# CODEJIN/multi_speaker_tts

Measured on AMD Instinct MI355X. Metric: mel-frames/sec (train step) at batch 32x(128 tok,800 mel), higher is better.
Workload: dtype f32

## Files before the change

### include/mstts.h

```cpp
#ifndef MSTTS_H_
#define MSTTS_H_
#include <stdint.h>
#ifdef __cplusplus
extern "C" {
#endif

typedef void* mstts_stream_t;

enum { MSTTS_OK = 0, MSTTS_ERR_SHAPE = -1, MSTTS_ERR_DTYPE = -2, MSTTS_ERR_ALIGN = -3, MSTTS_ERR_LAUNCH = -4 };
enum { MSTTS_ACT_NONE = 0, MSTTS_ACT_RELU = 1, MSTTS_ACT_TANH = 2, MSTTS_ACT_SIGMOID = 3 };

const char* mstts_last_error(void);
int mstts_abi_version(void);
int mstts_debug_park_cus(int32_t n_workgroups, int64_t microseconds, uint32_t* done_count, mstts_stream_t s);

typedef struct {
    const float* A; const float* B; float* C; const float* bias;
    int64_t M, N, K;
    int64_t lda, ldb, ldc;
    int32_t trans_a, trans_b;
    int32_t win_T, win_C, win_pad;
    int32_t act, accumulate, split_k;
    int64_t batch, stride_a, stride_b, stride_c;
    float alpha;
// ... 215 lines not shown
int32_t mstts_skinny_fwd_splits(int64_t N, int64_t K);
int mstts_skinny_fwd(const float* X, int64_t ldx, const float* W, int64_t ldw, float* P, int64_t pstride, int64_t M, int64_t N,
                     int64_t K, int32_t ksplit, mstts_stream_t s);
int32_t mstts_skinny_bwd_splits(int64_t R, int64_t N);
int mstts_skinny_bwd(const float* dG, int64_t ldg, const float* W, int64_t ldw, float* P, int64_t pstride, int64_t M, int64_t R,
                     int64_t N, int32_t nsplit, mstts_stream_t s);
int mstts_pack_skinny_bwd(const float* W, int64_t ldw, float* Wp, int64_t R, int64_t N, int32_t nsplit, mstts_stream_t s);
int mstts_skinny_bwd_pair(const float* dG, const float* dG2, int64_t ldg, const float* W, const float* W2, int64_t ldw, float* P, float* P2,
                          int64_t pstride, int64_t M, int64_t R, int64_t N, int32_t nsplit, mstts_stream_t s);
int mstts_skinny_bwd_packed(const float* dG, int64_t ldg, const float* Wp, float* P, int64_t pstride, int64_t M, int64_t R,
                            int64_t N, int32_t nsplit, mstts_stream_t s);

int mstts_wg_overlap_add(const float* Y, const float* bias, float* out, int64_t N, int64_t T, int64_t K, int64_t S, int64_t C, mstts_stream_t s);
int mstts_wg_gate(const float* a, int64_t lda, float* z, int64_t rows, int64_t C, mstts_stream_t s);
int mstts_wg_gate_add(const float* a, int64_t lda, const float* b, float* z, int64_t rows, int64_t C, mstts_stream_t s);
int mstts_wg_res_skip(const float* z, const float* rs, float* x, float* out, int64_t rows, int64_t C, int32_t last, int32_t first, mstts_stream_t s);
int mstts_wg_coupling_inv(const float* audio, const float* log_s_b, const float* w_inv, const float* early, float sigma, float* out,
                          int64_t rows, int64_t c, int64_t c_early, mstts_stream_t s);
int mstts_philox_normal(float* out, int64_t n, uint64_t seed, uint32_t stream_id, float sigma, mstts_stream_t s);

typedef struct {
    const float* v; const float* g; float* w; int64_t ldw;
    float* dv; float* dg;
    int64_t rows, cols;
} mstts_wg_wn_desc;
int mstts_wg_weight_norm_fwd(const mstts_wg_wn_desc* table, int64_t n, int64_t max_cols, mstts_stream_t s);
int mstts_wg_weight_norm_bwd(const mstts_wg_wn_desc* table, int64_t n, int64_t max_cols, mstts_stream_t s);
int mstts_wg_coupling_fwd(const float* y, const float* log_s_b, float* next, float* z, int64_t ldz, int64_t z_col, int64_t c_out,
                          float* loss, int64_t rows, int64_t c, mstts_stream_t s);
int mstts_wg_coupling_bwd(const float* y, const float* log_s_b, const float* z, int64_t ldz, int64_t z_col, int64_t c_out, const float* d_next,
                          float inv_size, float* d_y, float* d_log_s_b, int64_t rows, int64_t c, mstts_stream_t s);
int mstts_wg_inv1x1_logdet(const float* params, float* grad, const int64_t* table, int64_t n_flows, float grad_scale, float* loss, mstts_stream_t s);
int mstts_wg_gate_bwd(const float* a, int64_t lda, const float* dz, float* dpre, float* dpre2, int64_t ld2, int64_t rows, int64_t C, mstts_stream_t s);
int mstts_wg_res_skip_bwd(const float* d_x_next, const float* d_skip, float* d_rs, float* d_z, int64_t rows, int64_t C, int32_t last, mstts_stream_t s);
int mstts_wg_overlap_add_bwd(const float* d_up, float* dY, int64_t N, int64_t T, int64_t K, int64_t S, int64_t C, int64_t L, mstts_stream_t s);
int mstts_wg_bias_fold(const float* base, const int64_t* table, float* out, int64_t n_blocks, int64_t width, mstts_stream_t s);
int mstts_adam_tf_clip(float* p, const float* grad, float* m, float* v, const float* sumsq, float sumsq_scale, float clip_norm,
                       float lr_t, float beta1, float beta2, float eps, int64_t n, mstts_stream_t s);

int64_t mstts_ge2e_ws_floats(int64_t N, int64_t D, int64_t S);
int mstts_ge2e_loss_fwd_bwd(const float* x, int64_t ldx, int64_t S, int64_t P, int64_t D, const float* wb, float* out,
                            float* dx, int64_t lddx, float* ws, mstts_stream_t s);

int32_t mstts_skinny_bf16_fwd_splits(int64_t N, int64_t K);
int32_t mstts_skinny_bf16_bwd_splits(int64_t R, int64_t N);
int mstts_pack_bf16_fwd(const float* W, int64_t ldw, void* Wp, int64_t K, int64_t N, int32_t ksplit, mstts_stream_t s);
int mstts_pack_bf16_bwd(const float* W, int64_t ldw, void* Wq, int64_t R, int64_t N, int32_t nsplit, mstts_stream_t s);
int mstts_skinny_fwd_bf16(const float* X, int64_t ldx, const void* Wp, float* P, int64_t pstride, int64_t M, int64_t N, int64_t K,
                          int32_t ksplit, mstts_stream_t s);
int mstts_skinny_bwd_bf16(const float* dG, int64_t ldg, const void* Wq, float* P, int64_t pstride, int64_t M, int64_t R, int64_t N,
                          int32_t nsplit, mstts_stream_t s);

int mstts_fold_rows(const float* src, float* dst, int64_t rows, int64_t cols, int64_t r0, int64_t n, mstts_stream_t s);

typedef struct {
    int64_t B, T, H;
    const float* xw;
    const float* wh; int64_t wh_ld;
    const int32_t* lengths;
    int32_t reverse;
    float zoneout;
    const uint8_t* zc; const uint8_t* zh;
    const float* residual;
    float* out; int64_t out_sb, out_st;
    float* c_hist; float* h_hist; float* acts; float* c_raw;
    float* gates_ws;
    const float* wh_p; float* h_p;
} mstts_lstm_seq_fwd_desc;
int mstts_lstm_seq_fwd(const mstts_lstm_seq_fwd_desc* d, mstts_stream_t s);
int mstts_lstm_seq_fwd_pair(const mstts_lstm_seq_fwd_desc* a, const mstts_lstm_seq_fwd_desc* b, mstts_stream_t s);
int64_t mstts_lstm_seq_ws_floats(int64_t B, int64_t H, int32_t backward);

typedef struct {
    int64_t B, T, H;
    const float* wh; int64_t wh_ld;
    const int32_t* lengths; int32_t reverse;
    float zoneout;
    const uint8_t* zc; const uint8_t* zh;
    const float* d_out; int64_t dout_sb, dout_st;
    const float* c_hist; const float* acts; const float* c_raw;
    float* dgates_step; float* dgates_pos;
    float* ws;
} mstts_lstm_seq_bwd_desc;
int mstts_lstm_seq_bwd(const mstts_lstm_seq_bwd_desc* d, mstts_stream_t s);
int mstts_lstm_seq_bwd_pair(const mstts_lstm_seq_bwd_desc* a, const mstts_lstm_seq_bwd_desc* b, mstts_stream_t s);

int32_t mstts_persist_lstm_supported(int64_t B, int64_t H);
int64_t mstts_persist_lstm_pack_floats(void);
int64_t mstts_persist_lstm_ws_bytes(void);
int mstts_persist_lstm_pack(const float* wh, int64_t wh_ld, float* fwd_pk, float* bwd_pk, mstts_stream_t s);
int64_t mstts_persist_lstm_hist_floats(int64_t T);
int64_t mstts_persist_lstm_bwd_floats(int64_t T);
int mstts_lstm_seq_fwd_pair_persistent(const mstts_lstm_seq_fwd_desc* a, const mstts_lstm_seq_fwd_desc* b, const float* pk_a, const float* pk_b,
                                       float* xch, uint32_t* ctrl, float* hist, mstts_stream_t s);
int mstts_lstm_seq_bwd_pair_persistent(const mstts_lstm_seq_bwd_desc* a, const mstts_lstm_seq_bwd_desc* b, const float* pkt_a, const float* pkt_b,
                                       float* xch, uint32_t* ctrl, const float* hist, float* bws, mstts_stream_t s);
int32_t mstts_persist_lstm_supported_n(int64_t B, int64_t H, int32_t ndir);
int32_t mstts_persist_lstm_fwd_supported_n(int64_t B, int64_t H, int32_t ndir);
int mstts_persist_lstm_pack_fwd(const float* wh, int64_t wh_ld, int64_t H, float* fwd_pk, mstts_stream_t s);
int64_t mstts_persist_lstm_ws_bytes_n(int64_t B, int32_t ndir);
int64_t mstts_persist_lstm_hist_floats_n(int64_t T, int64_t B, int32_t ndir);
int64_t mstts_persist_lstm_bwd_floats_n(int64_t T, int64_t B, int32_t ndir);
int mstts_lstm_seq_fwd_persistent(const mstts_lstm_seq_fwd_desc* a, const float* pk, float* xch, uint32_t* ctrl, float* hist, mstts_stream_t s);
int mstts_lstm_seq_bwd_persistent(const mstts_lstm_seq_bwd_desc* a, const float* pkt, float* xch, uint32_t* ctrl, const float* hist, float* bws, mstts_stream_t s);

typedef struct {
    int64_t B, S, H, P;
    mstts_lsa_const lsa;
    const float* xw0;
    const float* w0f;
    const float* w1; const float* b1;
    const float* wq;
    const uint8_t* zc0; const uint8_t* zh0; const uint8_t* zc1; const uint8_t* zh1;
    float zoneout;
    float* in0; float* in1; float* pj;
    float* c0; float* c1; float* acts0; float* acts1; float* craw0; float* craw1;
    float* q_hist; float* align_hist; float* cum_hist;
    float* gates_ws; float* energy_ws;
    float* q_ws;
    int32_t chains;
    const void* bf_w0f_f; const void* bf_w1_f; const void* bf_wq_f; const void* bf_w0f_b; const void* bf_w1_b; const void* bf_wq_b;
    const float* w0p; const float* w1p;
    const void* w0p16; const void* w1p16;
    const float* w0f_bp; const float* w1_bp; const float* wq_bp;
    const float* wq_t;
    float* act_p;
    int64_t energy_ws_floats;
} mstts_decoder_train_desc;
int32_t mstts_decoder_bf16_splits(int64_t H, int64_t M, int64_t A, int32_t* out6);
int mstts_decoder_train_ws_floats(int64_t B, int64_t H, int64_t M, int64_t A, int64_t* gates, int64_t* q);
int mstts_decoder_train_fwd(const mstts_decoder_train_desc* d, mstts_stream_t s);

typedef struct {
    const float* w0pk; const float* w1pk; const float* wqpk;
    float* xch; uint32_t* ctrl; uint64_t* stamps;
    float* opk;
    int32_t selftest_fail_step;
    int32_t near_xcd;
    const float* pre; const float* b0;
    int32_t recurrent_bf16;
} mstts_persist_desc;
int32_t mstts_persist_fwd_supported(int64_t B, int64_t H, int64_t M, int64_t A, int64_t T, int64_t KS);
int64_t mstts_persist_fwd_ws_bytes(void);
int64_t mstts_persist_pack_floats(int32_t which);
int mstts_persist_pack(const float* w0f, const float* w1, const float* wq, const float* wx0, float* w0pk, float* w1pk, float* wqpk, mstts_stream_t s);
int mstts_decoder_train_fwd_persistent(const mstts_decoder_train_desc* d, const mstts_persist_desc* p, mstts_stream_t s);
int64_t mstts_persist_opk_floats(int64_t S);
int mstts_persist_unpack_history(const float* opk, const mstts_decoder_train_desc* d, mstts_stream_t s);

typedef struct {
    const mstts_decoder_train_desc* fwd;
    float* d_pj; float* dg0; float* dg1; float* dq_hist; float* de_hist; float* d_in0;
    float* ws;
} mstts_decoder_train_bwd_desc;
int mstts_decoder_train_bwd(const mstts_decoder_train_bwd_desc* d, mstts_stream_t s);
int64_t mstts_decoder_train_bwd_ws_floats(int64_t B, int64_t H, int64_t M, int64_t A, int64_t T, int64_t CH);
int32_t mstts_decoder_train_bwd_parts(int64_t H, int64_t M);

int32_t mstts_persist_bwd_supported(int64_t B, int64_t H, int64_t M, int64_t A, int64_t T, int64_t KS);
int64_t mstts_persist_bwd_ws_bytes(void);
int64_t mstts_persist_bwd_pack_floats(int32_t which);
int mstts_persist_bwd_pack(const float* w0f, const float* w1, const float* wq, float* w0t, float* w1t, float* wqt, mstts_stream_t s);
int mstts_decoder_train_bwd_persistent(const mstts_decoder_train_bwd_desc* bd, const mstts_persist_desc* p, mstts_stream_t s);

typedef struct {
    int64_t B, H, P, n_mel, Smax;
    mstts_lsa_const lsa;
    const float* pw0; const float* pb0; const float* pw1; const float* pb1;
    const uint8_t* pm0; const uint8_t* pm1; float prenet_keep;
    const float* wx0; const float* b0;
    const float* w0f; const float* w1; const float* b1; const float* wq;
    const float* wproj; const float* bproj;
    float zoneout;
    float* in0; float* in1; float* pj;
    float* c0; float* c1;
    float* cum;
    float* pre_ws;
    float* linear; float* stop; float* align_hist;
    const float* w0s; const float* wp_pad;
    const float* w0sp; const float* w1p; float* act_p;
    const float* wp_own; const float* vp;
} mstts_decoder_infer_desc;
int32_t mstts_decoder_infer_fast(int64_t B, int64_t H, int64_t P, int64_t M, int64_t A, int64_t n_mel);
int mstts_decoder_infer_steps(const mstts_decoder_infer_desc* d, int64_t step0, int64_t n, mstts_stream_t s);
int64_t mstts_decoder_infer_ws_floats(int64_t B, int64_t H, int64_t P, int64_t T, int64_t A, int64_t n_mel);

typedef struct {
    const float* w0pk; const float* w1pk; const float* wqppk;
    const float* pre0; const float* bf; const float* u; const float* vp; const float* bp_pad;
    float* xch; uint32_t* ctrl;
    void* stamps;
    int32_t selftest_fail_step;
    int32_t near_xcd;
} mstts_persist_infer_desc;
int32_t mstts_persist_infer_supported(int64_t B, int64_t H, int64_t P, int64_t M, int64_t A, int64_t T, int64_t KS, int64_t n_mel);
int64_t mstts_persist_infer_ws_bytes(void);
int64_t mstts_persist_infer_pack_floats(void);
int mstts_persist_infer_pack(const float* wq, const float* wp_pad, int64_t wp_ld, const float* wfm, float* wqppk, mstts_stream_t s);
int mstts_decoder_infer_persistent(const mstts_decoder_infer_desc* d, const mstts_persist_infer_desc* p, mstts_stream_t s);

int mstts_f32_to_bf16(const float* x, void* y_bf16, int64_t n, mstts_stream_t s);
int mstts_bf16_to_f32(const void* x_bf16, float* y, int64_t n, mstts_stream_t s);
int mstts_bf16_chunks_sum(const void* chunks_bf16, int32_t nchunks, int64_t stride, int64_t n, void* out_bf16, mstts_stream_t s);

enum { MSTTS_PROBE_OFF = 0, MSTTS_PROBE_LSA_ENERGY = 1, MSTTS_PROBE_LSA_CONTEXT = 2, MSTTS_PROBE_CELL0_GEMM = 3,
       MSTTS_PROBE_CELL1_GEMM = 4, MSTTS_PROBE_LSA_DALIGN = 5, MSTTS_PROBE_LSA_DENERGY = 6, MSTTS_PROBE_CELL0_DGEMM = 7,
       MSTTS_PROBE_CELL1_DGEMM = 8 };
int mstts_probe_begin(int32_t kind, int64_t max_launches);
int64_t mstts_probe_result(double* total_ms, double* empty_total_ms);

#ifdef __cplusplus
}
#endif
#endif
```

### multi_speaker_tts_amd/csrc/lsa.hip

```cpp
#include "common.h"

namespace mstts {

constexpr int TS = 8;
constexpr int A_ = 128;
constexpr int CH_ = 32;
constexpr int FLD = CH_ + 4;
constexpr int KS_MAX = 31;
constexpr int LKT_LD = 36;

__device__ __forceinline__ float fast_tanh(float x) {
    const float ax = fabsf(x);
    const float e = __expf(-2.0f * ax);
    return copysignf((1.0f - e) / (1.0f + e), x);
}


__global__ __launch_bounds__(256) void lsa_energy_kernel(mstts_lsa_const c, const float* __restrict__ q, int q_parts, long q_pstride,
                                                         float* __restrict__ q_sum, const float* __restrict__ cum,
                                                         float* __restrict__ energy) {
    __shared__ float s_cum[TS + KS_MAX - 1];
    __shared__ float s_red[TS][2];
    const int b = blockIdx.x, t0 = blockIdx.y * TS, T = (int)c.T, KS = (int)c.KS, pad = (KS - 1) / 2;
    const int k = threadIdx.x & (A_ - 1), grp = threadIdx.x >> 7;
// ... 880 lines not shown
        if (t < T) s_a[t] = av[i];
    }
    *reinterpret_cast<float4*>(&s_dc[lane * 4 + 256 * w]) = dsum;
    if (threadIdx.x < TS) s_gn[threadIdx.x] = gn_own;
#pragma unroll
    for (int i = 0; i < NLK4; ++i) {
        const int e = (threadIdx.x + 256 * i) * 4;
        if (e < KS_MAX * A_) *reinterpret_cast<float4*>(&s_lk[e / A_][e % A_]) = lkv[i];
    }
    if (threadIdx.x < TS + KS_MAX - 1) s_cum[threadIdx.x] = cwin;
    __syncthreads();
    float fac[TS / 2];
    {
        float lk[KS_MAX];
#pragma unroll
        for (int j = 0; j < KS_MAX; ++j) lk[j] = s_lk[j][k];
#pragma unroll
        for (int i = 0; i < TS / 2; ++i) {
            const int tt = grp + 2 * i;
            float pre = kv[i] + qk;
#pragma unroll
            for (int j = 0; j < KS_MAX; ++j) pre += s_cum[tt + j] * lk[j];
            const float u = fast_tanh(pre);
            fac[i] = (t0 + tt < T) ? wk * (1.f - u * u) : 0.f;
        }
    }
#pragma unroll
    for (int m = 0; m < MROW; ++m) dcv[m] = *reinterpret_cast<const float4*>(&s_dc[lane * 4 + 256 * m]);
    float part = 0.f;
#pragma unroll
    for (int i = 0; i < T_MAX / 256; ++i) part += av[i] * gnv[i];
    auto tile_dot = [&](const float4& hq, int e) {
        const int tau = e >> 3, j0 = (e & 7) * 4, t = tau - pad + j0;
        float r = 0.f;
        if (j0 < KS && t >= 0 && t < T) r += hq.x * s_a[t];
        if (j0 + 1 < KS && t + 1 >= 0 && t + 1 < T) r += hq.y * s_a[t + 1];
        if (j0 + 2 < KS && t + 2 >= 0 && t + 2 < T) r += hq.z * s_a[t + 2];
        if (j0 + 3 < KS && t + 3 >= 0 && t + 3 < T) r += hq.w * s_a[t + 3];
        return r;
    };
#pragma unroll
    for (int i = 0; i < HT4; ++i) part += tile_dot(ht[i], threadIdx.x + 256 * i);
    if (h_next)
        for (int e = threadIdx.x + 256 * HT4; (e >> 3) < T; e += 256)
            part += tile_dot(reinterpret_cast<const float4*>(h_next + (long)b * T * HLD)[e], e);
    if (w == 0) {
        float p2 = 0.f;
#pragma unroll
        for (int m = 0; m < MROW; ++m) p2 += cxv[m].x * dcv[m].x + cxv[m].y * dcv[m].y + cxv[m].z * dcv[m].z + cxv[m].w * dcv[m].w;
        for (int i = lane * 4 + 256 * MROW; i < M; i += 256) {
            const float4 x = *reinterpret_cast<const float4*>(ctx_fwd + (long)b * ctx_fwd_ld + i);
            float4 y = *reinterpret_cast<const float4*>(dc + i);
            if (d_ctx2)
                for (int pp = 0; pp < max(d_ctx2_parts, 1); ++pp) {
                    const float4 y2 = *reinterpret_cast<const float4*>(d_ctx2 + pp * d_ctx2_pstride + (long)b * d_ctx2_ld + i);
                    y.x += y2.x; y.y += y2.y; y.z += y2.z; y.w += y2.w;
                }
            p2 += x.x * y.x + x.y * y.y + x.z * y.z + x.w * y.w;
        }
        p2 = wave_sum(p2);
        if (lane == 0) s_dot2 = p2;
    }
    part = wave_sum(part);
    if (lane == 0) scratch[w] = part;
#pragma unroll
    for (int r = 0; r < TS / 4; ++r) {
        const int tt = w + 4 * r, t = t0 + tt;
        float acc = 0.f;
#pragma unroll
        for (int m = 0; m < MROW; ++m)
            acc += val[r][m].x * dcv[m].x + val[r][m].y * dcv[m].y + val[r][m].z * dcv[m].z + val[r][m].w * dcv[m].w;
        if (t < len) {
            for (int i = lane * 4 + 256 * MROW; i < M; i += 256) {
                const float4 x = *reinterpret_cast<const float4*>(c.values + ((long)b * T + t) * M + i);
                float4 y = *reinterpret_cast<const float4*>(dc + i);
                if (d_ctx2)
                    for (int pp = 0; pp < max(d_ctx2_parts, 1); ++pp) {
                        const float4 y2 = *reinterpret_cast<const float4*>(d_ctx2 + pp * d_ctx2_pstride + (long)b * d_ctx2_ld + i);
                        y.x += y2.x; y.y += y2.y; y.z += y2.z; y.w += y2.w;
                    }
                acc += x.x * y.x + x.y * y.y + x.z * y.z + x.w * y.w;
            }
        }
        acc = wave_sum(acc);
        if (lane == 0) {
            const float g = (t < T) ? s_G[tt] + s_gn[tt] : 0.f;
            if (t < T) G[(long)b * T + t] = g;
            s_da[tt] = (t < T) ? g + acc : 0.f;
        }
    }
    __syncthreads();
    const float dot = ((scratch[0] + scratch[1]) + (scratch[2] + scratch[3])) + s_dot2;
    if (threadIdx.x < TS) {
        const int t = t0 + threadIdx.x;
        if (t < T) d_e_out[(long)b * T + t] = a_own * (s_da[threadIdx.x] - dot);
    }
    float dq_acc = 0.f;
#pragma unroll
    for (int i = 0; i < TS / 2; ++i) {
        const int tt = grp + 2 * i;
        const float de = (t0 + tt < T) ? s_a[t0 + tt] * (s_da[tt] - dot) : 0.f;
        const float g = de * fac[i];
        s_g[tt][k] = g;
        dq_acc += g;
    }
    if (grp == 1) s_dq[k] = dq_acc;
    __syncthreads();
    if (grp == 0) atomicAdd(dq + (long)b * A_ + k, dq_acc + s_dq[k]);
    {
        const int tt = threadIdx.x >> 5, j = threadIdx.x & 31;
        float acc = 0.f;
        if (j < KS) {
#pragma unroll 8
            for (int kk = 0; kk < A_; kk += 4) {
                const float4 g4 = *reinterpret_cast<const float4*>(&s_g[tt][kk]);
                const float4 l4 = *reinterpret_cast<const float4*>(&s_lk[j][kk]);
                acc += g4.x * l4.x + g4.y * l4.y + g4.z * l4.z + g4.w * l4.w;
            }
        }
        if (t0 + tt < T) h[((long)b * T + t0 + tt) * HLD + j] = acc;
    }
}

constexpr int PT = 32;
constexpr int LP_ROWS = 34, LP_GROUPS = 16;
constexpr int LP_WN = 80;
typedef float lp_f32x16 __attribute__((ext_vector_type(16)));
typedef __bf16 lp_bf16x8 __attribute__((ext_vector_type(8)));
__device__ __forceinline__ uint32_t lp_cvt_pk(float a, float b) {
    uint32_t r;
    asm("v_cvt_pk_bf16_f32 %0, %1, %2" : "=v"(r) : "v"(a), "v"(b));
    return r;
}
__device__ __forceinline__ void lp_split2(float x0, float x1, uint32_t& hi, uint32_t& mid, uint32_t& lo) {
    hi = lp_cvt_pk(x0, x1);
    x0 -= __uint_as_float(hi << 16); x1 -= __uint_as_float(hi & 0xffff0000u);
    mid = lp_cvt_pk(x0, x1);
    x0 -= __uint_as_float(mid << 16); x1 -= __uint_as_float(mid & 0xffff0000u);
    lo = lp_cvt_pk(x0, x1);
}
__device__ __forceinline__ void lp_split8(const float* x, lp_bf16x8& hi, lp_bf16x8& mid, lp_bf16x8& lo) {
    uint4 h, m, l;
    lp_split2(x[0], x[1], h.x, m.x, l.x); lp_split2(x[2], x[3], h.y, m.y, l.y);
    lp_split2(x[4], x[5], h.z, m.z, l.z); lp_split2(x[6], x[7], h.w, m.w, l.w);
    hi = __builtin_bit_cast(lp_bf16x8, h); mid = __builtin_bit_cast(lp_bf16x8, m); lo = __builtin_bit_cast(lp_bf16x8, l);
}
#define LP_SIX(acc, ah, am, al, bh, bm, bl) do { \
        acc = __builtin_amdgcn_mfma_f32_32x32x16_bf16(al, bh, acc, 0, 0, 0); acc = __builtin_amdgcn_mfma_f32_32x32x16_bf16(ah, bl, acc, 0, 0, 0); \
        acc = __builtin_amdgcn_mfma_f32_32x32x16_bf16(am, bm, acc, 0, 0, 0); acc = __builtin_amdgcn_mfma_f32_32x32x16_bf16(am, bh, acc, 0, 0, 0); \
        acc = __builtin_amdgcn_mfma_f32_32x32x16_bf16(ah, bm, acc, 0, 0, 0); acc = __builtin_amdgcn_mfma_f32_32x32x16_bf16(ah, bh, acc, 0, 0, 0); } while (0)
#ifndef LSA_PARAM_WAVES
#define LSA_PARAM_WAVES 3
#endif
__global__ __launch_bounds__(256, LSA_PARAM_WAVES) void lsa_param_bwd_kernel(mstts_lsa_const c, int S, int steps_per_block,
                                                            const float* __restrict__ q_hist, const float* __restrict__ cum_hist,
                                                            const float* __restrict__ de_hist, float* __restrict__ d_keys,
                                                            float* __restrict__ d_loc_k, float* __restrict__ d_score_w,
                                                            float* __restrict__ d_score_b, float* __restrict__ part) {
    __shared__ __attribute__((aligned(16))) uint16_t s_wp[2][3][8][LP_WN];
    __shared__ __attribute__((aligned(16))) float s_de[2][PT];
    const int b = blockIdx.x, t0 = blockIdx.y * PT, T = (int)c.T, B = (int)c.B, KS = (int)c.KS, pad = (KS - 1) / 2;
    const int s_beg = blockIdx.z * steps_per_block, s_end = min(S, s_beg + steps_per_block);
    const int lane = threadIdx.x & 63, wave = threadIdx.x >> 6, l31 = lane & 31, kh = lane >> 5;
    const int a = wave * 32 + l31;
    const int pl = (l31 & 0x13) | ((l31 & 4) << 1) | ((l31 & 8) >> 1);
    const int o1 = (pl & 7) * LP_WN + 8 + (pl & ~7) + 8 * kh, o2 = (l31 & 7) * LP_WN + 8 + (l31 & ~7) + 8 * kh;
    lp_bf16x8 fh[2], fm[2], fl[2];
#pragma unroll
    for (int ks = 0; ks < 2; ++ks) {
        float f[8];
#pragma unroll
        for (int i = 0; i < 8; ++i) { const int j = 16 * ks + 8 * kh + i; f[i] = j < KS ? c.loc_k[j * A_ + a] : 0.f; }
        lp_split8(f, fh[ks], fm[ks], fl[ks]);
    }
    const float sb = c.score_b[a] + c.loc_b[a], wk = c.score_w[a];
    float key_v[16];
    lp_f32x16 acc_keys, acc_lk;
#pragma unroll
    for (int r = 0; r < 16; ++r) {
        const int t = t0 + (r & 7) + 8 * kh + 16 * (r >> 3);
        key_v[r] = t < T ? c.keys[((long)b * T + t) * A_ + a] : 0.f;
        acc_keys[r] = 0.f; acc_lk[r] = 0.f;
    }
    float acc_w = 0.f, acc_b = 0.f;
    auto load_win = [&](int s) -> float {
        float v = 0.f;
        if (wave < 3) {
            const int t = t0 - pad + lane;
            if (lane < PT + KS - 1 && t >= 0 && t < T) v = cum_hist[((long)s * B + b) * T + t];
        } else if (lane < PT) {
            if (t0 + lane < T) v = de_hist[((long)s * B + b) * T + t0 + lane];
        }
        return v;
    };
    float nv = 0.f, nq = 0.f;
    if (s_beg < s_end) { nv = load_win(s_beg); nq = q_hist[((long)s_beg * B + b) * A_ + a]; }
    int buf = 0;
    for (int s = s_beg; s < s_end; ++s, buf ^= 1) {
        if (wave < 3) {
            uint32_t p0, p1, p2;
            lp_split2(nv, 0.f, p0, p1, p2);
            const uint16_t bits = (uint16_t)(wave == 0 ? p0 : wave == 1 ? p1 : p2);
            uint16_t* w = &s_wp[buf][wave][0][8 + lane];
#pragma unroll
            for (int cc = 0; cc < 8; ++cc) w[cc * LP_WN - cc] = bits;
        } else if (lane < PT) s_de[buf][lane] = nv;
        const float qk = nq + sb;
        if (s + 1 < s_end) { nv = load_win(s + 1); nq = q_hist[((long)(s + 1) * B + b) * A_ + a]; }
        __syncthreads();
        const uint16_t* wp = &s_wp[buf][0][0][0];
        lp_f32x16 L;
#pragma unroll
        for (int r = 0; r < 16; ++r) L[r] = 0.f;
#pragma unroll
        for (int ks = 0; ks < 2; ++ks) {
            const lp_bf16x8 ah = *reinterpret_cast<const lp_bf16x8*>(wp + o1 + 16 * ks), am = *reinterpret_cast<const lp_bf16x8*>(wp + 8 * LP_WN + o1 + 16 * ks),
                            al = *reinterpret_cast<const lp_bf16x8*>(wp + 16 * LP_WN + o1 + 16 * ks);
            LP_SIX(L, ah, am, al, fh[ks], fm[ks], fl[ks]);
        }
        float g[16];
#pragma unroll
        for (int r8 = 0; r8 < 2; ++r8) {
            const float4 d0 = *reinterpret_cast<const float4*>(&s_de[buf][8 * kh + 16 * r8]), d1 = *reinterpret_cast<const float4*>(&s_de[buf][8 * kh + 16 * r8 + 4]);
            const float de8[8] = {d0.x, d0.y, d0.z, d0.w, d1.x, d1.y, d1.z, d1.w};
#pragma unroll
            for (int i = 0; i < 8; ++i) {
                const int r = 8 * r8 + i;
                const float u = tanhf_(L[r] + key_v[r] + qk);
                g[r] = de8[i] * wk * (1.f - u * u);
                acc_w += de8[i] * u;
                acc_b += g[r];
                acc_keys[r] += g[r];
            }
        }
#pragma unroll
        for (int ks = 0; ks < 2; ++ks) {
            lp_bf16x8 gh, gm, gl;
            lp_split8(g + 8 * ks, gh, gm, gl);
            const lp_bf16x8 ah = *reinterpret_cast<const lp_bf16x8*>(wp + o2 + 16 * ks), am = *reinterpret_cast<const lp_bf16x8*>(wp + 8 * LP_WN + o2 + 16 * ks),
                            al = *reinterpret_cast<const lp_bf16x8*>(wp + 16 * LP_WN + o2 + 16 * ks);
            LP_SIX(acc_lk, ah, am, al, gh, gm, gl);
        }
    }
#pragma unroll
    for (int r = 0; r < 16; ++r) {
        const int row = (r & 7) + 8 * kh + 16 * (r >> 3);
        if (t0 + row < T) atomicAdd(d_keys + ((long)b * T + t0 + row) * A_ + a, acc_keys[r]);
    }
    acc_w += __shfl_xor(acc_w, 32);
    acc_b += __shfl_xor(acc_b, 32);
    if (part) {
        float* pb = part + ((long)(blockIdx.z * gridDim.y + blockIdx.y) * gridDim.x + blockIdx.x) * (LP_ROWS * A_);
#pragma unroll
        for (int r = 0; r < 16; ++r) pb[((r & 3) + 8 * (r >> 2) + 4 * kh) * A_ + a] = acc_lk[r];
        if (kh == 0) { pb[32 * A_ + a] = acc_w; pb[33 * A_ + a] = acc_b; }
        return;
    }
#pragma unroll
    for (int r = 0; r < 16; ++r) {
        const int row = (r & 3) + 8 * (r >> 2) + 4 * kh;
        if (row < KS) atomicAdd(d_loc_k + row * A_ + a, acc_lk[r]);
    }
    if (kh == 0) {
        atomicAdd(d_score_w + a, acc_w);
        atomicAdd(d_score_b + a, acc_b);
    }
}
__global__ __launch_bounds__(256) void lsa_param_reduce1_kernel(const float* __restrict__ part, int nblk, double* __restrict__ gsum) {
    __shared__ double red[4][64];
    const int e = blockIdx.x * 64 + (threadIdx.x & 63), sub = threadIdx.x >> 6, gz = blockIdx.y;
    const int per = (nblk + LP_GROUPS - 1) / LP_GROUPS, b0 = gz * per, b1 = min(nblk, b0 + per);
    double acc = 0.0;
#pragma unroll 8
    for (int bl = b0 + sub; bl < b1; bl += 4) acc += (double)part[(long)bl * (LP_ROWS * A_) + e];
    red[sub][threadIdx.x & 63] = acc;
    __syncthreads();
    if (sub == 0) gsum[(long)gz * (LP_ROWS * A_) + e] = (red[0][threadIdx.x] + red[1][threadIdx.x]) + (red[2][threadIdx.x] + red[3][threadIdx.x]);
}
__global__ void lsa_param_reduce2_kernel(const double* __restrict__ gsum, int KS, float* __restrict__ d_loc_k, float* __restrict__ d_score_w, float* __restrict__ d_score_b) {
    const int e = blockIdx.x * blockDim.x + threadIdx.x;
    if (e >= LP_ROWS * A_) return;
    double v = 0.0;
#pragma unroll
    for (int gz = 0; gz < LP_GROUPS; ++gz) v += gsum[(long)gz * (LP_ROWS * A_) + e];
    const int row = e / A_, a = e - row * A_;
    if (row < KS) d_loc_k[row * A_ + a] += (float)v;
    else if (row == 32) d_score_w[a] += (float)v;
    else if (row == 33) d_score_b[a] += (float)v;
}

static int check_const(const mstts_lsa_const* c) {
    MSTTS_REQUIRE(c != nullptr, MSTTS_ERR_SHAPE, "lsa: null const block");
    MSTTS_REQUIRE(c->A == A_ && c->CH == CH_, MSTTS_ERR_SHAPE, "lsa: built for A=%d CH=%d, got A=%ld CH=%ld", A_, CH_, (long)c->A, (long)c->CH);
    MSTTS_REQUIRE(c->loc_k && c->loc_b, MSTTS_ERR_SHAPE, "lsa: folded location filter (loc_k/loc_b) missing - call mstts_lsa_fold_location first");
    MSTTS_REQUIRE(c->KS >= 1 && c->KS <= KS_MAX && (c->KS & 1), MSTTS_ERR_SHAPE, "lsa: conv taps must be odd and <= %d", KS_MAX);
    MSTTS_REQUIRE(c->T >= 1 && c->T <= T_MAX, MSTTS_ERR_SHAPE, "lsa: T must be in [1,%d]", T_MAX);
    MSTTS_REQUIRE(c->M % 4 == 0 && aligned16(c->values), MSTTS_ERR_ALIGN, "lsa: memory width %% 4 and 16-byte aligned values required");
    MSTTS_REQUIRE(c->B >= 1, MSTTS_ERR_SHAPE, "lsa: B must be >= 1");
    return MSTTS_OK;
}

}

using namespace mstts;
#define ST(s) ((hipStream_t)(s))

extern "C" int mstts_lsa_energy_fwd(const mstts_lsa_const* c, const float* q, int32_t q_parts, int64_t q_pstride, float* q_sum,
                                    const float* cum, float* energy, mstts_stream_t s) {
    int rc = check_const(c); if (rc) return rc;
    hipLaunchKernelGGL(lsa_energy_kernel, dim3((unsigned)c->B, cdiv(c->T, TS)), dim3(256), 0, ST(s), *c, q, (int)q_parts, (long)q_pstride, q_sum, cum, energy);
    MSTTS_CHECK_LAUNCH("lsa_energy_fwd");
    return MSTTS_OK;
}
extern "C" int mstts_lsa_context_fwd(const mstts_lsa_const* c, const float* energy, const float* cum, float* align, float* cum_next,
                                     float* ctx, int64_t ctx_ld, float* ctx2, int64_t ctx2_ld, mstts_stream_t s) {
    int rc = check_const(c); if (rc) return rc;
    hipLaunchKernelGGL(lsa_context_kernel, dim3((unsigned)c->B, cdiv(c->M, DS)), dim3(256), 0, ST(s), *c, energy, cum, align, cum_next,
                       ctx, (long)ctx_ld, ctx2, (long)ctx2_ld);
    MSTTS_CHECK_LAUNCH("lsa_context_fwd");
    return MSTTS_OK;
}
static void lsa_step_geometry(long T, long M, int* cs, int* tsl, int* dsl) {
    long n = cdiv(T, FS_TSL);
    const long nm = cdiv(M, FS_DSL);
    if (nm > n) n = nm;
    *cs = (int)n;
    *tsl = (int)cdiv(T, n);
    *dsl = (int)(cdiv(cdiv(M, n), 4) * 4);
}
extern "C" int64_t mstts_lsa_step_ws_bytes(int64_t B, int64_t T) { return (B * T + 1) * 8; }
static int lsa_step_fwd_launch(const mstts_lsa_const* c, const float* q, int32_t q_parts, int64_t q_pstride, float* q_sum,
                               const float* cum, float* align, float* cum_next, float* ctx, int64_t ctx_ld, float* ctx2, int64_t ctx2_ld,
                               const mstts_cell_packed_dst* ctx_p, void* granules, uint32_t epoch, int skip, mstts_stream_t s,
                               const LsaQIn* qin = nullptr, const LsaProj* proj = nullptr, const mstts_lsa_prenet* pre = nullptr) {
    int rc = check_const(c); if (rc) return rc;
    MSTTS_REQUIRE(granules && epoch != 0 && ((uintptr_t)granules & 7) == 0, MSTTS_ERR_SHAPE, "lsa_step_fwd: granule buffer (8-byte aligned) and a non-zero epoch required");
    PackedDst cp;
    rc = packed_dst_from(ctx_p, c->M, &cp, "ctx_p"); if (rc) return rc;
    int cs, tsl, dsl;
    lsa_step_geometry(c->T, c->M, &cs, &tsl, &dsl);
    LsaQIn qi;
    memset(&qi, 0, sizeof(qi));
    LsaProj pz;
    memset(&pz, 0, sizeof(pz));
    LsaPre px;
    memset(&px, 0, sizeof(px));
    const bool lkt = c->loc_kt && aligned16(c->loc_kt);
    if (qin && proj) {
        qi = *qin; pz = *proj;
        MSTTS_REQUIRE(cs >= 8 && qi.H == 128 * QJ && lkt, MSTTS_ERR_SHAPE, "lsa_step_fwd_qp: needs >= 8 slices, H == %d and the by-unit filter", 128 * QJ);
        MSTTS_REQUIRE(qi.m1 && qi.wq && aligned16(qi.m1) && aligned16(qi.wq) && qi.m1_ld % 4 == 0, MSTTS_ERR_ALIGN, "lsa_step_fwd_qp: m1 / wq must be 16-byte aligned");
        MSTTS_REQUIRE(pz.wp_own && aligned16(pz.wp_own) && pz.vp && pz.linear && pz.stop && pz.NP >= 2 && pz.NP <= 8 * PJ_OWN && pz.NM < pz.NP, MSTTS_ERR_SHAPE,
                      "lsa_step_fwd_qp: projection width must be 2..%d columns", 8 * PJ_OWN);
        if (pre) {
            MSTTS_REQUIRE(pre->w0 && pre->b0 && pre->w1 && pre->b1 && pre->m0 && pre->m1 && pre->out && pre->P == PR_P && pz.NM <= 8 * PR_K0 &&
                          pz.NM < PR_GLD && pz.NP == 4 * PF_Q && aligned16(pre->w0) && aligned16(pre->w1) && aligned16(pz.vp), MSTTS_ERR_SHAPE,
                          "lsa_step_fwd_qp: in-launch prenet needs P == %d, n_mel <= %d, NP == %d and 16-byte aligned w0 / w1 / vp", PR_P, 8 * PR_K0, 4 * PF_Q);
            px.w0 = pre->w0; px.b0 = pre->b0; px.w1 = pre->w1; px.b1 = pre->b1; px.m0 = pre->m0; px.m1 = pre->m1; px.inv_keep = pre->inv_keep;
            px.out = pre->out; px.out_ld = (long)pre->out_ld;
            rc = packed_dst_from(pre->out_p.base ? &pre->out_p : nullptr, PR_P, &px.out_p, "prenet out_p"); if (rc) return rc;
            px.gf = (unsigned long long*)granules + (c->B * c->T + 1 + c->B * A_);
            if (skip >= 0)
                hipLaunchKernelGGL((lsa_step_kernel<true, true, true, true, true>), dim3((unsigned)(cs * c->B)), dim3(FS_THREADS), 0, ST(s), *c, q, 0, 0L, q_sum, cum,
                                   align, cum_next, ctx, (long)ctx_ld, ctx2, (long)ctx2_ld, cp, (unsigned long long*)granules, (unsigned)epoch, tsl, dsl, cs, skip, qi, pz, px);
            else
                hipLaunchKernelGGL((lsa_step_kernel<false, true, true, true, true>), dim3((unsigned)(cs * c->B)), dim3(FS_THREADS), 0, ST(s), *c, q, 0, 0L, q_sum, cum,
                                   align, cum_next, ctx, (long)ctx_ld, ctx2, (long)ctx2_ld, cp, (unsigned long long*)granules, (unsigned)epoch, tsl, dsl, cs, -1, qi, pz, px);
        } else if (skip >= 0)
            hipLaunchKernelGGL((lsa_step_kernel<true, true, true, true>), dim3((unsigned)(cs * c->B)), dim3(FS_THREADS), 0, ST(s), *c, q, 0, 0L, q_sum, cum,
                               align, cum_next, ctx, (long)ctx_ld, ctx2, (long)ctx2_ld, cp, (unsigned long long*)granules, (unsigned)epoch, tsl, dsl, cs, skip, qi, pz, px);
        else
            hipLaunchKernelGGL((lsa_step_kernel<false, true, true, true>), dim3((unsigned)(cs * c->B)), dim3(FS_THREADS), 0, ST(s), *c, q, 0, 0L, q_sum, cum,
                               align, cum_next, ctx, (long)ctx_ld, ctx2, (long)ctx2_ld, cp, (unsigned long long*)granules, (unsigned)epoch, tsl, dsl, cs, -1, qi, pz, px);
    } else if (qin) {
        qi = *qin;
        MSTTS_REQUIRE(cs >= 8 && qi.H == 128 * QJ && lkt, MSTTS_ERR_SHAPE, "lsa_step_fwd_q: needs at least 8 slices (T > 112 or M > 672), H == %d and the by-unit filter", 128 * QJ);
        MSTTS_REQUIRE(qi.m1 && qi.wq && aligned16(qi.m1) && aligned16(qi.wq) && qi.m1_ld % 4 == 0, MSTTS_ERR_ALIGN, "lsa_step_fwd_q: m1 / wq must be 16-byte aligned");
        if (skip >= 0)
            hipLaunchKernelGGL((lsa_step_kernel<true, true, true>), dim3((unsigned)(cs * c->B)), dim3(FS_THREADS), 0, ST(s), *c, q, 0, 0L, q_sum, cum,
                               align, cum_next, ctx, (long)ctx_ld, ctx2, (long)ctx2_ld, cp, (unsigned long long*)granules, (unsigned)epoch, tsl, dsl, cs, skip, qi, pz, px);
        else
            hipLaunchKernelGGL((lsa_step_kernel<false, true, true>), dim3((unsigned)(cs * c->B)), dim3(FS_THREADS), 0, ST(s), *c, q, 0, 0L, q_sum, cum,
                               align, cum_next, ctx, (long)ctx_ld, ctx2, (long)ctx2_ld, cp, (unsigned long long*)granules, (unsigned)epoch, tsl, dsl, cs, -1, qi, pz, px);
    } else if (skip >= 0)
        hipLaunchKernelGGL(lsa_step_kernel<true>, dim3((unsigned)(cs * c->B)), dim3(FS_THREADS), 0, ST(s), *c, q, (int)q_parts, (long)q_pstride, q_sum, cum,
                           align, cum_next, ctx, (long)ctx_ld, ctx2, (long)ctx2_ld, cp, (unsigned long long*)granules, (unsigned)epoch, tsl, dsl, cs, skip, qi, pz, px);
    else if (lkt)
        hipLaunchKernelGGL((lsa_step_kernel<false, true>), dim3((unsigned)(cs * c->B)), dim3(FS_THREADS), 0, ST(s), *c, q, (int)q_parts, (long)q_pstride, q_sum, cum,
                           align, cum_next, ctx, (long)ctx_ld, ctx2, (long)ctx2_ld, cp, (unsigned long long*)granules, (unsigned)epoch, tsl, dsl, cs, -1, qi, pz, px);
    else
        hipLaunchKernelGGL(lsa_step_kernel<false>, dim3((unsigned)(cs * c->B)), dim3(FS_THREADS), 0, ST(s), *c, q, (int)q_parts, (long)q_pstride, q_sum, cum,
                           align, cum_next, ctx, (long)ctx_ld, ctx2, (long)ctx2_ld, cp, (unsigned long long*)granules, (unsigned)epoch, tsl, dsl, cs, -1, qi, pz, px);
    MSTTS_CHECK_LAUNCH("lsa_step_fwd");
    return MSTTS_OK;
}
extern "C" int mstts_lsa_step_fwd(const mstts_lsa_const* c, const float* q, int32_t q_parts, int64_t q_pstride, float* q_sum,
                                  const float* cum, float* align, float* cum_next, float* ctx, int64_t ctx_ld, float* ctx2, int64_t ctx2_ld,
                                  const mstts_cell_packed_dst* ctx_p, void* granules, uint32_t epoch, mstts_stream_t s) {
    return lsa_step_fwd_launch(c, q, q_parts, q_pstride, q_sum, cum, align, cum_next, ctx, ctx_ld, ctx2, ctx2_ld, ctx_p, granules, epoch, -1, s);
}
extern "C" int32_t mstts_lsa_step_q_supported(int64_t T, int64_t M, int64_t H) {
    int cs, tsl, dsl;
    if (T < 1 || M < 4) return 0;
    lsa_step_geometry(T, M, &cs, &tsl, &dsl);
    return cs >= 8 && H == 128 * QJ;
}
extern "C" int64_t mstts_lsa_step_q_ws_bytes(int64_t B, int64_t T) { return (B * T + 1 + B * A_) * 8; }
extern "C" int mstts_lsa_step_fwd_q(const mstts_lsa_const* c, const float* m1, int64_t m1_ld, const float* wq, int64_t H, int32_t q_bf16,
                                    float* q_sum, const float* cum, float* align, float* cum_next, float* ctx, int64_t ctx_ld, float* ctx2,
                                    int64_t ctx2_ld, const mstts_cell_packed_dst* ctx_p, void* granules, uint32_t epoch, int32_t skip_slice,
                                    mstts_stream_t s) {
    LsaQIn qi;
    qi.m1 = m1; qi.m1_ld = (long)m1_ld; qi.wq = wq; qi.H = (int)H; qi.bf16 = q_bf16 ? 1 : 0;
    return lsa_step_fwd_launch(c, nullptr, 0, 0, q_sum, cum, align, cum_next, ctx, ctx_ld, ctx2, ctx2_ld, ctx_p, granules, epoch,
                               skip_slice >= 0 ? skip_slice : -1, s, &qi);
}
extern "C" int32_t mstts_lsa_step_qp_supported(int64_t T, int64_t M, int64_t H, int64_t NP) {
    return mstts_lsa_step_q_supported(T, M, H) && NP >= 2 && NP <= 8 * PJ_OWN;
}
extern "C" int64_t mstts_lsa_step_qp_ws_bytes(int64_t B, int64_t T) { return (B * T + 1 + B * A_ + B * PR_GLD) * 8; }
extern "C" int32_t mstts_lsa_step_prenet_supported(int64_t P, int64_t NM) { return P == PR_P && NM >= 1 && NM <= 8 * PR_K0 && (NM + 1 + 3) / 4 == PF_Q; }
extern "C" int64_t mstts_lsa_proj_pack_floats(void) { return 8L * QJ * 128 * PJ_OW; }
namespace mstts {
__global__ void lsa_proj_pack_kernel(const float* __restrict__ wp, long ld, int NP, float* __restrict__ out) {
    const int idx = blockIdx.x * blockDim.x + threadIdx.x;
    if (idx >= 8 * QJ * 128 * PJ_OW) return;
    const int i = idx % PJ_OW, ch = (idx / PJ_OW) % 128, jj = (idx / (PJ_OW * 128)) % QJ, cs = idx / (PJ_OW * 128 * QJ);
    const int o = PJ_OWN * cs + i;
    out[idx] = (i < PJ_OWN && o < NP) ? wp[(long)(QJ * ch + jj) * ld + o] : 0.f;
}
}
extern "C" int mstts_lsa_proj_pack(const float* wp, int64_t ld, int64_t H, int64_t NP, float* wp_own, mstts_stream_t s) {
    MSTTS_REQUIRE(wp && wp_own && H == 128 * QJ && NP >= 1 && NP <= 8 * PJ_OWN && ld >= NP, MSTTS_ERR_SHAPE, "lsa_proj_pack: needs H == %d and NP <= %d", 128 * QJ, 8 * PJ_OWN);
    const int n = 8 * QJ * 128 * PJ_OW;
    hipLaunchKernelGGL(mstts::lsa_proj_pack_kernel, dim3((n + 255) / 256), dim3(256), 0, ST(s), wp, (long)ld, (int)NP, wp_own);
    MSTTS_CHECK_LAUNCH("lsa_proj_pack");
    return MSTTS_OK;
}
extern "C" int mstts_lsa_step_fwd_qp(const mstts_lsa_const* c, const float* m1, int64_t m1_ld, const float* wq, int64_t H, const float* wp_own,
                                     const float* vp, const float* bias, int64_t NP, int64_t NM, float* linear, float* stop, const float* cum,
                                     float* align, float* cum_next, float* ctx, int64_t ctx_ld, float* ctx2, int64_t ctx2_ld,
                                     const mstts_cell_packed_dst* ctx_p, const mstts_lsa_prenet* pre, void* granules, uint32_t epoch,
                                     int32_t skip_slice, mstts_stream_t s) {
    MSTTS_REQUIRE(c && granules, MSTTS_ERR_SHAPE, "lsa_step_fwd_qp: null pointer");
    LsaQIn qi;
    qi.m1 = m1; qi.m1_ld = (long)m1_ld; qi.wq = wq; qi.H = (int)H; qi.bf16 = 0;
    LsaProj pj;
    pj.wp_own = wp_own; pj.vp = vp; pj.bias = bias; pj.NP = (int)NP; pj.NM = (int)NM; pj.linear = linear; pj.stop = stop;
    return lsa_step_fwd_launch(c, nullptr, 0, 0, nullptr, cum, align, cum_next, ctx, ctx_ld, ctx2, ctx2_ld, ctx_p, granules, epoch,
                               skip_slice >= 0 ? skip_slice : -1, s, &qi, &pj, pre);
}
extern "C" int mstts_lsa_step_fwd_selftest(const mstts_lsa_const* c, const float* q, int32_t q_parts, int64_t q_pstride, float* q_sum,
                                           const float* cum, float* align, float* cum_next, float* ctx, int64_t ctx_ld, void* granules,
                                           uint32_t epoch, int32_t skip_slice, mstts_stream_t s) {
    MSTTS_REQUIRE(skip_slice >= 0, MSTTS_ERR_SHAPE, "lsa_step_fwd_selftest: skip_slice must be >= 0");
    return lsa_step_fwd_launch(c, q, q_parts, q_pstride, q_sum, cum, align, cum_next, ctx, ctx_ld, nullptr, 0, nullptr, granules, epoch, skip_slice, s);
}
extern "C" int mstts_lsa_dalign_bwd(const mstts_lsa_const* c, const float* d_ctx, int64_t d_ctx_ld, const float* d_ctx2, int64_t d_ctx2_ld,
                                    int32_t d_ctx2_parts, int64_t d_ctx2_pstride, const float* G_next, const float* d_f_next, float* G, float* d_align, mstts_stream_t s) {
    int rc = check_const(c); if (rc) return rc;
    MSTTS_REQUIRE(aligned16(d_ctx) && aligned16(d_ctx2) && d_ctx_ld % 4 == 0 && d_ctx2_ld % 4 == 0, MSTTS_ERR_ALIGN,
                  "lsa_dalign: d_ctx rows must be 16-byte aligned");
    hipLaunchKernelGGL(lsa_dalign_kernel, dim3((unsigned)c->B, cdiv(c->T, TS)), dim3(256), 0, ST(s), *c, d_ctx, (long)d_ctx_ld, d_ctx2,
                       (long)d_ctx2_ld, (int)d_ctx2_parts, (long)d_ctx2_pstride, G_next, d_f_next, G, d_align);
    MSTTS_CHECK_LAUNCH("lsa_dalign_bwd");
    return MSTTS_OK;
}
extern "C" int mstts_lsa_denergy_bwd(const mstts_lsa_const* c, const float* align, const float* d_align, const float* q, const float* cum,
                                     float* d_e, float* dq, float* d_f, mstts_stream_t s) {
    int rc = check_const(c); if (rc) return rc;
    hipLaunchKernelGGL(lsa_denergy_kernel, dim3((unsigned)c->B, cdiv(c->T, TS)), dim3(256), 0, ST(s), *c, align, d_align, q, cum, d_e, dq, d_f);
    MSTTS_CHECK_LAUNCH("lsa_denergy_bwd");
    return MSTTS_OK;
}
extern "C" int mstts_lsa_step_bwd(const mstts_lsa_const* c, const float* d_ctx, int64_t d_ctx_ld, const float* d_ctx2, int64_t d_ctx2_ld,
                                  int32_t d_ctx2_parts, int64_t d_ctx2_pstride, const float* G_next, const float* d_f_next, float* G,
                                  const float* align, const float* q, const float* cum, const float* ctx_fwd, int64_t ctx_fwd_ld,
                                  float* d_e, float* dq, float* d_f, mstts_stream_t s) {
    int rc = check_const(c); if (rc) return rc;
    MSTTS_REQUIRE(aligned16(d_ctx) && aligned16(d_ctx2) && d_ctx_ld % 4 == 0 && d_ctx2_ld % 4 == 0, MSTTS_ERR_ALIGN,
                  "lsa_step_bwd: d_ctx rows must be 16-byte aligned");
    MSTTS_REQUIRE(ctx_fwd && aligned16(ctx_fwd) && ctx_fwd_ld % 4 == 0, MSTTS_ERR_ALIGN, "lsa_step_bwd: the forward context rows (16-byte aligned) are required");
    MSTTS_REQUIRE(aligned16(c->loc_k), MSTTS_ERR_ALIGN, "lsa_step_bwd: the folded filter loc_k must be 16-byte aligned");
    hipLaunchKernelGGL(lsa_step_bwd_kernel, dim3((unsigned)(cdiv(c->T, TS) * c->B)), dim3(256), 0, ST(s), *c, d_ctx, (long)d_ctx_ld, d_ctx2,
                       (long)d_ctx2_ld, (int)d_ctx2_parts, (long)d_ctx2_pstride, G_next, d_f_next, G, align, q, cum, ctx_fwd, (long)ctx_fwd_ld, d_e, dq, d_f,
                       cdiv(c->T, TS));
    MSTTS_CHECK_LAUNCH("lsa_step_bwd");
    return MSTTS_OK;
}
namespace mstts { int gemm_deterministic_now(); }
static void lsa_param_geometry(long B, long T, long S, int* nt, int* chunks, int* spb, bool fixed_order) {
    *nt = cdiv(T, PT);
    int ch = (int)(2048 / (B * *nt));
    if (ch < 1) ch = 1;
    if (fixed_order) ch = 1;
    if (ch > S) ch = (int)S;
    *spb = cdiv(S, ch);
    *chunks = cdiv(S, *spb);
}
extern "C" int64_t mstts_lsa_param_bwd_ws_floats(int64_t B, int64_t T, int64_t S) {
    if (B < 1 || T < 1 || S < 1) return 0;
    int nt, chunks, spb;
    lsa_param_geometry(B, T, S, &nt, &chunks, &spb, false);
    return (int64_t)B * nt * chunks * (LP_ROWS * A_) + 2 * (int64_t)LP_GROUPS * (LP_ROWS * A_);
}
extern "C" int mstts_lsa_param_bwd(const mstts_lsa_const* c, int64_t S, const float* q_hist, const float* cum_hist, const float* de_hist,
                                   float* d_keys, float* d_loc_k, float* d_score_w, float* d_score_b, float* ws, mstts_stream_t s) {
    int rc = check_const(c); if (rc) return rc;
    if (S <= 0) return MSTTS_OK;
    MSTTS_REQUIRE(!ws || (reinterpret_cast<uintptr_t>(ws) & 7u) == 0, MSTTS_ERR_ALIGN, "lsa_param_bwd: the workspace must be 8-byte aligned");
    int nt, chunks, spb;
    lsa_param_geometry(c->B, c->T, S, &nt, &chunks, &spb, gemm_deterministic_now() != 0);
    hipLaunchKernelGGL(lsa_param_bwd_kernel, dim3((unsigned)c->B, nt, chunks), dim3(256), 0, ST(s), *c, (int)S, spb, q_hist, cum_hist,
                       de_hist, d_keys, d_loc_k, d_score_w, d_score_b, ws);
    MSTTS_CHECK_LAUNCH("lsa_param_bwd");
    if (ws) {
        const int nblk = (int)c->B * nt * chunks;
        long nb = (long)nblk * (LP_ROWS * A_);
        nb += nb & 1;
        double* gsum = reinterpret_cast<double*>(ws + nb);
        hipLaunchKernelGGL(lsa_param_reduce1_kernel, dim3(LP_ROWS * A_ / 64, LP_GROUPS), dim3(256), 0, ST(s), ws, nblk, gsum);
        MSTTS_CHECK_LAUNCH("lsa_param_reduce1");
        hipLaunchKernelGGL(lsa_param_reduce2_kernel, dim3(cdiv(LP_ROWS * A_, 256)), dim3(256), 0, ST(s), gsum, (int)c->KS, d_loc_k, d_score_w, d_score_b);
        MSTTS_CHECK_LAUNCH("lsa_param_reduce2");
    }
    return MSTTS_OK;
}

namespace mstts {
__global__ void lsa_filter_by_unit_kernel(const float* __restrict__ loc_k, float* __restrict__ loc_kt, int KS, int A) {
    const int i = blockIdx.x * blockDim.x + threadIdx.x;
    if (i >= A * LKT_LD) return;
    const int a = i / LKT_LD, j = i - a * LKT_LD;
    loc_kt[i] = j < KS ? loc_k[j * A + a] : 0.f;
}
}
extern "C" int mstts_lsa_filter_by_unit(const float* loc_k, float* loc_kt, int64_t KS, int64_t A, mstts_stream_t s) {
    MSTTS_REQUIRE(loc_k && loc_kt && KS >= 1 && KS <= KS_MAX && A >= 1, MSTTS_ERR_SHAPE, "lsa_filter_by_unit: bad arguments (KS <= %d)", KS_MAX);
    MSTTS_REQUIRE(aligned16(loc_kt), MSTTS_ERR_ALIGN, "lsa_filter_by_unit: loc_kt must be 16-byte aligned");
    hipLaunchKernelGGL(lsa_filter_by_unit_kernel, dim3((unsigned)((A * LKT_LD + 255) / 256)), dim3(256), 0, ST(s), loc_k, loc_kt, (int)KS, (int)A);
    MSTTS_CHECK_LAUNCH("lsa_filter_by_unit");
    return MSTTS_OK;
}

extern "C" int mstts_lsa_fold_location(const float* conv_k, const float* conv_b, const float* dense_k, float* loc_k, float* loc_b,
                                       int64_t KS, int64_t CH, int64_t A, mstts_stream_t s) {
    mstts_gemm_desc g;
    memset(&g, 0, sizeof(g));
    g.A = conv_k; g.B = dense_k; g.C = loc_k; g.M = KS; g.N = A; g.K = CH; g.lda = CH; g.ldb = A; g.ldc = A; g.alpha = 1.f; g.split_k = 1; g.batch = 1;
    int rc = mstts_gemm_f32(&g, s);
    if (rc) return rc;
    g.A = conv_b; g.C = loc_b; g.M = 1;
    return mstts_gemm_f32(&g, s);
}

extern "C" int mstts_lsa_unfold_location_grad(const float* conv_k, const float* conv_b, const float* dense_k, const float* d_loc_k,
                                              const float* d_loc_b, float* d_conv_k, float* d_conv_b, float* d_dense_k,
                                              int64_t KS, int64_t CH, int64_t A, mstts_stream_t s) {
    mstts_gemm_desc g;
    memset(&g, 0, sizeof(g));
    g.alpha = 1.f; g.split_k = 1; g.batch = 1; g.accumulate = 1;
    g.A = d_loc_k; g.lda = A; g.B = dense_k; g.ldb = A; g.trans_b = 1; g.C = d_conv_k; g.ldc = CH; g.M = KS; g.N = CH; g.K = A;
    int rc = mstts_gemm_f32(&g, s); if (rc) return rc;
    g.A = d_loc_b; g.C = d_conv_b; g.M = 1;
    rc = mstts_gemm_f32(&g, s); if (rc) return rc;
    memset(&g, 0, sizeof(g));
    g.alpha = 1.f; g.split_k = 1; g.batch = 1; g.accumulate = 1;
    g.A = conv_k; g.lda = CH; g.trans_a = 1; g.B = d_loc_k; g.ldb = A; g.C = d_dense_k; g.ldc = A; g.M = CH; g.N = A; g.K = KS;
    rc = mstts_gemm_f32(&g, s); if (rc) return rc;
    g.A = conv_b; g.lda = CH; g.B = d_loc_b; g.K = 1;
    return mstts_gemm_f32(&g, s);
}
```

### multi_speaker_tts_amd/csrc/persist_bwd.hip

```cpp
#include "persist_fwd_parts.h"

#ifndef BG0_LATE
#define BG0_LATE 10
#endif
#ifndef BSPLIT_C1
#define BSPLIT_C1 1
#endif
#ifndef BPTT_QOWN
#define BPTT_QOWN 1
#endif
#ifndef BPTT_W0LDS
#define BPTT_W0LDS 1
#endif
#ifndef BPTT_KEYS_PER_STEP
#define BPTT_KEYS_PER_STEP 0
#endif
#ifndef BPTT_LATE_OP0
#define BPTT_LATE_OP0 0
#endif
#ifndef BSPLIT_C0
#define BSPLIT_C0 0
#endif
namespace mstts {

__device__ __forceinline__ void bsp_split8(const float (&x)[8], pbf16x8& hi, pbf16x8& mid, pbf16x8& lo) {
#pragma unroll
    for (int e = 0; e < 8; ++e) {
        hi[e] = (__bf16)x[e]; const float r1 = x[e] - (float)hi[e];
        mid[e] = (__bf16)r1; lo[e] = (__bf16)(r1 - (float)mid[e]);
    }
}

constexpr long BDG = 8L * 8 * 2 * 4 * 256;
constexpr long BPART = 256L * 8 * 32 * 4;
constexpr long BPCTX = 32L * 192 * 8 * 4;
constexpr long BDM1 = 32L * 8 * PH;
constexpr long BDA = 32L * 8 * PTMAX;
constexpr long BO_DG1 = 0, BO_DG0 = BO_DG1 + PRING * BDG, BO_PM0 = BO_DG0 + PRING * BDG, BO_PH1 = BO_PM0 + PRING * BPART,
               BO_PH0 = BO_PH1 + PRING * BPART, BO_PCTX = BO_PH0 + PRING * BPART, BO_DM1 = BO_PCTX + PRING * BPCTX,
               BO_DA = BO_DM1 + PRING * BDM1, BXCH_FLOATS = BO_DA + PRING * BDA;
template <int TT> struct BL {
    static constexpr int B_RED = 0,
              B_G = B_RED,
              B_PC = B_G + (TT + 32) * 16,
              B_DA = B_PC + 192 * 4,
              B_PD = B_DA + 8 * TT,
              B_SCR_END = B_PD + 4 * TT,
              B_TR = B_SCR_END > B_RED + 8 * 4 * 256 ? B_SCR_END : B_RED + 8 * 4 * 256,
              B_GP = B_TR + 3 * 128 + 512,
              B_A = B_GP + TT, B_CUM = B_A + TT, B_DE = B_CUM + TT + 48, B_DC = B_DE + TT, B_DPJ = B_DC + 96, B_QF = B_DPJ + 96,
              B_DQ = B_QF + 16, B_DQF = B_DQ + 512, B_LK = B_DQF + 16, B_FLAG = B_LK + 32 * 16, B_STAMP = B_FLAG + 4,
              B_VALT = B_STAMP + 2 * 16,
              B_WQT = B_VALT + 96 * PT,
              B_WQO = B_WQT + 16 * 256 * 4,
              B_FLOATS = B_WQO + (BPTT_QOWN ? 4 * 128 : 0);
    static_assert(B_FLOATS * 4 <= 160 * 1024, "LDS budget");
};
constexpr int NBSTAMP = 16;

struct PersistBwd {
    const float* w1t; const float* w0t; const float* wqt;
    const float* acts0; const float* acts1; const float* craw0; const float* craw1; const float* c0; const float* c1;
    const uint8_t* zc0; const uint8_t* zh0; const uint8_t* zc1; const uint8_t* zh1; float keep;
    const float* align_hist; const float* cum_hist; const float* q_hist;
    const float* keys; const float* values; const int32_t* lengths;
    const float* loc_k; const float* loc_b; const float* score_w; const float* score_b;
    const float* d_pj;
    const float* opk;
    int B, S, T;
    float* dg0; float* dg1; float* dq_hist; float* de_hist; float* d_in0;
    float* xch; unsigned* ctrl; unsigned long long* stamps; int fail_step; int near_xcd;
};

__device__ __forceinline__ pf32x4 cell_bwd(float dm, float& dhs, float& dcs, float si, float tj, float sf, float so, float c, float cp,
                                           float mh, float mc) {
    dm += mh * dhs;
    const float tc = tanhf_(c);
    const float dc = dm * so * (1.f - tc * tc) + mc * dcs;
    pf32x4 dg;
    dg[0] = dc * tj * si * (1.f - si);
    dg[1] = dc * si * (1.f - tj * tj);
    dg[2] = dc * cp * sf * (1.f - sf);
    dg[3] = dm * tc * so * (1.f - so);
    dcs = dcs * (1.f - mc) + dc * sf;
    dhs = dhs * (1.f - mh);
    return dg;
}

template <bool PROF, int TT, bool BF16 = false>
__global__ __launch_bounds__(PTH) void persist_bwd_kernel(PersistBwd d) {
    typedef BL<TT> Y;
    constexpr int B_RED = Y::B_RED, B_G = Y::B_G, B_PC = Y::B_PC, B_DA = Y::B_DA, B_PD = Y::B_PD, B_TR = Y::B_TR, B_GP = Y::B_GP, B_A = Y::B_A, B_CUM = Y::B_CUM,
                  B_DE = Y::B_DE, B_DC = Y::B_DC, B_DPJ = Y::B_DPJ, B_QF = Y::B_QF, B_DQ = Y::B_DQ, B_DQF = Y::B_DQF, B_LK = Y::B_LK, B_FLAG = Y::B_FLAG,
                  B_STAMP = Y::B_STAMP, B_VALT = Y::B_VALT, B_WQT = Y::B_WQT, B_WQO = Y::B_WQO;
    constexpr bool QOWN = BPTT_QOWN != 0 && !BF16;
    constexpr bool W0L = QOWN && BPTT_W0LDS != 0 && !BF16;
    constexpr int NH = TT / 128;
    extern __shared__ __attribute__((aligned(16))) float sm[];
    const int g0 = blockIdx.x, tid0 = threadIdx.x, wave0 = __builtin_amdgcn_readfirstlane(tid0 >> 6);
    int g = g0, gi = g & 7, gj = g >> 3;
    int tid = tid0, lane = tid & 63, wave = wave0;
    const int B = d.B, S = d.S, T = d.T;
    const __amdgpu_buffer_rsrc_t xr = __builtin_amdgcn_make_buffer_rsrc(d.xch, 0, (int)(BXCH_FLOATS * 4), 0x00020000);
    unsigned* sflag = reinterpret_cast<unsigned*>(sm + B_FLAG);

    if (d.near_xcd) persist_scrub(xr, BO_DG1, BO_PM0 - BO_DG1, g0, tid);
    __syncthreads();
    if (tid == 0) {
        const int rz = persist_rendezvous(d.ctrl, g0);
        sflag[0] = rz == 0 ? 1u : 0u;
        sflag[1] = (rz == 2 && d.near_xcd) ? 1u : 0u;
        if (rz == 2 && g0 < 8) __hip_atomic_fetch_add(d.ctrl + 3, 1u, __ATOMIC_RELAXED, __HIP_MEMORY_SCOPE_AGENT);
    }
    __syncthreads();
    if (sflag[0]) return;
    const bool near = sflag[1] != 0;

    constexpr bool BS1 = BSPLIT_C1 != 0 && !BF16 && BPTT_QOWN != 0 && BPTT_W0LDS != 0, BS0 = BSPLIT_C0 != 0 && !BF16;
    constexpr int NW0 = BF16 ? 1 : ((BS0 ? 0 : 32) + (W0L ? 0 : 32)) > 0 ? ((BS0 ? 0 : 32) + (W0L ? 0 : 32)) : 1;
    constexpr int W0H1 = BS0 ? 0 : 32;
    float w1t[BF16 ? 1 : (BS1 ? 32 : 64)], w0t[NW0];
    pbf16x8 wb1t[BF16 ? 8 : 1], wb0t[BF16 ? 8 : 1];
    pbf16x8 w1s[3][BS1 ? 4 : 1];
    pbf16x8 w0s[3][BS0 ? 4 : 1];
    {
        const float* p1 = d.w1t + ((long)(g * 8 + wave) * 64) * 64 + lane;
        const float* p0 = d.w0t + ((long)(g * 8 + wave) * 64) * 64 + lane;
        if constexpr (BF16) {
#pragma unroll
            for (int r = 0; r < 64; ++r) { wb1t[r >> 3][r & 7] = (__bf16)p1[r * 64]; wb0t[r >> 3][r & 7] = (__bf16)p0[r * 64]; }
        } else {
            if constexpr (BS1) {
#pragma unroll
                for (int o = 0; o < 4; ++o) {
                    float x[8];
#pragma unroll
                    for (int e = 0; e < 8; ++e) x[e] = p1[((o >> 1) * 16 + 8 * (o & 1) + e) * 64];
                    bsp_split8(x, w1s[0][o], w1s[1][o], w1s[2][o]);
                }
#pragma unroll
                for (int r = 0; r < 32; ++r) w1t[r] = p1[(32 + r) * 64];
            } else {
#pragma unroll
                for (int r = 0; r < 64; ++r) w1t[r] = p1[r * 64];
            }
            if constexpr (BS0) {
#pragma unroll
                for (int o = 0; o < 4; ++o) {
                    float x[8];
#pragma unroll
                    for (int e = 0; e < 8; ++e) x[e] = p0[((o >> 1) * 16 + 8 * (o & 1) + e) * 64];
                    bsp_split8(x, w0s[0][o], w0s[1][o], w0s[2][o]);
                }
            } else {
#pragma unroll
                for (int r = 0; r < 32; ++r) w0t[r] = p0[r * 64];
            }
            if constexpr (W0L) {
#pragma unroll
                for (int r = 0; r < 32; ++r) sm[B_WQT + r * PTH + tid] = p0[(32 + r) * 64];
            } else {
#pragma unroll
                for (int r = 0; r < 32; ++r) w0t[W0H1 + r] = p0[(32 + r) * 64];
            }
        }
    }
    int ab = gj;
    const bool arow = ab < B;
    const int alen = arow ? (d.lengths ? d.lengths[ab] : T) : 0;
    int ak = tid & 15, atg = tid >> 4;
    float kreg[4 * NH];
    float asb = 0.f, awk = 0.f, asb2 = 0.f;
#define LOAD_KEYS() do { const int gi__ = g & 7, ab__ = g >> 3, ak__ = tid & 15, atg__ = tid >> 4; const bool ar__ = ab__ < B;              \
        _Pragma("unroll") for (int m = 0; m < 4 * NH; ++m) {                                                                              \
            const int t = 128 * (m >> 2) + 4 * atg__ + (m & 3);                                                                            \
            kreg[m] = d.keys[((long)(ar__ ? ab__ : 0) * T + (t < T ? t : 0)) * PA + 16 * gi__ + ak__];    \
        }                                                                                                                                  \
        asb = d.score_b[16 * gi__ + ak__]; asb2 = d.loc_b[16 * gi__ + ak__]; awk = d.score_w[16 * gi__ + ak__]; } while (0)
    {
        LOAD_KEYS();
#if !BPTT_KEYS_PER_STEP
        asb += asb2;
#endif
        for (int x = tid; x < 32 * 16; x += PTH) sm[B_LK + x] = (x < PKS * 16) ? d.loc_k[(x >> 4) * PA + 16 * gi + (x & 15)] : 0.f;
        for (int x = tid; x < 96 * PT; x += PTH) {
            const int c = x >> 7, t = x & 127;
            sm[B_VALT + x] = (arow && t < alen && t < T) ? d.values[((long)ab * T + t) * PM + 96 * gi + c] : 0.f;
        }
        for (int x = tid; x < TT + 48; x += PTH) sm[B_CUM + x] = 0.f;
        for (int x = tid; x < TT; x += PTH) { sm[B_GP + x] = 0.f; sm[B_A + x] = 0.f; sm[B_DE + x] = 0.f; }
        if constexpr (QOWN) {
            if (tid < 128) {
                const int sl = tid >> 4, k4 = (tid >> 2) & 3, e = tid & 3;
                pf32x4 v = reinterpret_cast<const pf32x4*>(d.wqt)[((long)(sl * 16 + k4 * 4 + e)) * 256 + g];
                if constexpr (BF16) { v[0] = bf16_round(v[0]); v[1] = bf16_round(v[1]); v[2] = bf16_round(v[2]); v[3] = bf16_round(v[3]); }
                *reinterpret_cast<pf32x4*>(sm + B_WQO + e * 128 + 16 * sl + 4 * k4) = v;
            }
        } else {
            const pf32x4* wqs = reinterpret_cast<const pf32x4*>(d.wqt) + (long)gi * 16 * 256;
            for (int x = tid; x < 16 * 256; x += PTH) {
                pf32x4 v = wqs[x];
                if constexpr (BF16) { v[0] = bf16_round(v[0]); v[1] = bf16_round(v[1]); v[2] = bf16_round(v[2]); v[3] = bf16_round(v[3]); }
                reinterpret_cast<pf32x4*>(sm + B_WQT)[x] = v;
            }
        }
    }
    int et = wave & 1, er = 16 * et + (lane & 15), ee = lane >> 4, eu = 4 * g + ee;
    bool ew = wave < 2, elive = ew && er < B;
    float dc0s = 0.f, dh0s = 0.f, dc1s = 0.f, dh1s = 0.f;
    unsigned long long* sstamp = reinterpret_cast<unsigned long long*>(sm + B_STAMP);
    unsigned tprev = 0;
    if (PROF && tid < NBSTAMP) sstamp[tid] = 0;
#define PSTAMP(idx) do { if (PROF && tid == 0) { const unsigned n__ = (unsigned)wall_clock64(); sstamp[idx] += (unsigned)(n__ - tprev); tprev = n__; } } while (0)
#define PABORT_CHECK() do { __syncthreads(); if (sflag[0]) return; } while (0)
#define PFAIL() do { sflag[0] = 1; unsigned z__ = 0u; __hip_atomic_compare_exchange_strong(d.ctrl + 1, &z__, 2u, __ATOMIC_RELAXED, __ATOMIC_RELAXED, __HIP_MEMORY_SCOPE_AGENT); } while (0)
    float rav = 0.f, rcv = 0.f, rqv = 0.f, rdv = 0.f;
    const int abc = arow ? ab : 0;
#define LOAD_ROWS(ST) do { const long r__ = (long)(ST) * B + abc; const int t__ = tid & (TT - 1);                                   \
        rav = (d.align_hist + r__ * T)[t__ < T ? t__ : 0]; rcv = (d.cum_hist + r__ * T)[t__ < T ? t__ : 0];                     \
        rqv = (d.q_hist + r__ * PA + 16 * (g & 7))[tid & 15]; rdv = (d.d_pj + r__ * (PH + PM) + PH + 96 * (g & 7))[tid < 96 ? tid : 0]; } while (0)
#define STORE_ROWS() do { const int t__ = tid & (TT - 1);                                                                           \
        sm[B_A + t__] = t__ < T ? rav : 0.f; sm[B_CUM + 15 + t__] = t__ < T ? rcv : 0.f;                                        \
        sm[B_QF + (tid & 15)] = rqv; sm[B_DPJ + (tid < 96 ? tid : 0)] = rdv; } while (0)
    float a1v[4], cr1, cp1, dpm1;
    uint8_t zc1v, zh1v;
#define LOAD_OPERANDS1(ST) do { const long b__ = (long)(ST) * B; const unsigned r__ = (16 * (wave & 1) + (tid & 15)) < (unsigned)B ? 16 * (wave & 1) + (tid & 15) : 0u; \
        const unsigned u__ = 4 * g + ((tid & 63) >> 4);                                                                                   \
                              \
        const pf32x4* ob__ = reinterpret_cast<const pf32x4*>(d.opk) + opk_index((ST), g, 1, 0, tid & 127);                                \
        const pf32x4 A__ = ob__[0], B__ = ob__[128];                                                                                        \
        a1v[0] = A__[0]; a1v[1] = A__[1]; a1v[2] = A__[2]; a1v[3] = A__[3]; cr1 = B__[0]; cp1 = B__[1];                                      \
        zc1v = (uint8_t)(__float_as_uint(B__[2]) & 1u); zh1v = (uint8_t)((__float_as_uint(B__[2]) >> 1) & 1u);                               \
        dpm1 = (d.d_pj + b__ * (PH + PM))[wave < 2 ? r__ * (PH + PM) + u__ : 0u]; } while (0)
    LOAD_OPERANDS1(S - 1);
    LOAD_ROWS(S - 1);
    __syncthreads();
    STORE_ROWS();
    __syncthreads();
    if (PROF && tid == 0) tprev = (unsigned)wall_clock64();

    for (int s = S - 1; s >= 0; --s) {
        const bool first = s == S - 1;
        const unsigned kk = (unsigned)(S - 1 - s);
        const unsigned slot = kk & 3u, nslot = (kk + 3u) & 3u;
        const unsigned gen = (kk >> 2) & 1u, ngen = ((kk - 1u) >> 2) & 1u;
        tid = tid0; g = g0; wave = wave0;
        asm volatile("" : "+v"(tid));
        asm volatile("" : "+s"(g), "+s"(wave));
        lane = tid & 63; gi = g & 7; gj = g >> 3; ab = gj; ak = tid & 15; atg = tid >> 4;
        et = wave & 1; er = 16 * et + (lane & 15); ee = lane >> 4; eu = 4 * g + ee;
        ew = wave < 2; elive = ew && er < B;
        if (s == d.fail_step && g == 0 && tid == 0) {
            __hip_atomic_store(d.ctrl + 1, 3u, __ATOMIC_RELAXED, __HIP_MEMORY_SCOPE_AGENT);
            sflag[0] = 1;
        }
        const long sB = (long)s * B, sB1 = sB + B;
        const bool rowok = er < B;
        const unsigned erc = rowok ? (unsigned)er : 0u;
        const unsigned oH = erc * PH + eu, o4H = erc * 4 * PH + eu;
        unsigned uoff[2], qoff[QOWN ? 5 : 1];
        pf32x4 uv[2] = {{0.f, 0.f, 0.f, 0.f}, {0.f, 0.f, 0.f, 0.f}};
        pf32x4 qv5[QOWN ? 5 : 1];
#define ISSUE_UPDATE1() do { if (tid < 256) { const int row = tid >> 3, sl = tid & 7;                                                  \
            if constexpr (QOWN) {                   \
                _Pragma("unroll") for (int p = 0; p < 4; ++p) qoff[p] = (unsigned)((BO_DM1 + slot * BDM1 + ((long)row * 8 + sl) * 16 + 4 * p) * 4); \
                qoff[4] = first ? qoff[0] : (unsigned)((BO_PH1 + nslot * BPART + (((long)g * 8 + sl) * 32 + row) * 4) * 4);           \
                issue<5>(xr, qoff, qv5);                                                                                              \
            } else {                                                                                                                  \
            uoff[0] = (unsigned)((BO_DM1 + slot * BDM1 + (((long)g * 8 + sl) * 32 + row) * 4) * 4);                                   \
            uoff[1] = first ? uoff[0] : (unsigned)((BO_PH1 + nslot * BPART + (((long)g * 8 + sl) * 32 + row) * 4) * 4);               \
            issue<2>(xr, uoff, uv); } } } while (0)
#define ISSUE_UPDATE0() do { if (tid < 256) { const int row = tid >> 3, src = tid & 7;                                                 \
            uoff[0] = (unsigned)((BO_PM0 + slot * BPART + (((long)g * 8 + src) * 32 + row) * 4) * 4);                                 \
            uoff[1] = first ? uoff[0] : (unsigned)((BO_PH0 + nslot * BPART + (((long)g * 8 + src) * 32 + row) * 4) * 4);              \
            issue<2>(xr, uoff, uv); } } while (0)
        float fac[4 * NH];
#pragma unroll
        for (int m = 0; m < 4 * NH; ++m) fac[m] = 0.f;
        if (arow) {
            sm[B_G + (tid < 240 ? tid : (15 + TT) * 16 + (tid - 240))] = 0.f;
            pf32x4 pc[1] = {{0.f, 0.f, 0.f, 0.f}};
            unsigned pcoff[1];
            pcoff[0] = (unsigned)((BO_PCTX + nslot * BPCTX + ((long)ab * 192 + 24 * gi) * 32) * 4 + 16 * (tid < 192 ? tid : 0));
            if (!first && tid < 192) issue<1>(xr, pcoff, pc);
            __syncthreads();
            PSTAMP(15);
            {
                const float qk = sm[B_QF + ak] + (BPTT_KEYS_PER_STEP ? asb + asb2 : asb);
#pragma unroll
                for (int hh = 0; hh < NH; ++hh) {
                    pf32x4 loc = {0.f, 0.f, 0.f, 0.f};
#pragma unroll
                    for (int ks = 0; ks < 8; ++ks)
                        loc = PMFMA(sm[B_CUM + 128 * hh + 16 * wave + (lane & 15) + 4 * ks + (lane >> 4)], sm[B_LK + (4 * ks + (lane >> 4)) * 16 + (lane & 15)], loc);
#pragma unroll
                    for (int m = 0; m < 4; ++m) {
                        const float kv = (128 * hh + 4 * atg + m < T) ? kreg[4 * hh + m] : 0.f;
                        const float u = tanhf_(kv + qk + loc[m]); fac[4 * hh + m] = awk * (1.f - u * u);
                    }
                }
            }
            PSTAMP(0);
            if (!first) {
                if (tid < 192) {
                    { const unsigned g1[1] = {ngen}; if (!complete<1>(xr, pcoff, pc, d.ctrl, g1)) PFAIL(); }
                    *reinterpret_cast<pf32x4*>(sm + B_PC + 4 * tid) = pc[0];
                }
            }
            PABORT_CHECK();
            PSTAMP(1);
            if (tid < 24) {
                pf32x4 acc = {0.f, 0.f, 0.f, 0.f};
                if (!first) {
#pragma unroll
                    for (int src = 0; src < 8; ++src) acc += *reinterpret_cast<const pf32x4*>(sm + B_PC + (tid * 8 + src) * 4);
                    reinterpret_cast<pf32x4*>(d.d_in0 + (sB1 + ab) * (PM + PH) + 96 * gi)[tid] = acc;
                }
                *reinterpret_cast<pf32x4*>(sm + B_DC + 4 * tid) = acc + *reinterpret_cast<const pf32x4*>(sm + B_DPJ + 4 * tid);
            }
            __syncthreads();
            {
                const int t = tid & 127, cq = tid >> 7;
                pf32x4 vg[6];
                if (NH > 1) {
                    const int tt = 128 + t < T ? 128 + t : 0;
                    const pf32x4* vp4 = reinterpret_cast<const pf32x4*>(d.values + ((long)ab * T + tt) * PM + 96 * gi + 24 * cq);
#pragma unroll
                    for (int c4 = 0; c4 < 6; ++c4) vg[c4] = vp4[c4];
                }
                float acc = 0.f, acc2 = 0.f;
#pragma unroll 2
                for (int c4 = 0; c4 < 6; ++c4) {
                    const pf32x4 dcv = *reinterpret_cast<const pf32x4*>(sm + B_DC + 24 * cq + 4 * c4);
#pragma unroll
                    for (int e = 0; e < 4; ++e) acc += sm[B_VALT + (24 * cq + 4 * c4 + e) * PT + t] * dcv[e];
                }
                sm[B_PD + cq * TT + t] = acc;
                if (NH > 1) {
#pragma unroll
                    for (int c4 = 0; c4 < 6; ++c4) {
                        const pf32x4 dcv = *reinterpret_cast<const pf32x4*>(sm + B_DC + 24 * cq + 4 * c4);
#pragma unroll
                        for (int e = 0; e < 4; ++e) acc2 += vg[c4][e] * dcv[e];
                    }
                    sm[B_PD + cq * TT + 128 + t] = 128 + t < T ? acc2 : 0.f;
                }
            }
            __syncthreads();
            if (tid < 32 * NH) {
                pf32x4 pd = (*reinterpret_cast<const pf32x4*>(sm + B_PD + 4 * tid) + *reinterpret_cast<const pf32x4*>(sm + B_PD + TT + 4 * tid)) +
                            (*reinterpret_cast<const pf32x4*>(sm + B_PD + 2 * TT + 4 * tid) + *reinterpret_cast<const pf32x4*>(sm + B_PD + 3 * TT + 4 * tid));
                pd += *reinterpret_cast<const pf32x4*>(sm + B_GP + 4 * tid);
                const long o = ((long)ab * 8 + gi) * TT + 4 * tid;
                xpublish(xr, (unsigned)((BO_DA + slot * BDA + o) * 4), pd, gen);
            }
            PSTAMP(2);
        }
        if (arow) {
            if (tid < 256 * NH) {
                unsigned off[1]; pf32x4 v[1];
                off[0] = (unsigned)((BO_DA + slot * BDA + (long)ab * 8 * TT) * 4 + 16 * tid);
                const unsigned g1[1] = {gen};
                if (!gather<1>(xr, off, v, d.ctrl, g1)) PFAIL();
                *reinterpret_cast<pf32x4*>(sm + B_DA + 4 * tid) = v[0];
            }
            PABORT_CHECK();
            PSTAMP(3);
            if (wave == 0) {
                float da[2 * NH], av[2 * NH];
                float dp = 0.f;
#pragma unroll
                for (int i = 0; i < 2 * NH; ++i) {
                    float x = 0.f;
#pragma unroll
                    for (int k = 0; k < 8; ++k) x += sm[B_DA + k * TT + 64 * i + lane];
                    da[i] = x; av[i] = sm[B_A + 64 * i + lane];
                }
                if (NH == 1) dp = av[0] * da[0] + av[1] * da[1];
                else {
#pragma unroll
                    for (int i = 0; i < 2 * NH; ++i) dp += av[i] * da[i];
                }
                const float dot = wave_sum(dp);
                float* de = d.de_hist + (sB + ab) * T;
#pragma unroll
                for (int i = 0; i < 2 * NH; ++i) {
                    const float e = av[i] * (da[i] - dot);
                    sm[B_DE + 64 * i + lane] = e;
                    if (gi == 0 && lane + 64 * i < T) de[lane + 64 * i] = e;
                }
            }
            __syncthreads();
            {
                float dqp = 0.f;
#pragma unroll
                for (int m = 0; m < 4 * NH; ++m) {
                    const int t = 128 * (m >> 2) + 4 * atg + (m & 3);
                    const float gv = sm[B_DE + t] * fac[m];
                    sm[B_G + (15 + t) * 16 + ak] = gv;
                    dqp += gv;
                }
                sm[B_DQ + atg * 16 + ak] = dqp;
            }
            __syncthreads();
            if (tid < 16) {
                float qv = 0.f;
#pragma unroll
                for (int u = 0; u < 32; ++u) qv += sm[B_DQ + u * 16 + tid];
                sm[B_DQF + tid] = BF16 ? bf16_round(qv) : qv;
                (d.dq_hist + (sB + ab) * PA + 16 * gi)[tid] = qv;
            }
            __syncthreads();
            if constexpr (QOWN) {
                if (tid < 4) xpublish(xr, (unsigned)((BO_DM1 + slot * BDM1 + ((long)ab * 8 + gi) * 16 + 4 * tid) * 4), *reinterpret_cast<const pf32x4*>(sm + B_DQF + 4 * tid), gen);
            } else
            if (tid < 256) {
                pf32x4 out = {0.f, 0.f, 0.f, 0.f};
#pragma unroll 1
                for (int k4 = 0; k4 < 4; ++k4) {
                    const pf32x4 dq4 = *reinterpret_cast<const pf32x4*>(sm + B_DQF + 4 * k4);
#pragma unroll
                    for (int e = 0; e < 4; ++e) {
                        const pf32x4 wv = *reinterpret_cast<const pf32x4*>(sm + B_WQT + ((k4 * 4 + e) * 256 + tid) * 4);
                        out[e] += wv[0] * dq4[0] + wv[1] * dq4[1] + wv[2] * dq4[2] + wv[3] * dq4[3];
                    }
                }
                const long o = (((long)tid * 8 + gi) * 32 + ab) * 4;
                xpublish(xr, (unsigned)((BO_DM1 + slot * BDM1 + o) * 4), out, gen);
            }
            PSTAMP(4);
#pragma unroll 1
            for (int hh = 0; hh < NH; ++hh) {
                const int p0 = 128 * hh + 4 * atg;
                float acc[4] = {0.f, 0.f, 0.f, 0.f};
                float w0 = sm[B_G + p0 * 16 + ak], w1 = sm[B_G + (p0 + 1) * 16 + ak], w2 = sm[B_G + (p0 + 2) * 16 + ak],
                      w3 = sm[B_G + (p0 + 3) * 16 + ak];
#pragma unroll 4
                for (int x = 0; x < PKS; ++x) {
                    const float lk = sm[B_LK + (PKS - 1 - x) * 16 + ak];
                    acc[0] += w0 * lk; acc[1] += w1 * lk; acc[2] += w2 * lk; acc[3] += w3 * lk;
                    w0 = w1; w1 = w2; w2 = w3; w3 = sm[B_G + (p0 + x + 4) * 16 + ak];
                }
#pragma unroll
                for (int m = 0; m < 4; ++m) {
                    float v = acc[m];
                    v += dpp_mov<0xB1, 0xf>(0.f, v);
                    v += dpp_mov<0x4E, 0xf>(0.f, v);
                    v += dpp_mov<0x141, 0xf>(0.f, v);
                    v += dpp_mov<0x140, 0xf>(0.f, v);
                    acc[m] = v;
                }
                if (ak == 0) {
#pragma unroll
                    for (int m = 0; m < 4; ++m) sm[B_GP + p0 + m] += acc[m];
                }
            }
        } else {
            PSTAMP(0); PSTAMP(1); PSTAMP(2); PSTAMP(3);
            if constexpr (QOWN) {
                if (tid < 4) xpublish(xr, (unsigned)((BO_DM1 + slot * BDM1 + ((long)ab * 8 + gi) * 16 + 4 * tid) * 4), (pf32x4){0.f, 0.f, 0.f, 0.f}, gen);
            } else
            if (tid < 256) {
                const long o = (((long)tid * 8 + gi) * 32 + ab) * 4;
                xpublish(xr, (unsigned)((BO_DM1 + slot * BDM1 + o) * 4), (pf32x4){0.f, 0.f, 0.f, 0.f}, gen);
            }
            PSTAMP(4);
        }
        PSTAMP(5);
        LOAD_ROWS(s > 0 ? s - 1 : 0);
        __syncthreads();
        ISSUE_UPDATE1();
        if (tid < 256) {
            const int row = tid >> 3, sl = tid & 7;
            if constexpr (QOWN) {
                { const unsigned g5[5] = {gen, gen, gen, gen, first ? gen : ngen}; if (!complete<5>(xr, qoff, qv5, d.ctrl, g5)) PFAIL(); }
                uv[1] = qv5[4];
                uv[0] = (pf32x4){0.f, 0.f, 0.f, 0.f};
#pragma unroll
                for (int p = 0; p < 4; ++p) {
#pragma unroll
                    for (int e = 0; e < 4; ++e) {
                        const pf32x4 wv = *reinterpret_cast<const pf32x4*>(sm + B_WQO + e * 128 + 16 * sl + 4 * p);
                        uv[0][e] += wv[0] * qv5[p][0] + wv[1] * qv5[p][1] + wv[2] * qv5[p][2] + wv[3] * qv5[p][3];
                    }
                    asm volatile("" ::: "memory");
                }
            } else {
                const unsigned g2[2] = {gen, first ? gen : ngen}; if (!complete<2>(xr, uoff, uv, d.ctrl, g2)) PFAIL();
            }
            if (first) uv[1] = (pf32x4){0.f, 0.f, 0.f, 0.f};
#pragma unroll
            for (int e = 0; e < 4; ++e) {
                float x = uv[0][e], y = uv[1][e];
                x += dpp_mov<0xB1, 0xf>(0.f, x); x += dpp_mov<0x4E, 0xf>(0.f, x); x += dpp_mov<0x141, 0xf>(0.f, x);
                y += dpp_mov<0xB1, 0xf>(0.f, y); y += dpp_mov<0x4E, 0xf>(0.f, y); y += dpp_mov<0x141, 0xf>(0.f, y);
                uv[0][e] = x; uv[1][e] = y;
            }
            if (sl == 0) {
                *reinterpret_cast<pf32x4*>(sm + B_TR + row * 4) = uv[0];
                *reinterpret_cast<pf32x4*>(sm + B_TR + 128 + row * 4) = uv[1];
            }
        }
        STORE_ROWS();
        PABORT_CHECK();
        PSTAMP(6);
        {
            const float dm = sm[B_TR + er * 4 + ee] + dpm1;
            float dhs = dh1s + sm[B_TR + 128 + er * 4 + ee];
            const float mh = zh1v ? d.keep : 0.f, mc = zc1v ? d.keep : 0.f;
            const pf32x4 dgv = cell_bwd(dm, dhs, dc1s, a1v[0], a1v[1], a1v[2], a1v[3], cr1, cp1, mh, mc);
            dh1s = dhs;
            if (ew) {
#pragma unroll
                for (int q = 0; q < 4; ++q) sm[B_TR + 384 + (q * 32 + er) * 4 + ee] = dgv[q];
            }
            __syncthreads();
            if (tid < 128) {
                const int gate = tid >> 5, row = tid & 31;
                const pf32x4 val = *reinterpret_cast<const pf32x4*>(sm + B_TR + 384 + tid * 4);
                const long o = ((((long)(gi * 8 + (gj >> 2)) * 2 + (row >> 4)) * 4 + (gj & 3)) * 64 + gate * 16 + (row & 15)) * 4;
                xpublish_near(xr, (unsigned)((BO_DG1 + slot * BDG + o) * 4), val, gen, near);
            }
            if (elive) { float* o = d.dg1 + sB * 4 * PH; o[o4H] = dgv[0]; o[o4H + PH] = dgv[1]; o[o4H + 2 * PH] = dgv[2]; o[o4H + 3 * PH] = dgv[3]; }
        }
        PSTAMP(7);
#define PROD_GATHER(OFF_DG)                                                                                                           \
        pf32x4 bq[8];                                                                                                                \
        {                                                                                                                            \
            unsigned off[8];                                                                                                         \
            _Pragma("unroll") for (int x = 0; x < 8; ++x)                                                                            \
                off[x] = (unsigned)(((OFF_DG) + slot * BDG + ((((long)(gi * 8 + wave) * 2 + (x >> 2)) * 4 + (x & 3)) * 64 + lane) * 4) * 4); \
            const unsigned g8[8] = {gen, gen, gen, gen, gen, gen, gen, gen};                                                         \
            if (!gather<8>(xr, off, bq, d.ctrl, g8)) PFAIL();                                                                            \
        }                                                                                                                            \
        pbf16x8 bqh[BF16 ? 4 : 1];              \
        if constexpr (BF16) {                                                                                                        \
            _Pragma("unroll") for (int x = 0; x < 4; ++x)                                                                            \
                _Pragma("unroll") for (int e = 0; e < 8; ++e) bqh[x][e] = (__bf16)bq[(x >> 1) * 4 + 2 * (x & 1) + (e >> 2)][e & 3];  \
        }
#define PROD_HALF(half, WT, WBASE, WB, WS, OFF_OUT, IS_CTX, SPL, ALDS)                                                                \
        {                                                                                                                            \
            pf32x4 acc[2][2];                                                                                                        \
            _Pragma("unroll") for (int kt = 0; kt < 2; ++kt)                                                                         \
                _Pragma("unroll") for (int t = 0; t < 2; ++t) acc[kt][t] = (pf32x4){0.f, 0.f, 0.f, 0.f};                             \
            if constexpr (BF16) {                                                                                                    \
                _Pragma("unroll") for (int j = 0; j < 2; ++j)                                                                        \
                    _Pragma("unroll") for (int kt = 0; kt < 2; ++kt) {                                                               \
                        acc[kt][0] = PMFMA_BF16(WB[(half) * 4 + kt * 2 + j], bqh[j], acc[kt][0]);                                     \
                        acc[kt][1] = PMFMA_BF16(WB[(half) * 4 + kt * 2 + j], bqh[2 + j], acc[kt][1]);                                 \
                    }                                                                                                                \
            } else if constexpr (SPL) {                                                                                              \
                                                   \
                _Pragma("unroll") for (int t = 0; t < 2; ++t) {                                                                      \
                    pbf16x8 bp__[3][2];                                                                                              \
                    _Pragma("unroll") for (int j = 0; j < 2; ++j) {                                                                  \
                        float f__[8];                                                                                                \
                        _Pragma("unroll") for (int e = 0; e < 8; ++e) f__[e] = bq[t * 4 + 2 * j + (e >> 2)][e & 3];                  \
                        bsp_split8(f__, bp__[0][j], bp__[1][j], bp__[2][j]);                                                         \
                    }                                                                                                                \
                    _Pragma("unroll") for (int kt = 0; kt < 2; ++kt) {                                                               \
                        pf32x4 a__ = {0.f, 0.f, 0.f, 0.f};                                                                           \
                        _Pragma("unroll") for (int j = 0; j < 2; ++j) {                                                              \
                            a__ = PMFMA_BF16(WS[2][kt * 2 + j], bp__[0][j], a__);                                                    \
                            a__ = PMFMA_BF16(WS[0][kt * 2 + j], bp__[2][j], a__);                                                    \
                            a__ = PMFMA_BF16(WS[1][kt * 2 + j], bp__[1][j], a__);                                                    \
                            a__ = PMFMA_BF16(WS[1][kt * 2 + j], bp__[0][j], a__);                                                    \
                            a__ = PMFMA_BF16(WS[0][kt * 2 + j], bp__[1][j], a__);                                                    \
                            a__ = PMFMA_BF16(WS[0][kt * 2 + j], bp__[0][j], a__);                                                    \
                        }                                                                                                            \
                        *reinterpret_cast<pf32x4*>(sm + B_RED + ((wave * 4 + kt * 2 + t) * 64 + lane) * 4) = a__;                    \
                    }                                                                                                                \
                    __builtin_amdgcn_sched_barrier(0);                                                                               \
                }                                                                                                                    \
            } else {                                                                                                                 \
                _Pragma("unroll") for (int ks = 0; ks < 16; ++ks)                                                                    \
                    _Pragma("unroll") for (int kt = 0; kt < 2; ++kt) {                                                               \
                        float a__;                                                                                                   \
                        if constexpr (ALDS) a__ = sm[B_WQT + (kt * 16 + ks) * PTH + tid]; else a__ = WT[(WBASE) + kt * 16 + ks];     \
                        acc[kt][0] = PMFMA(a__, bq[ks >> 2][ks & 3], acc[kt][0]);                                                    \
                        acc[kt][1] = PMFMA(a__, bq[4 + (ks >> 2)][ks & 3], acc[kt][1]);                                              \
                    }                                                                                                                \
            }                                                                                                                        \
            if ((half) == 1) __syncthreads();                                                 \
            if constexpr (BF16 || !(SPL)) {                           \
                _Pragma("unroll") for (int kt = 0; kt < 2; ++kt)                                                                     \
                    _Pragma("unroll") for (int t = 0; t < 2; ++t)                                                                    \
                        *reinterpret_cast<pf32x4*>(sm + B_RED + ((wave * 4 + kt * 2 + t) * 64 + lane) * 4) = acc[kt][t];             \
            }                                                                                                                        \
            PABORT_CHECK();                                                                                                          \
            if (tid < 256) {                                                                                                         \
                const int tile = tid >> 6, l = tid & 63, kt = tile >> 1, t = tile & 1;                                               \
                pf32x4 r = {0.f, 0.f, 0.f, 0.f};                                                                                     \
                _Pragma("unroll") for (int w = 0; w < 8; ++w) r += *reinterpret_cast<const pf32x4*>(sm + B_RED + ((w * 4 + tile) * 64 + l) * 4); \
                const int blk = 4 * kt + (l >> 4), row = 16 * t + (l & 15);                                                          \
                if (IS_CTX) {                                                                                                        \
                    if (blk < 6) {                                                                                                   \
                        const long o = (((long)row * 192 + 6 * gj + blk) * 8 + gi) * 4;                                              \
                        xpublish(xr, (unsigned)((BO_PCTX + slot * BPCTX + o) * 4), r, gen);                                                 \
                    }                                                                                                                \
                } else {                                                                                                             \
                    const long o = (((long)(8 * gj + blk) * 8 + gi) * 32 + row) * 4;                                                 \
                    xpublish(xr, (unsigned)(((OFF_OUT) + slot * BPART + o) * 4), r, gen);                                                   \
                }                                                                                                                    \
            }                                                                                                                        \
        }
        pf32x4 A0_, B0_;
        {
            PROD_GATHER(BO_DG1)
            PROD_HALF(0, w1t, 0, wb1t, w1s, BO_PM0, false, BS1, false)
            PSTAMP(8);
#define LOAD_OPERANDS0() do {  \
                const pf32x4* ob = reinterpret_cast<const pf32x4*>(d.opk) + opk_index(s, g, 0, 0, tid & 127);        \
                A0_ = ob[0]; B0_ = ob[128];                                                                                           \
                 \
            } while (0)
#if !BPTT_LATE_OP0
            LOAD_OPERANDS0();
#endif
            PROD_HALF(1, w1t, (BS1 ? 0 : 32), wb1t, w1s, BO_PH1, false, false, false)
        }
        PSTAMP(9);
        __syncthreads();
#if BPTT_LATE_OP0
        LOAD_OPERANDS0();
#endif
        ISSUE_UPDATE0();
        if (tid < 256) {
            const int row = tid >> 3, src = tid & 7;
            { const unsigned g2[2] = {gen, first ? gen : ngen}; if (!complete<2>(xr, uoff, uv, d.ctrl, g2)) PFAIL(); }
            if (first) uv[1] = (pf32x4){0.f, 0.f, 0.f, 0.f};
#pragma unroll
            for (int e = 0; e < 4; ++e) {
                float x = uv[0][e], y = uv[1][e];
                x += dpp_mov<0xB1, 0xf>(0.f, x); x += dpp_mov<0x4E, 0xf>(0.f, x); x += dpp_mov<0x141, 0xf>(0.f, x);
                y += dpp_mov<0xB1, 0xf>(0.f, y); y += dpp_mov<0x4E, 0xf>(0.f, y); y += dpp_mov<0x141, 0xf>(0.f, y);
                uv[0][e] = x; uv[1][e] = y;
            }
            if (src == 0) {
                *reinterpret_cast<pf32x4*>(sm + B_TR + row * 4) = uv[0];
                *reinterpret_cast<pf32x4*>(sm + B_TR + 128 + row * 4) = uv[1];
            }
        }
        PABORT_CHECK();
        PSTAMP(10);
        {
            const float dm = sm[B_TR + er * 4 + ee];
            float dhs = dh0s + sm[B_TR + 128 + er * 4 + ee];
            const unsigned bits0 = __float_as_uint(B0_[2]);
            const float mh = (bits0 & 2u) ? d.keep : 0.f, mc = (bits0 & 1u) ? d.keep : 0.f;
            const pf32x4 dgv = cell_bwd(dm, dhs, dc0s, A0_[0], A0_[1], A0_[2], A0_[3], B0_[0], B0_[1], mh, mc);
            dh0s = dhs;
            if (ew) {
#pragma unroll
                for (int q = 0; q < 4; ++q) sm[B_TR + 384 + (q * 32 + er) * 4 + ee] = dgv[q];
            }
            __syncthreads();
            if (tid < 128) {
                const int gate = tid >> 5, row = tid & 31;
                const pf32x4 val = *reinterpret_cast<const pf32x4*>(sm + B_TR + 384 + tid * 4);
                const long o = ((((long)(gi * 8 + (gj >> 2)) * 2 + (row >> 4)) * 4 + (gj & 3)) * 64 + gate * 16 + (row & 15)) * 4;
                xpublish_near(xr, (unsigned)((BO_DG0 + slot * BDG + o) * 4), val, gen, near);
            }
            if (elive) { float* o = d.dg0 + sB * 4 * PH; o[o4H] = dgv[0]; o[o4H + PH] = dgv[1]; o[o4H + 2 * PH] = dgv[2]; o[o4H + 3 * PH] = dgv[3]; }
        }
        PSTAMP(11);
        {
            if constexpr (BG0_LATE > 0) { const unsigned long long t__ = wall_clock64(); while (wall_clock64() - t__ < (unsigned long long)BG0_LATE) __builtin_amdgcn_s_sleep(1); }
            PROD_GATHER(BO_DG0)
            PROD_HALF(0, w0t, 0, wb0t, w0s, BO_PM0, true, BS0, false)
            PSTAMP(12);
            PROD_HALF(1, w0t, W0H1, wb0t, w0s, BO_PH0, false, false, W0L)
        }
        PSTAMP(13);
#ifndef EXP_NO_OPLOAD
        LOAD_OPERANDS1(s > 0 ? s - 1 : 0);
#endif
#if BPTT_KEYS_PER_STEP
        LOAD_KEYS();
#endif
        __syncthreads();
        PSTAMP(14);
    }
    if (tid == 0) {
        __hip_atomic_fetch_add(d.ctrl + 2, 1u, __ATOMIC_RELAXED, __HIP_MEMORY_SCOPE_AGENT);
        if (PROF && d.stamps) {
#pragma unroll
            for (int x = 0; x < NBSTAMP; ++x) d.stamps[(long)g * NBSTAMP + x] = sstamp[x];
        }
    }
#undef PSTAMP
#undef PABORT_CHECK
#undef PFAIL
#undef PROD_GATHER
#undef ISSUE_UPDATE1
#undef ISSUE_UPDATE0
#undef PROD_HALF
#undef LOAD_OPERANDS0
#undef LOAD_KEYS
#undef LOAD_ROWS
#undef LOAD_OPERANDS1
#undef STORE_ROWS
}

__global__ void persist_pack_bwd_kernel(const float* __restrict__ w0f, const float* __restrict__ w1, float* __restrict__ w0t, float* __restrict__ w1t) {
    const long n = 256L * 8 * 64 * 64;
    for (long p = blockIdx.x * (long)blockDim.x + threadIdx.x; p < 2 * n; p += (long)gridDim.x * blockDim.x) {
        const bool c1 = p >= n;
        long r = c1 ? p - n : p;
        const int lane = (int)(r & 63); r >>= 6;
        const int reg = (int)(r & 63); r >>= 6;
        const int wave = (int)(r & 7), g = (int)(r >> 3);
        const int gi = g & 7, gj = g >> 3;
        const int half = reg >> 5, kt = (reg >> 4) & 1, ks = reg & 15;
        const int m = lane & 15, gate = lane >> 4;
        const int unit_c = 32 * (4 * wave + (ks >> 2)) + 4 * gi + (ks & 3);
        const long col = (long)gate * PH + unit_c;
        const int ok = 16 * kt + m;
        float v;
        if (c1) {
            const long row = (half == 0 ? 0 : PH) + 32 * gj + ok;
            v = w1[row * 4 * PH + col];
        } else if (half == 0) {
            v = ok < 24 ? w0f[(long)(24 * gj + ok) * 4 * PH + col] : 0.f;
        } else {
            v = w0f[(long)(PM + 32 * gj + ok) * 4 * PH + col];
        }
        if (c1) w1t[p - n] = v; else w0t[p] = v;
    }
}
__global__ void persist_pack_wqt_kernel(const float* __restrict__ wq, float* __restrict__ wqt) {
    const int p = blockIdx.x * blockDim.x + threadIdx.x;
    if (p >= 8 * 16 * 256 * 4) return;
    const int kq = p & 3, l = (p >> 2) & 255, ke = (p >> 10) & 15, gi = p >> 14;
    const int k4 = ke >> 2, e = ke & 3;
    wqt[p] = wq[(long)(4 * l + e) * PA + 16 * gi + 4 * k4 + kq];
}

__global__ void persist_unpack_history_kernel(const float* __restrict__ opk, int S, int B, float* acts0, float* acts1, float* craw0, float* craw1,
                                              float* c0, float* c1) {
    const long n = (long)S * PWG * 2 * 128;
    for (long i = blockIdx.x * (long)blockDim.x + threadIdx.x; i < n; i += (long)gridDim.x * blockDim.x) {
        const int tid = (int)(i & 127), cell = (int)((i >> 7) & 1), g = (int)((i >> 8) & 255), s = (int)(i >> 16);
        const int row = 16 * (tid >> 6) + (tid & 15), u = 4 * g + ((tid & 63) >> 4);
        if (row >= B) continue;
        const pf32x4* ob = reinterpret_cast<const pf32x4*>(opk) + opk_index(s, g, cell, 0, tid);
        const pf32x4 A = ob[0], Bv = ob[128];
        float* acts = (cell ? acts1 : acts0) + ((long)s * B + row) * 4 * PH + u;
        acts[0] = A[0]; acts[PH] = A[1]; acts[2 * PH] = A[2]; acts[3 * PH] = A[3];
        (cell ? craw1 : craw0)[((long)s * B + row) * PH + u] = Bv[0];
        (cell ? c1 : c0)[((long)s * B + row) * PH + u] = Bv[1];
    }
}

}
using namespace mstts;

extern "C" int64_t mstts_persist_opk_floats(int64_t S) { return S * OPK_FLOATS_PER_STEP; }

extern "C" int mstts_persist_unpack_history(const float* opk, const mstts_decoder_train_desc* d, mstts_stream_t s) {
    MSTTS_REQUIRE(opk && d && d->acts0 && d->acts1 && d->craw0 && d->craw1 && d->c0 && d->c1 && d->H == PH && d->B >= 1 && d->B <= PROWS, MSTTS_ERR_SHAPE,
                  "persist_unpack_history: null pointer or unsupported shape");
    hipLaunchKernelGGL(persist_unpack_history_kernel, dim3(4096), dim3(256), 0, (hipStream_t)s, opk, (int)d->S, (int)d->B, d->acts0, d->acts1, d->craw0,
                       d->craw1, d->c0, d->c1);
    MSTTS_CHECK_LAUNCH("persist_unpack_history");
    return MSTTS_OK;
}

extern "C" int64_t mstts_persist_bwd_ws_bytes(void) { return BXCH_FLOATS * 4; }
extern "C" int64_t mstts_persist_bwd_pack_floats(int32_t which) { return which < 2 ? 256L * 8 * 64 * 64 : 8L * 16 * 256 * 4; }

extern "C" int32_t mstts_persist_bwd_supported(int64_t B, int64_t H, int64_t M, int64_t A, int64_t T, int64_t KS) {
    if (!(B >= 1 && B <= PROWS && H == PH && M == PM && A == PA && T >= 1 && T <= PTMAX && KS == PKS)) return 0;
    static int memo[PERSIST_MAX_DEVICES];
    return persist_device_memo(memo, [](int dev) {
        int cus = 0, per_cu = 0;
        if (hipDeviceGetAttribute(&cus, hipDeviceAttributeMultiprocessorCount, dev) != hipSuccess || cus < PWG) return false;
        bool ok = true;
        int per = 0;
#define PBW_SETUP(P_, T_)                                                                                                                              \
        ok = ok && hipFuncSetAttribute((const void*)persist_bwd_kernel<P_, T_>, hipFuncAttributeMaxDynamicSharedMemorySize, (int)(BL<T_>::B_FLOATS * 4)) == hipSuccess && \
             hipOccupancyMaxActiveBlocksPerMultiprocessor(&per, (const void*)persist_bwd_kernel<P_, T_>, PTH, (size_t)BL<T_>::B_FLOATS * 4) == hipSuccess && per >= 1;
        PBW_SETUP(false, 128) PBW_SETUP(true, 128) PBW_SETUP(false, 256) PBW_SETUP(true, 256)
#undef PBW_SETUP
#define PBW_SETUP16(P_, T_)                                                                                                                            \
        ok = ok && hipFuncSetAttribute((const void*)persist_bwd_kernel<P_, T_, true>, hipFuncAttributeMaxDynamicSharedMemorySize, (int)(BL<T_>::B_FLOATS * 4)) == hipSuccess && \
             hipOccupancyMaxActiveBlocksPerMultiprocessor(&per, (const void*)persist_bwd_kernel<P_, T_, true>, PTH, (size_t)BL<T_>::B_FLOATS * 4) == hipSuccess && per >= 1;
        PBW_SETUP16(false, 128) PBW_SETUP16(true, 128) PBW_SETUP16(false, 256) PBW_SETUP16(true, 256)
#undef PBW_SETUP16
        (void)per_cu;
        return ok;
    });
}

extern "C" int mstts_persist_bwd_pack(const float* w0f, const float* w1, const float* wq, float* w0t, float* w1t, float* wqt, mstts_stream_t s) {
    MSTTS_REQUIRE(w0f && w1 && wq && w0t && w1t && wqt, MSTTS_ERR_SHAPE, "persist_bwd_pack: null pointer");
    hipLaunchKernelGGL(persist_pack_bwd_kernel, dim3(4096), dim3(256), 0, (hipStream_t)s, w0f, w1, w0t, w1t);
    MSTTS_CHECK_LAUNCH("persist_pack_bwd");
    hipLaunchKernelGGL(persist_pack_wqt_kernel, dim3(8 * 16 * 4), dim3(256), 0, (hipStream_t)s, wq, wqt);
    MSTTS_CHECK_LAUNCH("persist_pack_wqt");
    return MSTTS_OK;
}

extern "C" int mstts_decoder_train_bwd_persistent(const mstts_decoder_train_bwd_desc* bd, const mstts_persist_desc* p, mstts_stream_t s) {
    MSTTS_REQUIRE(bd && bd->fwd && p && bd->d_pj && bd->dg0 && bd->dg1 && bd->dq_hist && bd->de_hist && bd->d_in0 && p->w0pk && p->w1pk && p->wqpk &&
                  p->xch && p->ctrl, MSTTS_ERR_SHAPE, "decoder_train_bwd_persistent: null pointer");
    const mstts_decoder_train_desc* d = bd->fwd;
    const long B = d->B, S = d->S, H = d->H, M = d->lsa.M, A = d->lsa.A, T = d->lsa.T;
    MSTTS_REQUIRE(d->lsa.B == B && mstts_persist_bwd_supported(B, H, M, A, T, d->lsa.KS), MSTTS_ERR_SHAPE,
                  "decoder_train_bwd_persistent: shape or device not supported (see mstts_persist_bwd_supported)");
    MSTTS_REQUIRE(d->zc0 && d->zh0 && d->zc1 && d->zh1, MSTTS_ERR_SHAPE, "decoder_train_bwd_persistent: the four zoneout keep-masks are required");
    MSTTS_REQUIRE(p->opk, MSTTS_ERR_SHAPE, "decoder_train_bwd_persistent: the packed operand blocks of the persistent forward (opk) are required");
    MSTTS_REQUIRE(d->align_hist && d->cum_hist && d->q_hist && d->lsa.keys && d->lsa.values &&
                  d->lsa.loc_k && d->lsa.loc_b && d->lsa.score_w && d->lsa.score_b, MSTTS_ERR_SHAPE, "decoder_train_bwd_persistent: forward state missing");
    MSTTS_REQUIRE(aligned16(p->xch) && aligned16(bd->d_in0) && (M + H) % 4 == 0, MSTTS_ERR_ALIGN, "decoder_train_bwd_persistent: 16-byte alignment");
    hipStream_t hs = (hipStream_t)s;
    hipError_t e = hipMemsetAsync(p->xch, 0xFF, BXCH_FLOATS * 4, hs);
    if (e == hipSuccess) e = hipMemsetAsync(p->ctrl, 0, PCTRL_WORDS * sizeof(unsigned), hs);
    if (e != hipSuccess) return set_err(MSTTS_ERR_LAUNCH, "decoder_train_bwd_persistent: memset: %s", hipGetErrorString(e));
    PersistBwd a;
    a.w1t = p->w1pk; a.w0t = p->w0pk; a.wqt = p->wqpk;
    a.acts0 = d->acts0; a.acts1 = d->acts1; a.craw0 = d->craw0; a.craw1 = d->craw1; a.c0 = d->c0; a.c1 = d->c1;
    a.zc0 = d->zc0; a.zh0 = d->zh0; a.zc1 = d->zc1; a.zh1 = d->zh1; a.keep = 1.f - d->zoneout;
    a.align_hist = d->align_hist; a.cum_hist = d->cum_hist; a.q_hist = d->q_hist;
    a.keys = d->lsa.keys; a.values = d->lsa.values; a.lengths = d->lsa.lengths;
    a.loc_k = d->lsa.loc_k; a.loc_b = d->lsa.loc_b; a.score_w = d->lsa.score_w; a.score_b = d->lsa.score_b;
    a.d_pj = bd->d_pj; a.opk = p->opk; a.B = (int)B; a.S = (int)S; a.T = (int)T;
    a.dg0 = bd->dg0; a.dg1 = bd->dg1; a.dq_hist = bd->dq_hist; a.de_hist = bd->de_hist; a.d_in0 = bd->d_in0;
    a.xch = p->xch; a.ctrl = p->ctrl; a.stamps = (unsigned long long*)p->stamps; a.fail_step = p->selftest_fail_step > 0 ? p->selftest_fail_step - 1 : -1; a.near_xcd = p->near_xcd;
#define PBW_LAUNCH(T_)                                                                                                                  \
    {                                                                                                                                   \
        const size_t lds = (size_t)BL<T_>::B_FLOATS * 4;                                                                                \
        if (p->recurrent_bf16) {                                                                                                        \
            if (p->stamps) hipLaunchKernelGGL((persist_bwd_kernel<true, T_, true>), dim3(PWG), dim3(PTH), lds, hs, a);                  \
            else hipLaunchKernelGGL((persist_bwd_kernel<false, T_, true>), dim3(PWG), dim3(PTH), lds, hs, a);                           \
        } else {                                                                                                                        \
            if (p->stamps) hipLaunchKernelGGL((persist_bwd_kernel<true, T_>), dim3(PWG), dim3(PTH), lds, hs, a);                        \
            else hipLaunchKernelGGL((persist_bwd_kernel<false, T_>), dim3(PWG), dim3(PTH), lds, hs, a);                                 \
        }                                                                                                                               \
    }
    if (a.T <= 128) PBW_LAUNCH(128) else PBW_LAUNCH(256)
#undef PBW_LAUNCH
    MSTTS_CHECK_LAUNCH("persist_bwd");
    return MSTTS_OK;
}
```

### multi_speaker_tts_amd/engine.py

```python
from __future__ import annotations

import ctypes as C
import os
import warnings

import numpy as np
import torch

from . import lib
from .lib import ACT_NONE, ACT_RELU, ACT_TANH, gemm, ptr, call
from .masks import MaskSet, step_seed
from .params import CELL, ENC_CELL, LSA, VOC, Dims, ParamStore, bank_suffix
from .training import (Engine, _split_k, _split_k_big, bn_train_fwd, conv_bn_bwd, conv_fwd, exponential_decay, lstm_layer_grads, lstm_seq_bwd,
                       lstm_seq_fwd)

MAX_PLANS = 64



def learning_rate(step):
    from . import Hyper_Parameters as hp
    return exponential_decay(hp.Train.Learning_Rate, step)


PERSIST_STRIKES = 2
PERSIST_COOLDOWN = 200
VOC_OVERLAP = os.environ.get("MSTTS_VOC_OVERLAP", "1") != "0"
POSTNET_WGRAD_OVERLAP = os.environ.get("MSTTS_POSTNET_WGRAD_OVERLAP", "1") != "0"
ENC_TAIL_OVERLAP = os.environ.get("MSTTS_ENC_TAIL_OVERLAP", "1") != "0"
ENC_OVERLAP = os.environ.get("MSTTS_ENC_OVERLAP", "1") != "0"


class _WS:
    """Attribute bag of device buffers for one (B, T_enc, L) shape: views into the engine's workspace arena."""


class _LateScalars:

    def __init__(self, event, slot, wr_rate):
        self.event, self.slot, self.wr_rate, self._res = event, slot, wr_rate, None

    def get(self):
        if self._res is None:
            self.event.synchronize()
            s = self.slot.numpy().copy()
            wr = float(s[3]) * self.wr_rate
            self._res = {"Linear_Loss": float(s[0]), "Postnet_Loss": float(s[1]), "Stop_Loss": float(s[2]),
                         "Weight_Regularization_Loss": wr, "Loss": float(s[0] + s[1] + s[2]) + wr}
        return self._res


class _Arena:

    ALIGN = 256

    def __init__(self, device):
        self.device, self.buf, self.cap, self.generation = device, None, 0, 0

    def ensure(self, nbytes):
        if nbytes <= self.cap:
            return False
        self.buf = None
        self.cap = int(nbytes)
        self.buf = torch.zeros(self.cap, dtype=torch.uint8, device=self.device)
        self.generation += 1
        return True


class _Carver:

    def __init__(self, arena, count):
        self.arena, self.count, self.off = arena, count, 0
        self.zero = []
        self.overflow = False

    def take(self, shape, dtype=torch.float32, zero=False):
        n = int(np.prod(shape)) if not isinstance(shape, int) else int(shape)
        size = torch.empty(0, dtype=dtype).element_size()
        nbytes = (n * size + _Arena.ALIGN - 1) // _Arena.ALIGN * _Arena.ALIGN
        off, self.off = self.off, self.off + max(nbytes, _Arena.ALIGN)
        if self.count or self.off > self.arena.cap:
            self.overflow = self.overflow or not self.count
            return None
        t = self.arena.buf[off:off + n * size].view(dtype)
        t = t.view(shape) if not isinstance(shape, int) else t
        if zero:
            self.zero.append(t)
        return t


class TrainEngine(Engine):
    def __init__(self, dims: Dims = None, device="cuda", seed=1234, rank=0, world=1, values=None,
                 update_vocoder_bn=True, use_l1=None, wr_rate=None, adam=None, recurrent_dtype=None, gemm_dtype=None, fuse_query=True,
                 arena_hint=None, deterministic=None):
        lib.load()
        self.d = dims or Dims()
        self.device = torch.device(device)
        self.seed, self.rank, self.world = seed, rank, world
        self.update_vocoder_bn = update_vocoder_bn
        self.fuse_query = bool(fuse_query)
        from . import Hyper_Parameters as hp
        self.use_l1 = bool(hp.Train.Use_L1_Loss) if use_l1 is None else use_l1
        self.wr_rate = float(hp.Train.Weight_Regularization_Rate) if wr_rate is None else wr_rate
        self.adam = (hp.Train.ADAM.Beta1, hp.Train.ADAM.Beta2, hp.Train.ADAM.Epsilon) if adam is None else adam
        self.params = ParamStore(self.d, self.device, seed=seed, values=values)
        self._plans = {}
        self._arena = _Arena(self.device)
        self._active_plan = None
        self._pinned = {}
        self.arena_hint = arena_hint
        self.deterministic = (os.environ.get("MSTTS_DETERMINISTIC", "0") == "1") if deterministic is None else bool(deterministic)
        self.arena_poison = os.environ.get("MSTTS_ARENA_POISON", "0") == "1"
        self.global_step = 0
        d = self.d
        H, M = d.dec_lstm, d.mem
        self.w0f = self._f(M + H, 4 * H)
        self.proj_ld = (d.n_mel + 1 + 3) // 4 * 4
        self.wp_pad = self._f(H + M, self.proj_ld)
        self.bp_pad = self._f(self.proj_ld)
        self.dwp_pad = self._f(H + M, self.proj_ld)
        self.dw0f = self._f(M + H, 4 * H)
        self.loc_k, self.loc_b, self.d_loc_k = self._f(d.att_k, d.att), self._f(d.att), self._f(d.att_k, d.att)
        self.loc_kt = self._f(d.att, 36) if d.att_k <= 31 else None
        lb = lib.load()
        self.fused_cells = bool(lb.mstts_cell_fwd_supported(H, M + H)) and bool(lb.mstts_cell_fwd_supported(H, 2 * H))
        self.w0p = self._f((M + H) * 4 * H) if self.fused_cells else None
        self.w1p = self._f(2 * H * 4 * H) if self.fused_cells else None
        self.w0p16 = self.w1p16 = None
        self.bwd_splits = (int(lb.mstts_skinny_bwd_splits(M + H, 4 * H)), int(lb.mstts_skinny_bwd_splits(2 * H, 4 * H)), int(lb.mstts_skinny_bwd_splits(H, d.att)))
        ok = lambda R, sp: sp > 0 and R % 32 == 0
        self.w0f_bp = self._f((M + H) * 4 * H) if ok(M + H, self.bwd_splits[0]) else None
        self.w1_bp = self._f(2 * H * 4 * H) if ok(2 * H, self.bwd_splits[1]) else None
        self.wq_bp = self._f(H * d.att) if ok(H, self.bwd_splits[2]) else None
        He = d.enc_lstm
        self.enc_whp = {dr: self._f(He * 4 * He) for dr in ("fw", "bw")} if lb.mstts_cell_fwd_supported(He, He) else None
        self.wq_t = self._f(d.att * H) if d.att == 128 else None
        rdt, gdt = (recurrent_dtype or "f32").lower(), (gemm_dtype or "f32").lower()
        self.persist_bf16 = rdt == "bf16" and gdt == "bf16" and d.prenet == 256 and os.environ.get("MSTTS_PERSIST_BF16", "1") != "0"
        self.persist = (os.environ.get("MSTTS_PERSIST", "1") != "0" and (rdt == "f32" or self.persist_bf16)
                        and bool(lb.mstts_persist_fwd_supported(1, H, M, d.att, 1, d.att_k)))
        self.exact_f32_products = False
        self.persist_fallbacks = 0
        self._moving_snapshot = None
        self._persist_strikes = 0
        self._persist_off = 0
        self._persist_warned = False
        self.persist_disabled_steps = 0
        self.non_persistent_plans = 0
        self._warned_shapes = set()
        self.persist_selftest = 0
        self.persist_bwd_selftest = 0
        self.persist_stamps = None
        self.persist_bwd = self.persist and os.environ.get("MSTTS_PERSIST_BWD", "1") != "0" and bool(lb.mstts_persist_bwd_supported(1, H, M, d.att, 1, d.att_k))
        self.persist_bwd_fallbacks = 0
        self.speaker_ticket_redos = 0
        self.trace_events, self.bptt_end_event = False, None
        self.collective_redos = 0
        self.persist_bwd_stamps = None
        if self.persist:
            self.pk = [self._f(int(lb.mstts_persist_pack_floats(i))) for i in range(3)]
        self.persist_enc = os.environ.get("MSTTS_PERSIST_ENC", "1") != "0" and bool(lb.mstts_persist_lstm_supported(1, He))
        self.persist_enc_fallbacks = 0
        if self.persist_enc:
            n = int(lb.mstts_persist_lstm_pack_floats())
            self.enc_pk = {dr: (self._f(n), self._f(n)) for dr in ("fw", "bw")}
        if self.device.type == "cuda":
            self._side = torch.cuda.Stream(device=self.device)
            self._enc_stream = torch.cuda.Stream(device=self.device)
            self._voc_stream = self._enc_stream
        if self.persist_bwd:
            self.pkb = [self._f(int(lb.mstts_persist_bwd_pack_floats(i))) for i in range(3)]
        self.flip = {}
        self.big_tiles = os.environ.get("MSTTS_SPLIT_K_BIG", "1") != "0"
        self._derived_stale = True
        self.gemm_dtype = (gemm_dtype or "f32").lower()
        if self.gemm_dtype not in ("f32", "bf16"):
            raise ValueError("gemm_dtype must be 'f32' or 'bf16'")
        self.recurrent_dtype = (recurrent_dtype or "f32").lower()
        if self.recurrent_dtype not in ("f32", "bf16"):
            raise ValueError("recurrent_dtype must be 'f32' or 'bf16'")
        self.bf = None
        if self.recurrent_dtype == "bf16" and lb.mstts_cell_fwd_bf16_supported(H, M + H) and lb.mstts_cell_fwd_bf16_supported(H, 2 * H):
# ... 405 lines not shown
        host = w.enc_ctrl_host if which == 0 else w.enc_ctrl_host_b
        host.copy_(w.enc_ctrl, non_blocking=True)
        done = torch.cuda.Event()
        done.record()
        return done, host, n_wg

    def _enc_check(self, w, ticket):
        done, host, n_wg = ticket
        done.synchronize()
        if int(host[1]) != 0 or int(host[2]) != n_wg:
            self.persist_enc_fallbacks += 1
            self._step_fell_back = True
            return False
        return True

    def _persist_begin_step(self):
        if getattr(self, "_step_fell_back", False):
            self._persist_strikes += 1
            if self._persist_strikes >= PERSIST_STRIKES:
                self._persist_off = PERSIST_COOLDOWN
                self._persist_strikes = 0
                if not self._persist_warned:
                    self._persist_warned = True
                    warnings.warn("multi_speaker_tts_amd: %d consecutive steps fell back from the persistent launches (status %r: something "
                                  "else holds compute units); running the launch-per-step loops for %d steps before probing again"
                                  % (PERSIST_STRIKES, getattr(self, "persist_last_status", None), PERSIST_COOLDOWN), RuntimeWarning, stacklevel=4)
        elif getattr(self, "_step_was_persistent", False):
            self._persist_strikes = 0
        self._step_fell_back = False
        if self._persist_off > 0:
            self._persist_off -= 1
            self.persist_disabled_steps += 1
            self._step_was_persistent = False
            return False
        self._step_was_persistent = True
        return True

    def unpack_history(self, w):
        if getattr(w, "opk_valid", False):
            call("mstts_persist_unpack_history", ptr(w.opk), C.byref(w.dec))

    def _forward_tail(self, w, overlap_vocoder=False):
        d = self.d
        B, S = w.B, w.S
        H, M = d.dec_lstm, d.mem
        mk = w.masks
        self._gemm(w.pj, self.wp_pad, w.proj, S * B, self.proj_ld, H + M, H + M, self.proj_ld, self.proj_ld, bias=self.bp_pad)
        call("mstts_unpack_proj", ptr(w.proj), self.proj_ld, ptr(w.linear), ptr(w.stop), B, S, d.n_mel)
        x, cin = w.linear, d.n_mel
        for i in range(d.post_n):
            pre = "decoder/conv_%d/" % i
            cout = d.post_ch if i < d.post_n - 1 else d.n_mel
            conv_fwd(self, self._gemm, x, B * S, S, cin, cout, d.post_k, pre + "conv1d", w.post_a[i], ACT_TANH)
            bn_train_fwd(self, pre + "batch_normalization/", w.post_a[i], w.post_y[i], w.post_mean[i], w.post_rstd[i],
                         mk["post_drop_%d" % i], 1 - d.conv_drop, B * S, cout, w.bn_ws)
            x, cin = w.post_y[i], cout
        call("mstts_add", ptr(w.linear), ptr(x), ptr(w.mel_out), B * S * d.n_mel)
        if self.update_vocoder_bn and overlap_vocoder:
            ready = torch.cuda.Event()
            ready.record()
            with torch.cuda.stream(self._voc_stream):
                self._voc_stream.wait_event(ready)
                self._vocoder_bn_update(w)
                w.voc_done = torch.cuda.Event()
                w.voc_done.record()
        elif self.update_vocoder_bn:
            self._vocoder_bn_update(w)

    def _join_vocoder(self, w):
        if getattr(w, "voc_done", None) is not None:
            torch.cuda.current_stream().wait_event(w.voc_done)
            w.voc_done = None
        if getattr(w, "side_wgrads", False):
            done = torch.cuda.Event()
            done.record(self._enc_stream)
            torch.cuda.current_stream().wait_event(done)
            w.side_wgrads = False

    def _vocoder_bn_update(self, w):
        d = self.d
        B, S = w.B, w.S
        rows = B * S
        for k in range(1, d.bank_k + 1):
            sfx = bank_suffix(k)
            kk, ok = self.P(VOC + "convbank_0/conv1d%s/kernel" % sfx); b, ob = self.P(VOC + "convbank_0/conv1d%s/bias" % sfx)
            self._gemm(w.mel_out, kk, w.v_tmp, rows, d.bank_ch, k * d.n_mel, d.n_mel, d.bank_ch, d.bank_ch, bias=b, act=ACT_RELU,
                 win=(S, d.n_mel, (k - 1) // 2), b_off=ok, bias_off=ob, exact=True)
            bn_train_fwd(self, VOC + "convbank_0/batch_normalization%s/" % sfx, w.v_tmp, w.v_tmp2, w.v_stat, w.v_stat[d.bank_ch:], None, 1.0, rows, d.bank_ch, w.v_bn_ws)
            call("mstts_copy2d", ptr(w.v_tmp2), d.bank_ch, ptr(w.v_cat, (k - 1) * d.bank_ch), d.bank_k * d.bank_ch, rows, d.bank_ch, 0)
        C1 = d.bank_k * d.bank_ch
        call("mstts_maxpool2_same", ptr(w.v_cat), ptr(w.v_pool), B, S, C1)
        kk, ok = self.P(VOC + "convbank_0/conv1d_8/kernel"); b, ob = self.P(VOC + "convbank_0/conv1d_8/bias")
        self._gemm(w.v_pool, kk, w.v_p1, rows, d.proj1_ch, d.proj1_k * C1, C1, d.proj1_ch, d.proj1_ch, bias=b, act=ACT_RELU,
             win=(S, C1, (d.proj1_k - 1) // 2), b_off=ok, bias_off=ob, exact=True)
        bn_train_fwd(self, VOC + "convbank_0/batch_normalization_8/", w.v_p1, w.v_p1y, w.v_stat, w.v_stat[d.proj1_ch:], None, 1.0, rows, d.proj1_ch, w.v_bn_ws)
        kk, ok = self.P(VOC + "convbank_0/conv1d_9/kernel"); b, ob = self.P(VOC + "convbank_0/conv1d_9/bias")
        self._gemm(w.v_p1y, kk, w.v_p2, rows, d.n_mel, d.proj2_k * d.proj1_ch, d.proj1_ch, d.n_mel, d.n_mel, bias=b,
             win=(S, d.proj1_ch, (d.proj2_k - 1) // 2), b_off=ok, bias_off=ob, exact=True)
        bn_train_fwd(self, VOC + "convbank_0/batch_normalization_9/", w.v_p2, w.v_p2y, w.v_stat, w.v_stat[d.n_mel:], None, 1.0, rows, d.n_mel, w.v_bn_ws)

    def loss_and_backward(self, w, grad_scale=1.0, on_ready=None, on_abort=None, agree=None, agree_async=None, _redo=False):
        d, ps = self.d, self.params
        B, Te, L, S = w.B, w.Te, w.L, w.S
        H, M, A, Pn, He = d.dec_lstm, d.mem, d.att, d.prenet, d.enc_lstm
        mk, batch = w.masks, w.batch
        tok, tlen, mel, mlen = batch["Token"], batch["Token_Length"], batch["Mel"], batch["Mel_Length"]
        ps.grad.zero_()
        w.scalars.zero_()
        call("mstts_tts_loss_fwd_bwd", ptr(w.linear), ptr(w.mel_out), ptr(mel), ptr(w.stop), ptr(mlen), B, S, d.n_mel,
             int(self.use_l1), float(grad_scale), ptr(w.scalars), ptr(w.d_linear), ptr(w.d_post), ptr(w.d_stop))
        call("mstts_l2_loss_acc", ptr(ps.train), ptr(ps.wd_mask), ps.n_train, ptr(w.scalars, 3))
        wg_stream = self._enc_stream if (POSTNET_WGRAD_OVERLAP and getattr(w, "voc_done", None) is not None and not _redo) else None
        w.side_wgrads = wg_stream is not None
        chans = [d.post_ch] * (d.post_n - 1) + [d.n_mel]
        dy = w.d_post
        for i in range(d.post_n - 1, -1, -1):
            cin = d.n_mel if i == 0 else d.post_ch
            x_in = w.linear if i == 0 else w.post_y[i - 1]
            dx = w.post_dx if (i % 2 == 0) else w.post_dx2
            pre = "decoder/conv_%d/" % i
            conv_bn_bwd(self, self._gemm, pre + "conv1d", pre + "batch_normalization/", dy, x_in, w.post_a[i], w.post_mean[i], w.post_rstd[i],
                        mk["post_drop_%d" % i], 1 - d.conv_drop, ACT_TANH, B * S, S, cin, chans[i], d.post_k, w.post_dz[i], dx, self._bnws,
                        wgrad_stream=wg_stream)
            dy = dx
        postnet_ready_deferred = on_ready is not None and bool(getattr(w, "persist_bwd_now", False)) and bool(getattr(w, "persist_bwd", False)) and not _redo
        if on_ready is not None and not postnet_ready_deferred:
            self._join_vocoder(w)
            on_ready(*self._grad_range("decoder/conv_"))
        n = B * S * d.n_mel
        call("mstts_add", ptr(w.d_linear), ptr(w.d_post), ptr(w.d_linear), n)
        call("mstts_add", ptr(w.d_linear), ptr(dy), ptr(w.d_linear), n)
        call("mstts_pack_dproj", ptr(w.d_linear), ptr(w.d_stop), ptr(w.d_proj), self.proj_ld, B, S, d.n_mel)
        self.dwp_pad.zero_()
        self._gemm(w.pj, w.d_proj, self.dwp_pad, H + M, self.proj_ld, S * B, H + M, self.proj_ld, self.proj_ld, trans_a=True,
             split_k=max(2, _split_k(H + M, self.proj_ld, S * B)))
        gwp, ogwp = self.G("decoder/decoder/linear_projection/dense/kernel")
        gbp, ogbp = self.G("decoder/decoder/linear_projection/dense/bias")
        call("mstts_copy2d", ptr(self.dwp_pad), self.proj_ld, ptr(gwp, ogwp), d.n_mel + 1, H + M, d.n_mel + 1, 1)
        call("mstts_colsum", ptr(w.d_proj), S * B, d.n_mel + 1, self.proj_ld, ptr(gbp, ogbp), 1)
        self._gemm(w.d_proj, self.wp_pad, w.d_pj, S * B, H + M, self.proj_ld, self.proj_ld, self.proj_ld, H + M, trans_b=True)
        self._join_vocoder(w)
        w.dq_hist.zero_()
        db = w.dec_b
        db.fwd = C.pointer(w.dec)
        db.d_pj, db.dg0, db.dg1, db.dq_hist, db.de_hist, db.d_in0, db.ws = (ptr(w.d_pj), ptr(w.dg0), ptr(w.dg1), ptr(w.dq_hist),
                                                                             ptr(w.de_hist), ptr(w.d_in0), ptr(w.dec_bwd_ws))
        SB = S * B
        self.dw0f.zero_()
        w.d_keys.zero_()
        self.d_loc_k.zero_()
        parts = w.d_in0_parts
        use_pbwd = bool(getattr(w, "persist_bwd_now", False)) and bool(getattr(w, "persist_bwd", False)) and bool(getattr(w, "opk_valid", False)) and not _redo
        bwd_done = None
        if getattr(w, "opk_valid", False) and not use_pbwd:
            self.unpack_history(w)
        if use_pbwd:
            pb = w.pdesc_b
            pb.w0pk, pb.w1pk, pb.wqpk, pb.xch, pb.ctrl = ptr(self.pkb[0]), ptr(self.pkb[1]), ptr(self.pkb[2]), ptr(w.xch_b), ptr(w.pctrl_b)
            pb.stamps = ptr(self.persist_bwd_stamps) if self.persist_bwd_stamps is not None else None
            pb.opk = ptr(w.opk)
            pb.selftest_fail_step = int(self.persist_bwd_selftest)
            pb.near_xcd = int(os.environ.get("MSTTS_PERSIST_NEAR", "1") != "0")
            pb.recurrent_bf16 = int(self.persist_bf16)
            call("mstts_decoder_train_bwd_persistent", C.byref(db), C.byref(pb))
            ev = torch.cuda.Event(enable_timing=self.trace_events)
            ev.record()
            self.bptt_end_event = ev
            w.pctrl_b_host.copy_(w.pctrl_b, non_blocking=True)
            bwd_done = torch.cuda.Event()
            bwd_done.record()
            parts = 1
        else:
            self._ensure_fallback_packs()
            call("mstts_decoder_train_bwd", C.byref(db))
        if postnet_ready_deferred:
            on_ready(*self._grad_range("decoder/conv_"))
        def decoder_products():
            self._recurrent_wgrads(w, 0, S, part="products")
            g0, og0 = self.G(CELL % 0 + "kernel")
            call("mstts_copy2d", ptr(self.dw0f), 4 * H, ptr(g0, og0 + Pn * 4 * H), 4 * H, M, 4 * H, 1)
            call("mstts_copy2d", ptr(self.dw0f), 4 * H, ptr(g0, og0 + (Pn + M) * 4 * H), 4 * H, M, 4 * H, 1)
            call("mstts_copy2d", ptr(self.dw0f, M * 4 * H), 4 * H, ptr(g0, og0 + (Pn + 2 * M) * 4 * H), 4 * H, H, 4 * H, 1)
            dcur, dnxt = w.d_pre, w.d_pre2
            for i in range(d.prenet_n - 1, -1, -1):
                cin = d.n_mel if i == 0 else Pn
                x_in = w.frames if i == 0 else w.pre_d[i - 1]
                call("mstts_relu_dropout_bwd", ptr(dcur), ptr(w.pre_d[i]), ptr(mk["prenet_drop_%d" % i]), 1 - d.prenet_drop, ptr(dcur), SB * Pn)
                gk, ogk = self.G("decoder/decoder/prenet_%d/dense/kernel" % i); gb, ogb = self.G("decoder/decoder/prenet_%d/dense/bias" % i)
                self._gemm(x_in, dcur, gk, cin, Pn, SB, cin, Pn, Pn, trans_a=True, split_k=max(2, _split_k(cin, Pn, SB)), c_off=ogk)
                call("mstts_colsum", ptr(dcur), SB, Pn, Pn, ptr(gb, ogb), 1)
                if i > 0:
                    k, ok = self.P("decoder/decoder/prenet_%d/dense/kernel" % i)
                    self._gemm(dcur, k, dnxt, SB, cin, Pn, Pn, Pn, cin, trans_b=True, b_off=ok)
                    dcur, dnxt = dnxt, dcur
            gs = {}
            for field, name in (("conv_k", "attention_convolution_dense_layer/conv1d/kernel"), ("conv_b", "attention_convolution_dense_layer/conv1d/bias"),
                                ("dense_k", "attention_convolution_dense_layer/dense/kernel"), ("score_w", "score_layer/weight_w"), ("score_b", "score_layer/bias_b")):
                t, o = self.G(LSA + name)
                gs[field] = ptr(t, o)
            ls = w.dec.lsa
            call("mstts_lsa_unfold_location_grad", ls.conv_k, ls.conv_b, ls.dense_k, ptr(self.d_loc_k), gs["score_b"],
                 gs["conv_k"], gs["conv_b"], gs["dense_k"], d.att_k, d.att_ch, d.att)

        def memory_gradient():
            self._gemm(w.align_hist, w.d_pj, w.d_values, Te, M, S, B * Te, B * (H + M), M, trans_a=True, batch=B,
                       strides=(Te, H + M, Te * M), b_off=H, exact=True)
            if S > 1:
                for part in range(parts):
                    self._gemm(w.align_hist, w.d_in0, w.d_values, Te, M, S - 1, B * Te, B * (M + H), M, trans_a=True, batch=B,
                               strides=(Te, M + H, Te * M), b_off=(part * S + 1) * B * (M + H), accumulate=True, exact=True)
            wm, owm = self.P("attention/memory_layer/kernel"); gwm, ogwm = self.G("attention/memory_layer/kernel")
            self._gemm(w.values, w.d_keys, gwm, M, A, B * Te, M, A, A, trans_a=True, split_k=max(2, _split_k(M, A, B * Te)), c_off=ogwm)
            self._gemm(w.d_keys, wm, w.d_values, B * Te, M, A, A, A, M, trans_b=True, accumulate=True, b_off=owm)

        x_in, cin = w.enc_y[-1], d.enc_conv_ch
        bseqs = []
        for di, dr in enumerate(("fw", "bw")):
            k, ok = self.P(ENC_CELL % dr + "kernel")
            bseqs.append(lstm_seq_bwd(B, Te, He, (k, ok + cin * 4 * He), tlen, di, d.zoneout, mk["enc_zc_" + dr], mk["enc_zh_" + dr],
                                      (w.d_values, di * He), Te * M, M, w.enc_c[dr], w.enc_acts[dr], w.enc_craw[dr], w.enc_dgs[dr], w.enc_dgp[dr],
                                      w.enc_bwd_ws[dr]))
        def encoder_tail():
            x_in, cin = w.enc_y[-1], d.enc_conv_ch
            for di, dr in enumerate(("fw", "bw")):
                lstm_layer_grads(self, self._gemm, ENC_CELL % dr, x_in, w.enc_h[dr], w.enc_dgp[dr], w.enc_dgs[dr], w.enc_dy, B * Te, cin, He,
                                 dx_accumulate=di == 1)
            dy = w.enc_dy
            bufs = [w.enc_dx, w.enc_dy]
            for i in range(d.enc_conv_n - 1, -1, -1):
                cin = d.emb if i == 0 else d.enc_conv_ch
                x_in = w.emb if i == 0 else w.enc_y[i - 1]
                dx = bufs[(d.enc_conv_n - 1 - i) % 2]
                pre = "encoder/conv_%d/" % i
                conv_bn_bwd(self, self._gemm, pre + "conv1d", pre + "batch_normalization/", dy, x_in, w.enc_a[i], w.enc_mean[i], w.enc_rstd[i],
                            mk["enc_conv_drop_%d" % i], 1 - d.conv_drop, ACT_RELU, B * Te, Te, cin, d.enc_conv_ch, d.enc_conv_k, w.enc_dz, dx, self._bnws)
                dy = dx
            ge, oge = self.G("encoder/embedding_variable")
            call("mstts_embedding_bwd", ptr(tok), ptr(dy), ptr(ge, oge), B * Te, d.n_tok, d.emb)

        enc_ticket = None
        enc_persistent = bool(getattr(w, "enc_hist_valid", False)) and not _redo
        if enc_persistent and ENC_OVERLAP:
            self._recurrent_wgrads(w, 0, S, part="attention")
            memory_gradient()
            ready = torch.cuda.Event()
            ready.record()
            with torch.cuda.stream(self._enc_stream):
                self._enc_stream.wait_event(ready)
                enc_ticket = self._enc_persistent(w, "mstts_lstm_seq_bwd_pair_persistent", bseqs, 1, 32)
                if ENC_TAIL_OVERLAP:
                    encoder_tail()
                enc_done = torch.cuda.Event()
                enc_done.record()
            decoder_products()
            if on_ready is not None:
                on_ready(*self._grad_range("attention/", "decoder/decoder"))
            torch.cuda.current_stream().wait_event(enc_done)
            if not ENC_TAIL_OVERLAP:
                encoder_tail()
        else:
            self._recurrent_wgrads(w, 0, S, part="attention")
            decoder_products()
            memory_gradient()
            if on_ready is not None:
                on_ready(*self._grad_range("attention/", "decoder/decoder"))
            if enc_persistent:
                enc_ticket = self._enc_persistent(w, "mstts_lstm_seq_bwd_pair_persistent", bseqs, 1, 32)
            else:
                self._ensure_fallback_packs()
                call("mstts_lstm_seq_bwd_pair", C.byref(bseqs[0]), C.byref(bseqs[1]))
            encoder_tail()
        if on_ready is not None:
            on_ready(*self._grad_range("encoder/"))
        job_flag = None
        if agree_async is not None and not _redo:
            with torch.cuda.stream(self._side):
                if bwd_done is not None:
                    self._side.wait_event(bwd_done)
                if enc_ticket is not None:
                    self._side.wait_event(enc_ticket[0])
                if enc_ticket is None and bwd_done is None:
                    self._side.wait_stream(torch.cuda.current_stream())
                call("mstts_persist_status", ptr(w.pctrl_b) if bwd_done is not None else None, 256,
                     ptr(w.enc_ctrl) if enc_ticket is not None else None, enc_ticket[2] if enc_ticket is not None else 0, ptr(w.job_flag))
                agree_async(w.job_flag)
                w.job_flag_host.copy_(w.job_flag, non_blocking=True)
                job_flag = torch.cuda.Event()
                job_flag.record()
        passed = True
        if enc_ticket is not None:
            passed = self._enc_check(w, enc_ticket)
        if bwd_done is not None:
            bwd_done.synchronize()
            st = w.pctrl_b_host
            if int(st[1]) != 0 or int(st[2]) != 256:
                self.persist_bwd_fallbacks += 1
                self._step_fell_back = True
                self.persist_last_status = (int(st[0]), int(st[1]), int(st[2]))
                passed = False
        if job_flag is not None:
            job_flag.synchronize()
            job_ok = int(w.job_flag_host[0]) == 1
            if passed and not job_ok:
                self.collective_redos += 1
            passed = passed and job_ok
        else:
            passed = self._pass_verdict(passed, agree, _redo)
        if not passed:
            if on_abort is not None:
                on_abort()
            torch.cuda.current_stream().synchronize()
            return self.loss_and_backward(w, grad_scale=grad_scale, on_ready=on_ready, on_abort=on_abort, agree=agree, agree_async=agree_async, _redo=True)

    def _pass_verdict(self, passed, agree, redo):
        if agree is not None and not redo:
            mine = passed
            passed = bool(agree(passed))
            if mine and not passed:
                self.collective_redos += 1
        return passed

    def _recurrent_wgrads(self, w, lo, hi, part="all"):
        d = self.d
        B, Te = w.B, w.Te
        H, M, A, Pn = d.dec_lstm, d.mem, d.att, d.prenet
        n = (hi - lo) * B
        r = lo * B
        if part in ("all", "attention"):
            gsw, ogsw = self.G(LSA + "score_layer/weight_w"); gsb, ogsb = self.G(LSA + "score_layer/bias_b")
            call("mstts_lsa_param_bwd", C.byref(w.dec.lsa), hi - lo, ptr(w.q_hist, r * A), ptr(w.cum_hist, r * Te), ptr(w.de_hist, r * Te), ptr(w.d_keys),
                 ptr(self.d_loc_k), ptr(gsw, ogsw), ptr(gsb, ogsb), ptr(w.lsa_param_ws))
        if part == "attention":
            return
        g1, og1 = self.G(CELL % 1 + "kernel"); gb1, ogb1 = self.G(CELL % 1 + "bias")
        g0, og0 = self.G(CELL % 0 + "kernel"); gb0, ogb0 = self.G(CELL % 0 + "bias")
        call("mstts_colsum", ptr(w.dg1, r * 4 * H), n, 4 * H, 4 * H, ptr(gb1, ogb1), 1)
        call("mstts_colsum", ptr(w.dg0, r * 4 * H), n, 4 * H, 4 * H, ptr(gb0, ogb0), 1)
        self._gemm(w.in0, w.dg0, self.dw0f, M + H, 4 * H, n, M + H, 4 * H, 4 * H, trans_a=True, split_k=_split_k(M + H, 4 * H, n), accumulate=True,
             a_off=r * (M + H), b_off=r * 4 * H)
        self._gemm(w.in1, w.dg1, g1, 2 * H, 4 * H, n, 2 * H, 4 * H, 4 * H, trans_a=True, split_k=_split_k(2 * H, 4 * H, n), accumulate=True,
             a_off=r * 2 * H, b_off=r * 4 * H, c_off=og1)
        self._gemm(w.pre_d[-1], w.dg0, g0, Pn, 4 * H, n, Pn, 4 * H, 4 * H, trans_a=True, split_k=max(2, _split_k(Pn, 4 * H, n)),
             a_off=r * Pn, b_off=r * 4 * H, c_off=og0)
        k0, o0 = self.P(CELL % 0 + "kernel")
        self._gemm(w.dg0, k0, w.d_pre, n, Pn, 4 * H, 4 * H, 4 * H, Pn, trans_b=True, a_off=r * 4 * H, b_off=o0, c_off=r * Pn)
        gq, ogq = self.G(LSA + "query_layer/kernel")
        self._gemm(w.pj, w.dq_hist, gq, H, A, n, H + M, A, A, trans_a=True, split_k=max(2, _split_k(H, A, n)), a_off=r * (H + M), b_off=r * A, c_off=ogq)

    def _grad_range(self, *prefixes):
        ps = self.params
        offs = [(ps.offset[n], ps.offset[n] + (int(np.prod(ps.shape[n])) + 3) // 4 * 4) for n, _, _ in ps.table
                if ps.trainable[n] and n.startswith(prefixes)]
        return min(o for o, _ in offs), max(e for _, e in offs)

    def adam_step(self, grad_scale=1.0):
        lr = learning_rate(self.global_step)
        self._adam(lr, self.wr_rate, grad_scale)
        self._derived_stale = True
        self.refresh_derived()
        return lr

    def moving_stat_ranges(self):
        ps = self.params
        r = sorted((ps.offset[n], ps.offset[n] + (int(np.prod(ps.shape[n])) + 3) // 4 * 4) for n, _, _ in ps.table
                   if not ps.trainable[n] and n.endswith(("moving_mean", "moving_variance")))
        out = []
        for lo, hi in r:
            if out and out[-1][1] == lo:
                out[-1][1] = hi
            else:
                out.append([lo, hi])
        return [tuple(x) for x in out]

    def sync_statistics(self, group=None):
        from .dist import average_
        average_([self.params.frozen[lo:hi] for lo, hi in self.moving_stat_ranges()], group=group)

    def scalars(self, w, average=False, group=None):
        if average:
            from .dist import average_
            avg = w.scalars.clone()
            average_([avg], group=group)
            s = avg.cpu().numpy()
        else:
            s = w.scalars.detach().cpu().numpy()
        wr = float(s[3]) * self.wr_rate
        return {"Linear_Loss": float(s[0]), "Postnet_Loss": float(s[1]), "Stop_Loss": float(s[2]),
                "Weight_Regularization_Loss": wr, "Loss": float(s[0] + s[1] + s[2]) + wr}

    def scalars_async(self, w, average=False, group=None):
        if getattr(self, "_scalar_ring", None) is None:
            self._scalar_ring = torch.zeros(4, 4, dtype=torch.float32).pin_memory()
            self._scalar_next = 0
            self._scalar_avg = torch.zeros(4, dtype=torch.float32, device=self.device)
            self._scalar_handles = [None] * 4
        old = self._scalar_handles[self._scalar_next]
        if old is not None:
            old.get()
        slot = self._scalar_ring[self._scalar_next]
        src = w.scalars
        if average:
            from .dist import average_
            self._scalar_avg.copy_(w.scalars)
            average_([self._scalar_avg], group=group)
            src = self._scalar_avg
        slot.copy_(src, non_blocking=True)
        ev = torch.cuda.Event()
        ev.record()
        h = self._scalar_handles[self._scalar_next] = _LateScalars(ev, slot, self.wr_rate)
        self._scalar_next = (self._scalar_next + 1) % 4
        return h

    def exchange_timeouts(self, w):
        return int(w.energy_ws.view(torch.int64)[w.B * w.Te].item())

    def broadcast_state(self, src=0, group=None):
        from .dist import broadcast_
        ps = self.params
        step = torch.tensor([self.global_step], dtype=torch.int64, device=self.device)
        broadcast_([ps.train, ps.frozen, ps.adam_m, ps.adam_v, step], src=src, group=group)
        self.global_step = int(step.item())
        ps.touch()
        self._derived_stale = True

    def train_step(self, batch, masks=None, all_reduce=None):
        if self.deterministic and not getattr(lib.deterministic_gemm._depth, "n", 0):
            with lib.deterministic_gemm():
                return self.train_step(batch, masks=masks, all_reduce=all_reduce)
        B, Te = batch["Token"].shape
        L = batch["Mel"].shape[1]
        w = self.plan(B, Te, L)
        self.forward(batch, w, masks=masks, allowed=self._persist_begin_step(), overlap_vocoder=True)
        if all_reduce is not None:
            g = self.params.grad
            self.loss_and_backward(w, on_ready=lambda lo, hi: all_reduce.start(g, lo, hi), on_abort=lambda: all_reduce.finish(g),
                                   agree=all_reduce.agree, agree_async=all_reduce.agree_async if getattr(all_reduce, "async_flag", False) else None)
            all_reduce.finish(g)
        else:
            self.loss_and_backward(w)
        self.adam_step(grad_scale=1.0 / self.world if all_reduce is not None else 1.0)
        return w
```

### multi_speaker_tts_amd/lib.py

```python
from __future__ import annotations

import ctypes as C
import os

import torch

_HERE = os.path.dirname(os.path.abspath(__file__))
LIB_PATH = os.path.join(_HERE, "libmstts_hip.so")

ACT_NONE, ACT_RELU, ACT_TANH, ACT_SIGMOID = 0, 1, 2, 3

vp, i64, i32, f32, u64, u32 = C.c_void_p, C.c_int64, C.c_int32, C.c_float, C.c_uint64, C.c_uint32


class GemmDesc(C.Structure):
    _fields_ = [("A", vp), ("B", vp), ("C", vp), ("bias", vp),
                ("M", i64), ("N", i64), ("K", i64), ("lda", i64), ("ldb", i64), ("ldc", i64),
                ("trans_a", i32), ("trans_b", i32), ("win_T", i32), ("win_C", i32), ("win_pad", i32),
                ("act", i32), ("accumulate", i32), ("split_k", i32),
                ("batch", i64), ("stride_a", i64), ("stride_b", i64), ("stride_c", i64), ("alpha", f32), ("win_dil", i32)]


class LstmPointFwd(C.Structure):
    _fields_ = [("B", i64), ("H", i64), ("gates_h", vp), ("gates_parts", i32), ("gates_pstride", i64), ("xw", vp), ("xw_sb", i64), ("xw_st", i64), ("bias", vp),
                ("c_prev", vp), ("h_prev", vp), ("h_prev_ld", i64), ("zc", vp), ("zh", vp), ("zoneout", f32),
                ("lengths", vp), ("step", i32), ("reverse", i32), ("residual", vp), ("res_sb", i64), ("res_st", i64),
                ("out", vp), ("out_sb", i64), ("out_st", i64), ("c_next", vp), ("h_next", vp), ("h_next_ld", i64),
                ("acts_out", vp), ("c_raw", vp)]


class LstmPointBwd(C.Structure):
    _fields_ = [("B", i64), ("H", i64), ("d_out", vp), ("dout_sb", i64), ("dout_st", i64), ("dout_parts", i32), ("dout_pstride", i64),
                ("d_out2", vp), ("dout2_parts", i32), ("dout2_pstride", i64),
                ("d_c_state", vp), ("d_h_state", vp), ("d_h_state2", vp), ("dhs2_ld", i64), ("dhs2_parts", i32), ("dhs2_pstride", i64),
                ("acts", vp), ("c_raw", vp), ("c_prev", vp), ("zc", vp), ("zh", vp), ("zoneout", f32),
                ("lengths", vp), ("step", i32), ("reverse", i32), ("dgates", vp), ("dgates_pos", vp),
                ("dgp_sb", i64), ("dgp_st", i64), ("d_c_prev", vp), ("d_h_prev", vp), ("dq", vp), ("wq_t", vp), ("A", i64), ("dq_bf16", i32)]


class CellPackedDst(C.Structure):
    _fields_ = [("base", vp), ("K", i64), ("col0", i64), ("bf16", i32)]


class LsaPrenet(C.Structure):
    _fields_ = [("w0", vp), ("b0", vp), ("w1", vp), ("b1", vp), ("m0", vp), ("m1", vp), ("inv_keep", f32), ("P", i32),
                ("out", vp), ("out_ld", i64), ("out_p", CellPackedDst)]


class CellFwd(C.Structure):
    _fields_ = [("B", i64), ("H", i64), ("K", i64), ("Xp", vp), ("Wp", vp), ("xw", vp), ("xw_ld", i64), ("bias", vp),
                ("c_prev", vp), ("h_prev", vp), ("h_prev_ld", i64), ("zc", vp), ("zh", vp), ("zoneout", f32),
                ("out", vp), ("out_ld", i64), ("c_next", vp), ("h_next", vp), ("h_next_ld", i64), ("acts", vp), ("c_raw", vp),
                ("out_p", CellPackedDst), ("h_next_p", CellPackedDst),
                ("lengths", vp), ("step", i32), ("reverse", i32), ("xw_st", i64), ("out_st", i64), ("bf16", i32)]


class LsaConst(C.Structure):
    _fields_ = [("B", i64), ("T", i64), ("A", i64), ("M", i64), ("KS", i64), ("CH", i64),
                ("keys", vp), ("values", vp), ("lengths", vp),
                ("conv_k", vp), ("conv_b", vp), ("dense_k", vp), ("score_w", vp), ("score_b", vp), ("loc_k", vp), ("loc_b", vp), ("loc_kt", vp)]


class LstmSeqFwd(C.Structure):
    _fields_ = [("B", i64), ("T", i64), ("H", i64), ("xw", vp), ("wh", vp), ("wh_ld", i64), ("lengths", vp),
                ("reverse", i32), ("zoneout", f32), ("zc", vp), ("zh", vp), ("residual", vp),
                ("out", vp), ("out_sb", i64), ("out_st", i64),
                ("c_hist", vp), ("h_hist", vp), ("acts", vp), ("c_raw", vp), ("gates_ws", vp), ("wh_p", vp), ("h_p", vp)]


class LstmSeqBwd(C.Structure):
    _fields_ = [("B", i64), ("T", i64), ("H", i64), ("wh", vp), ("wh_ld", i64), ("lengths", vp), ("reverse", i32),
                ("zoneout", f32), ("zc", vp), ("zh", vp), ("d_out", vp), ("dout_sb", i64), ("dout_st", i64),
                ("c_hist", vp), ("acts", vp), ("c_raw", vp), ("dgates_step", vp), ("dgates_pos", vp), ("ws", vp)]


class DecoderTrain(C.Structure):
    _fields_ = [("B", i64), ("S", i64), ("H", i64), ("P", i64), ("lsa", LsaConst),
                ("xw0", vp), ("w0f", vp), ("w1", vp), ("b1", vp), ("wq", vp),
                ("zc0", vp), ("zh0", vp), ("zc1", vp), ("zh1", vp), ("zoneout", f32),
                ("in0", vp), ("in1", vp), ("pj", vp), ("c0", vp), ("c1", vp),
                ("acts0", vp), ("acts1", vp), ("craw0", vp), ("craw1", vp),
                ("q_hist", vp), ("align_hist", vp), ("cum_hist", vp), ("gates_ws", vp), ("energy_ws", vp), ("q_ws", vp), ("chains", i32),
                ("bf_w0f_f", vp), ("bf_w1_f", vp), ("bf_wq_f", vp), ("bf_w0f_b", vp), ("bf_w1_b", vp), ("bf_wq_b", vp),
                ("w0p", vp), ("w1p", vp), ("w0p16", vp), ("w1p16", vp), ("w0f_bp", vp), ("w1_bp", vp), ("wq_bp", vp), ("wq_t", vp), ("act_p", vp),
                ("energy_ws_floats", i64)]


class WgWnDesc(C.Structure):
    _fields_ = [("v", vp), ("g", vp), ("w", vp), ("ldw", i64), ("dv", vp), ("dg", vp), ("rows", i64), ("cols", i64)]


class PersistDesc(C.Structure):
    _fields_ = [("w0pk", vp), ("w1pk", vp), ("wqpk", vp), ("xch", vp), ("ctrl", vp), ("stamps", vp), ("opk", vp), ("selftest_fail_step", i32), ("near_xcd", i32), ("pre", vp), ("b0", vp), ("recurrent_bf16", i32)]


class PersistInferDesc(C.Structure):
    _fields_ = [("w0pk", vp), ("w1pk", vp), ("wqppk", vp), ("pre0", vp), ("bf", vp), ("u", vp), ("vp", vp), ("bp_pad", vp),
                ("xch", vp), ("ctrl", vp), ("stamps", vp), ("selftest_fail_step", i32), ("near_xcd", i32)]


class DecoderTrainBwd(C.Structure):
    _fields_ = [("fwd", C.POINTER(DecoderTrain)), ("d_pj", vp), ("dg0", vp), ("dg1", vp), ("dq_hist", vp),
                ("de_hist", vp), ("d_in0", vp), ("ws", vp)]


class DecoderInfer(C.Structure):
    _fields_ = [("B", i64), ("H", i64), ("P", i64), ("n_mel", i64), ("Smax", i64), ("lsa", LsaConst),
                ("pw0", vp), ("pb0", vp), ("pw1", vp), ("pb1", vp), ("pm0", vp), ("pm1", vp), ("prenet_keep", f32),
                ("wx0", vp), ("b0", vp), ("w0f", vp), ("w1", vp), ("b1", vp), ("wq", vp), ("wproj", vp), ("bproj", vp),
                ("zoneout", f32), ("in0", vp), ("in1", vp), ("pj", vp), ("c0", vp), ("c1", vp), ("cum", vp),
                ("pre_ws", vp), ("linear", vp), ("stop", vp), ("align_hist", vp), ("w0s", vp), ("wp_pad", vp), ("w0sp", vp), ("w1p", vp), ("act_p", vp), ("wp_own", vp), ("vp", vp)]


P = C.POINTER
SIGNATURES = {
    "mstts_last_error": (C.c_char_p, []),
    "mstts_abi_version": (i32, []),
    "mstts_debug_park_cus": (i32, [i32, i64, vp, vp]),
    "mstts_gemm_f32": (i32, [P(GemmDesc), vp]),
    "mstts_gemm_tail_split": (i32, [i32]),
    "mstts_gemm_split3": (i32, [i32]),
    "mstts_gemm_deterministic": (i32, [i32]),
    "mstts_gemm_split_big": (i32, [i32]),
    "mstts_gemm_big_min_workgroups": (i32, [i32, i32]),
    "mstts_gemm_bf16_autocut": (i32, [i32]),
    "mstts_persist_status": (i32, [vp, i32, vp, i32, vp, vp]),
    "mstts_gemm_bf16": (i32, [P(GemmDesc), vp]),
    "mstts_gemm_bf16_big": (i32, [i32]),
    "mstts_philox_keep_mask": (i32, [vp, i64, u64, u32, f32, vp]),
    "mstts_philox_keep_mask_rows": (i32, [vp, i64, i64, i64, u64, u32, u64, f32, vp]),
    "mstts_embedding_fwd": (i32, [vp, vp, vp, i64, i64, i64, vp]),
    "mstts_embedding_bwd": (i32, [vp, vp, vp, i64, i64, i64, vp]),
    "mstts_bn_train_fwd": (i32, [vp, vp, vp, vp, vp, vp, vp, vp, vp, f32, f32, f32, i64, i64, vp, vp]),
    "mstts_bn_infer_fwd": (i32, [vp, vp, vp, vp, vp, vp, f32, i64, i64, vp]),
    "mstts_bn_train_bwd": (i32, [vp, vp, vp, vp, vp, vp, f32, i32, vp, vp, vp, vp, i64, i64, vp, vp]),
    "mstts_dropout": (i32, [vp, vp, f32, vp, i64, vp]),
    "mstts_relu_dropout_bwd": (i32, [vp, vp, vp, f32, vp, i64, vp]),
    "mstts_colsum": (i32, [vp, i64, i64, i64, vp, i32, vp]),
    "mstts_add": (i32, [vp, vp, vp, i64, vp]),
    "mstts_fill": (i32, [vp, f32, i64, vp]),
    "mstts_copy2d": (i32, [vp, i64, vp, i64, i64, i64, i32, vp]),
    "mstts_maxpool2_same": (i32, [vp, vp, i64, i64, i64, vp]),
    "mstts_highway_combine": (i32, [vp, vp, vp, vp, i64, vp]),
    "mstts_maxpool2_same_bwd": (i32, [vp, vp, vp, i64, i64, i64, vp]),
    "mstts_highway_combine_bwd": (i32, [vp, vp, vp, vp, vp, vp, vp, i64, vp]),
    "mstts_l1_loss_fwd_bwd": (i32, [vp, vp, i64, vp, vp, vp]),
    "mstts_lstm_point_fwd": (i32, [P(LstmPointFwd), vp]),
    "mstts_lstm_point_bwd": (i32, [P(LstmPointBwd), vp]),
    "mstts_cell_fwd_supported": (i32, [i64, i64]),
    "mstts_pack_cell_fwd": (i32, [vp, i64, vp, i64, i64, vp]),
    "mstts_cell_fwd": (i32, [P(CellFwd), vp]),
    "mstts_cell_fwd_bf16_supported": (i32, [i64, i64]),
    "mstts_pack_cell_fwd_bf16": (i32, [vp, i64, vp, i64, i64, vp]),
    "mstts_pack_cell_act_bf16": (i32, [vp, i64, vp, i64, i64, vp]),
    "mstts_cell_fwd_pair": (i32, [P(CellFwd), P(CellFwd), vp]),
    "mstts_cell_act_floats": (i64, [i64, i64]),
    "mstts_pack_cell_act": (i32, [vp, i64, vp, i64, i64, vp]),
    "mstts_lsa_energy_fwd": (i32, [P(LsaConst), vp, i32, i64, vp, vp, vp, vp]),
    "mstts_lsa_context_fwd": (i32, [P(LsaConst), vp, vp, vp, vp, vp, i64, vp, i64, vp]),
    "mstts_lsa_step_ws_bytes": (i64, [i64, i64]),
    "mstts_lsa_step_bwd": (i32, [P(LsaConst), vp, i64, vp, i64, i32, i64, vp, vp, vp, vp, vp, vp, vp, i64, vp, vp, vp, vp]),
    "mstts_lsa_step_fwd": (i32, [P(LsaConst), vp, i32, i64, vp, vp, vp, vp, vp, i64, vp, i64, P(CellPackedDst), vp, C.c_uint32, vp]),
    "mstts_lsa_step_q_supported": (i32, [i64, i64, i64]),
    "mstts_lsa_step_q_ws_bytes": (i64, [i64, i64]),
    "mstts_lsa_step_qp_supported": (i32, [i64, i64, i64, i64]),
    "mstts_lsa_proj_pack_floats": (i64, []),
    "mstts_lsa_proj_pack": (i32, [vp, i64, i64, i64, vp, vp]),
    "mstts_lsa_step_qp_ws_bytes": (i64, [i64, i64]),
    "mstts_lsa_step_prenet_supported": (i32, [i64, i64]),
    "mstts_lsa_step_fwd_qp": (i32, [P(LsaConst), vp, i64, vp, i64, vp, vp, vp, i64, i64, vp, vp, vp, vp, vp, vp, i64, vp, i64, P(CellPackedDst),
                                    P(LsaPrenet), vp, C.c_uint32, i32, vp]),
    "mstts_lsa_step_fwd_q": (i32, [P(LsaConst), vp, i64, vp, i64, i32, vp, vp, vp, vp, vp, i64, vp, i64, P(CellPackedDst), vp, C.c_uint32, i32, vp]),
    "mstts_lsa_step_fwd_selftest": (i32, [P(LsaConst), vp, i32, i64, vp, vp, vp, vp, vp, i64, vp, C.c_uint32, i32, vp]),
    "mstts_lsa_dalign_bwd": (i32, [P(LsaConst), vp, i64, vp, i64, i32, i64, vp, vp, vp, vp, vp]),
    "mstts_lsa_denergy_bwd": (i32, [P(LsaConst), vp, vp, vp, vp, vp, vp, vp, vp]),
    "mstts_lsa_param_bwd": (i32, [P(LsaConst), i64, vp, vp, vp, vp, vp, vp, vp, vp, vp]),
    "mstts_lsa_param_bwd_ws_floats": (i64, [i64, i64, i64]),
    "mstts_lsa_fold_location": (i32, [vp, vp, vp, vp, vp, i64, i64, i64, vp]),
    "mstts_lsa_filter_by_unit": (i32, [vp, vp, i64, i64, vp]),
    "mstts_lsa_unfold_location_grad": (i32, [vp, vp, vp, vp, vp, vp, vp, vp, i64, i64, i64, vp]),
    "mstts_tts_loss_fwd_bwd": (i32, [vp, vp, vp, vp, vp, i64, i64, i64, i32, f32, vp, vp, vp, vp, vp]),
    "mstts_l2_loss_acc": (i32, [vp, vp, i64, vp, vp]),
    "mstts_shift_frames": (i32, [vp, vp, i64, i64, i64, vp]),
    "mstts_unpack_proj": (i32, [vp, i64, vp, vp, i64, i64, i64, vp]),
    "mstts_pack_dproj": (i32, [vp, vp, vp, i64, i64, i64, i64, vp]),
    "mstts_speaker_tile": (i32, [vp, vp, vp, i64, i64, i64, i64, i64, vp]),
    "mstts_conv_kernel_flip": (i32, [vp, vp, i64, i64, i64, vp]),
    "mstts_transpose01": (i32, [vp, vp, i64, i64, i64, vp]),
    "mstts_speaker_finalize": (i32, [vp, vp, i64, i64, i64, i64, vp]),
    "mstts_adam_tf": (i32, [vp, vp, vp, vp, vp, f32, f32, f32, f32, f32, f32, i64, vp]),
    "mstts_stft_mel": (i32, [vp, i64, f32, vp, vp, i32, i32, i32, i32, f32, vp, vp, i64, vp]),
    "mstts_stft_mel_ws_floats": (i64, [i64, i32, i64]),
    "mstts_stft_fft_supported": (i32, [i32, i32]),
    "mstts_stft_fft": (i32, [vp, vp, vp, i32, f32, vp, vp, vp, vp, i32, i32, i32, i32, f32, f32, vp, vp, i64, vp, vp, f32, i32, vp]),
    "mstts_griffin_lim_supported": (i32, [i32, i32, i32]),
    "mstts_griffin_lim_ws_floats": (i64, [i64, i32, i32]),
    "mstts_griffin_lim": (i32, [vp, vp, vp, P(i64), vp, i32, vp, vp, i32, i32, i32, f32, f32, f32, i32, vp, vp, vp]),
    "mstts_wav_resample_supported": (i32, [i32, i32]),
    "mstts_wav_resample_taps": (i32, [i32, i32]),
    "mstts_wav_resample": (i32, [vp, vp, vp, i32, i64, vp, i32, i32, vp, vp]),
    "mstts_wav_trim_ws_floats": (i64, [i64, i32]),
    "mstts_wav_trim": (i32, [vp, vp, i32, i64, i64, i32, i32, f32, vp, vp, vp, vp]),
    "mstts_wav_gather_scale": (i32, [vp, vp, vp, vp, i32, i64, f32, i32, i32, vp, vp, vp, vp]),
    "mstts_fold_rows": (i32, [vp, vp, i64, i64, i64, i64, vp]),
    "mstts_decoder_bf16_splits": (i32, [i64, i64, i64, P(i32)]),
    "mstts_skinny_bf16_fwd_splits": (i32, [i64, i64]),
    "mstts_skinny_bf16_bwd_splits": (i32, [i64, i64]),
    "mstts_pack_bf16_fwd": (i32, [vp, i64, vp, i64, i64, i32, vp]),
    "mstts_pack_bf16_bwd": (i32, [vp, i64, vp, i64, i64, i32, vp]),
    "mstts_skinny_fwd_bf16": (i32, [vp, i64, vp, vp, i64, i64, i64, i64, i32, vp]),
    "mstts_skinny_bwd_bf16": (i32, [vp, i64, vp, vp, i64, i64, i64, i64, i32, vp]),
    "mstts_ge2e_ws_floats": (i64, [i64, i64, i64]),
    "mstts_ge2e_loss_fwd_bwd": (i32, [vp, i64, i64, i64, i64, vp, vp, vp, i64, vp, vp]),
    "mstts_wg_overlap_add": (i32, [vp, vp, vp, i64, i64, i64, i64, i64, vp]),
    "mstts_wg_gate": (i32, [vp, i64, vp, i64, i64, vp]),
    "mstts_wg_gate_add": (i32, [vp, i64, vp, vp, i64, i64, vp]),
    "mstts_wg_res_skip": (i32, [vp, vp, vp, vp, i64, i64, i32, i32, vp]),
    "mstts_wg_coupling_inv": (i32, [vp, vp, vp, vp, f32, vp, i64, i64, i64, vp]),
    "mstts_philox_normal": (i32, [vp, i64, u64, u32, f32, vp]),
    "mstts_wg_weight_norm_fwd": (i32, [vp, i64, i64, vp]),
    "mstts_wg_weight_norm_bwd": (i32, [vp, i64, i64, vp]),
    "mstts_wg_coupling_fwd": (i32, [vp, vp, vp, vp, i64, i64, i64, vp, i64, i64, vp]),
    "mstts_wg_coupling_bwd": (i32, [vp, vp, vp, i64, i64, i64, vp, f32, vp, vp, i64, i64, vp]),
    "mstts_wg_inv1x1_logdet": (i32, [vp, vp, vp, i64, f32, vp, vp]),
    "mstts_wg_gate_bwd": (i32, [vp, i64, vp, vp, vp, i64, i64, i64, vp]),
    "mstts_wg_res_skip_bwd": (i32, [vp, vp, vp, vp, i64, i64, i32, vp]),
    "mstts_wg_overlap_add_bwd": (i32, [vp, vp, i64, i64, i64, i64, i64, i64, vp]),
    "mstts_wg_bias_fold": (i32, [vp, vp, vp, i64, i64, vp]),
    "mstts_adam_tf_clip": (i32, [vp, vp, vp, vp, vp, f32, f32, f32, f32, f32, f32, i64, vp]),
    "mstts_lstm_seq_fwd": (i32, [P(LstmSeqFwd), vp]),
    "mstts_lstm_seq_bwd": (i32, [P(LstmSeqBwd), vp]),
    "mstts_lstm_seq_fwd_pair": (i32, [P(LstmSeqFwd), P(LstmSeqFwd), vp]),
    "mstts_lstm_seq_bwd_pair": (i32, [P(LstmSeqBwd), P(LstmSeqBwd), vp]),
    "mstts_persist_lstm_supported": (i32, [i64, i64]),
    "mstts_persist_lstm_pack_floats": (i64, []),
    "mstts_persist_lstm_ws_bytes": (i64, []),
    "mstts_persist_lstm_pack": (i32, [vp, i64, vp, vp, vp]),
    "mstts_persist_lstm_supported_n": (i32, [i64, i64, i32]),
    "mstts_persist_lstm_fwd_supported_n": (i32, [i64, i64, i32]),
    "mstts_persist_lstm_pack_fwd": (i32, [vp, i64, i64, vp, vp]),
    "mstts_persist_lstm_ws_bytes_n": (i64, [i64, i32]),
    "mstts_persist_lstm_hist_floats_n": (i64, [i64, i64, i32]),
    "mstts_persist_lstm_bwd_floats_n": (i64, [i64, i64, i32]),
    "mstts_lstm_seq_fwd_persistent": (i32, [P(LstmSeqFwd), vp, vp, vp, vp, vp]),
    "mstts_lstm_seq_bwd_persistent": (i32, [P(LstmSeqBwd), vp, vp, vp, vp, vp, vp]),
    "mstts_persist_lstm_hist_floats": (i64, [i64]),
    "mstts_persist_lstm_bwd_floats": (i64, [i64]),
    "mstts_lstm_seq_fwd_pair_persistent": (i32, [P(LstmSeqFwd), P(LstmSeqFwd), vp, vp, vp, vp, vp, vp]),
    "mstts_lstm_seq_bwd_pair_persistent": (i32, [P(LstmSeqBwd), P(LstmSeqBwd), vp, vp, vp, vp, vp, vp, vp]),
    "mstts_lstm_point_bwd_pair": (i32, [P(LstmPointBwd), P(LstmPointBwd), vp]),
    "mstts_skinny_bwd_pair": (i32, [vp, vp, i64, vp, vp, i64, vp, vp, i64, i64, i64, i64, i32, vp]),
    "mstts_lstm_seq_ws_floats": (i64, [i64, i64, i32]),
    "mstts_decoder_train_fwd": (i32, [P(DecoderTrain), vp]),
    "mstts_decoder_train_bwd": (i32, [P(DecoderTrainBwd), vp]),
    "mstts_persist_fwd_supported": (i32, [i64, i64, i64, i64, i64, i64]),
    "mstts_persist_fwd_ws_bytes": (i64, []),
# ... 143 lines not shown
```

Before: 637,200.

## Fuse LSTM bias-gradient sums and optional d_keys into persistent BPTT kernel

The persistent backward kernel now accumulates the LSTM gate bias gradients in LDS using DPP reductions and writes them out at the end, so the two colsum passes over dg0/dg1 are skipped. It can also scatter d_keys atomics inside the recurrence (off by default), in which case a templated lsa_param_bwd variant skips the keys accumulation and the attention-param launch can be rescheduled. This adds LDS atomics and per-step work inside the latency-critical recurrent loop in exchange for removing separate reduction kernels.

```diff
diff --git a/include/mstts.h b/include/mstts.h
--- a/include/mstts.h
+++ b/include/mstts.h
@@ -391,6 +391,8 @@
     const mstts_decoder_train_desc* fwd;
     float* d_pj; float* dg0; float* dg1; float* dq_hist; float* de_hist; float* d_in0;
     float* ws;
+    float* db0; float* db1;
+    float* d_keys;
 } mstts_decoder_train_bwd_desc;
 int mstts_decoder_train_bwd(const mstts_decoder_train_bwd_desc* d, mstts_stream_t s);
 int64_t mstts_decoder_train_bwd_ws_floats(int64_t B, int64_t H, int64_t M, int64_t A, int64_t T, int64_t CH);
diff --git a/multi_speaker_tts_amd/csrc/lsa.hip b/multi_speaker_tts_amd/csrc/lsa.hip
--- a/multi_speaker_tts_amd/csrc/lsa.hip
+++ b/multi_speaker_tts_amd/csrc/lsa.hip
@@ -1056,6 +1056,7 @@
 #ifndef LSA_PARAM_WAVES
 #define LSA_PARAM_WAVES 3
 #endif
+template <bool KEYS>
 __global__ __launch_bounds__(256, LSA_PARAM_WAVES) void lsa_param_bwd_kernel(mstts_lsa_const c, int S, int steps_per_block,
                                                             const float* __restrict__ q_hist, const float* __restrict__ cum_hist,
                                                             const float* __restrict__ de_hist, float* __restrict__ d_keys,
@@ -1084,21 +1085,24 @@
     for (int r = 0; r < 16; ++r) {
         const int t = t0 + (r & 7) + 8 * kh + 16 * (r >> 3);
         key_v[r] = t < T ? c.keys[((long)b * T + t) * A_ + a] : 0.f;
-        acc_keys[r] = 0.f; acc_lk[r] = 0.f;
+        if constexpr (KEYS) acc_keys[r] = 0.f;
+        acc_lk[r] = 0.f;
     }
     float acc_w = 0.f, acc_b = 0.f;
     auto load_win = [&](int s) -> float {
         float v = 0.f;
+        const long row = ((long)s * B + b) * T;
         if (wave < 3) {
             const int t = t0 - pad + lane;
-            if (lane < PT + KS - 1 && t >= 0 && t < T) v = cum_hist[((long)s * B + b) * T + t];
+            if (lane < PT + KS - 1 && t >= 0 && t < T) v = KEYS ? cum_hist[row + t] : (cum_hist + row)[(unsigned)t];
         } else if (lane < PT) {
-            if (t0 + lane < T) v = de_hist[((long)s * B + b) * T + t0 + lane];
+            if (t0 + lane < T) v = KEYS ? de_hist[row + t0 + lane] : (de_hist + row)[(unsigned)(t0 + lane)];
         }
         return v;
     };
+    auto load_q = [&](int s) -> float { return KEYS ? q_hist[((long)s * B + b) * A_ + a] : (q_hist + ((long)s * B + b) * A_)[(unsigned)a]; };
     float nv = 0.f, nq = 0.f;
-    if (s_beg < s_end) { nv = load_win(s_beg); nq = q_hist[((long)s_beg * B + b) * A_ + a]; }
+    if (s_beg < s_end) { nv = load_win(s_beg); nq = load_q(s_beg); }
     int buf = 0;
     for (int s = s_beg; s < s_end; ++s, buf ^= 1) {
         if (wave < 3) {
@@ -1108,9 +1112,13 @@
             uint16_t* w = &s_wp[buf][wave][0][8 + lane];
 #pragma unroll
             for (int cc = 0; cc < 8; ++cc) w[cc * LP_WN - cc] = bits;
-        } else if (lane < PT) s_de[buf][lane] = nv;
+        } else if (lane < PT) {
+            int ln = lane;
+            if constexpr (!KEYS) asm volatile("" : "+v"(ln));
+            s_de[buf][ln] = nv;
+        }
         const float qk = nq + sb;
-        if (s + 1 < s_end) { nv = load_win(s + 1); nq = q_hist[((long)(s + 1) * B + b) * A_ + a]; }
+        if (s + 1 < s_end) { nv = load_win(s + 1); nq = load_q(s + 1); }
         __syncthreads();
         const uint16_t* wp = &s_wp[buf][0][0][0];
         lp_f32x16 L;
@@ -1134,7 +1142,7 @@
                 g[r] = de8[i] * wk * (1.f - u * u);
                 acc_w += de8[i] * u;
                 acc_b += g[r];
-                acc_keys[r] += g[r];
+                if constexpr (KEYS) acc_keys[r] += g[r];
             }
         }
 #pragma unroll
@@ -1146,26 +1154,31 @@
             LP_SIX(acc_lk, ah, am, al, gh, gm, gl);
         }
     }
-#pragma unroll
-    for (int r = 0; r < 16; ++r) {
-        const int row = (r & 7) + 8 * kh + 16 * (r >> 3);
-        if (t0 + row < T) atomicAdd(d_keys + ((long)b * T + t0 + row) * A_ + a, acc_keys[r]);
-    }
+    if constexpr (KEYS) {
+#pragma unroll
+        for (int r = 0; r < 16; ++r) {
+            const int row = (r & 7) + 8 * kh + 16 * (r >> 3);
+            if (t0 + row < T) atomicAdd(d_keys + ((long)b * T + t0 + row) * A_ + a, acc_keys[r]);
+        }
+    }
+    int kh_e = lane;
+    if constexpr (!KEYS) asm volatile("" : "+v"(kh_e));
+    kh_e >>= 5;
     acc_w += __shfl_xor(acc_w, 32);
     acc_b += __shfl_xor(acc_b, 32);
     if (part) {
         float* pb = part + ((long)(blockIdx.z * gridDim.y + blockIdx.y) * gridDim.x + blockIdx.x) * (LP_ROWS * A_);
 #pragma unroll
-        for (int r = 0; r < 16; ++r) pb[((r & 3) + 8 * (r >> 2) + 4 * kh) * A_ + a] = acc_lk[r];
-        if (kh == 0) { pb[32 * A_ + a] = acc_w; pb[33 * A_ + a] = acc_b; }
+        for (int r = 0; r < 16; ++r) pb[((r & 3) + 8 * (r >> 2) + 4 * kh_e) * A_ + a] = acc_lk[r];
+        if (kh_e == 0) { pb[32 * A_ + a] = acc_w; pb[33 * A_ + a] = acc_b; }
         return;
     }
 #pragma unroll
     for (int r = 0; r < 16; ++r) {
-        const int row = (r & 3) + 8 * (r >> 2) + 4 * kh;
+        const int row = (r & 3) + 8 * (r >> 2) + 4 * kh_e;
         if (row < KS) atomicAdd(d_loc_k + row * A_ + a, acc_lk[r]);
     }
-    if (kh == 0) {
+    if (kh_e == 0) {
         atomicAdd(d_score_w + a, acc_w);
         atomicAdd(d_score_b + a, acc_b);
     }
@@ -1415,8 +1428,10 @@
     MSTTS_REQUIRE(!ws || (reinterpret_cast<uintptr_t>(ws) & 7u) == 0, MSTTS_ERR_ALIGN, "lsa_param_bwd: the workspace must be 8-byte aligned");
     int nt, chunks, spb;
     lsa_param_geometry(c->B, c->T, S, &nt, &chunks, &spb, gemm_deterministic_now() != 0);
-    hipLaunchKernelGGL(lsa_param_bwd_kernel, dim3((unsigned)c->B, nt, chunks), dim3(256), 0, ST(s), *c, (int)S, spb, q_hist, cum_hist,
-                       de_hist, d_keys, d_loc_k, d_score_w, d_score_b, ws);
+    if (d_keys) hipLaunchKernelGGL(lsa_param_bwd_kernel<true>, dim3((unsigned)c->B, nt, chunks), dim3(256), 0, ST(s), *c, (int)S, spb, q_hist, cum_hist,
+                                   de_hist, d_keys, d_loc_k, d_score_w, d_score_b, ws);
+    else hipLaunchKernelGGL(lsa_param_bwd_kernel<false>, dim3((unsigned)c->B, nt, chunks), dim3(256), 0, ST(s), *c, (int)S, spb, q_hist, cum_hist,
+                            de_hist, nullptr, d_loc_k, d_score_w, d_score_b, ws);
     MSTTS_CHECK_LAUNCH("lsa_param_bwd");
     if (ws) {
         const int nblk = (int)c->B * nt * chunks;
diff --git a/multi_speaker_tts_amd/csrc/persist_bwd.hip b/multi_speaker_tts_amd/csrc/persist_bwd.hip
--- a/multi_speaker_tts_amd/csrc/persist_bwd.hip
+++ b/multi_speaker_tts_amd/csrc/persist_bwd.hip
@@ -17,6 +17,12 @@
 #endif
 #ifndef BPTT_LATE_OP0
 #define BPTT_LATE_OP0 0
+#endif
+#ifndef BPTT_BIAS_SUMS
+#define BPTT_BIAS_SUMS 1
+#endif
+#ifndef BPTT_DKEYS
+#define BPTT_DKEYS 1
 #endif
 #ifndef BSPLIT_C0
 #define BSPLIT_C0 0
@@ -47,6 +53,7 @@
               B_PD = B_DA + 8 * TT,
               B_SCR_END = B_PD + 4 * TT,
               B_TR = B_SCR_END > B_RED + 8 * 4 * 256 ? B_SCR_END : B_RED + 8 * 4 * 256,
+              B_BS = B_TR + 2 * 128,
               B_GP = B_TR + 3 * 128 + 512,
               B_A = B_GP + TT, B_CUM = B_A + TT, B_DE = B_CUM + TT + 48, B_DC = B_DE + TT, B_DPJ = B_DC + 96, B_QF = B_DPJ + 96,
               B_DQ = B_QF + 16, B_DQF = B_DQ + 512, B_LK = B_DQF + 16, B_FLAG = B_LK + 32 * 16, B_STAMP = B_FLAG + 4,
@@ -69,6 +76,8 @@
     const float* opk;
     int B, S, T;
     float* dg0; float* dg1; float* dq_hist; float* de_hist; float* d_in0;
+    float* d_keys;
+    float* db0; float* db1;
     float* xch; unsigned* ctrl; unsigned long long* stamps; int fail_step; int near_xcd;
 };
 
@@ -92,7 +101,7 @@
     typedef BL<TT> Y;
     constexpr int B_RED = Y::B_RED, B_G = Y::B_G, B_PC = Y::B_PC, B_DA = Y::B_DA, B_PD = Y::B_PD, B_TR = Y::B_TR, B_GP = Y::B_GP, B_A = Y::B_A, B_CUM = Y::B_CUM,
                   B_DE = Y::B_DE, B_DC = Y::B_DC, B_DPJ = Y::B_DPJ, B_QF = Y::B_QF, B_DQ = Y::B_DQ, B_DQF = Y::B_DQF, B_LK = Y::B_LK, B_FLAG = Y::B_FLAG,
-                  B_STAMP = Y::B_STAMP, B_VALT = Y::B_VALT, B_WQT = Y::B_WQT, B_WQO = Y::B_WQO;
+                  B_STAMP = Y::B_STAMP, B_BS = Y::B_BS, B_VALT = Y::B_VALT, B_WQT = Y::B_WQT, B_WQO = Y::B_WQO;
     constexpr bool QOWN = BPTT_QOWN != 0 && !BF16;
     constexpr bool W0L = QOWN && BPTT_W0LDS != 0 && !BF16;
     constexpr int NH = TT / 128;
@@ -189,6 +198,7 @@
         }
         for (int x = tid; x < TT + 48; x += PTH) sm[B_CUM + x] = 0.f;
         for (int x = tid; x < TT; x += PTH) { sm[B_GP + x] = 0.f; sm[B_A + x] = 0.f; sm[B_DE + x] = 0.f; }
+        if (tid < 128) sm[B_BS + tid] = 0.f;
         if constexpr (QOWN) {
             if (tid < 128) {
                 const int sl = tid >> 4, k4 = (tid >> 2) & 3, e = tid & 3;
@@ -213,6 +223,19 @@
     if (PROF && tid < NBSTAMP) sstamp[tid] = 0;
 #define PSTAMP(idx) do { if (PROF && tid == 0) { const unsigned n__ = (unsigned)wall_clock64(); sstamp[idx] += (unsigned)(n__ - tprev); tprev = n__; } } while (0)
 #define PABORT_CHECK() do { __syncthreads(); if (sflag[0]) return; } while (0)
+#define BIAS_ACC(CELL, DG) do { if (BPTT_BIAS_SUMS && ew) {                                                                             \
+        _Pragma("unroll") for (int q = 0; q < 4; ++q) {                                                                                \
+            float v__ = rowok ? DG[q] : 0.f;                                                                                           \
+            v__ += dpp_mov<0xB1, 0xf>(0.f, v__); v__ += dpp_mov<0x4E, 0xf>(0.f, v__);                                                  \
+            v__ += dpp_mov<0x141, 0xf>(0.f, v__); v__ += dpp_mov<0x140, 0xf>(0.f, v__);                                                \
+            if ((lane & 15) == 0) (void)__hip_atomic_fetch_add(sm + B_BS + (CELL) * 32 + et * 16 + q * 4 + ee, v__, __ATOMIC_RELAXED, __HIP_MEMORY_SCOPE_WORKGROUP); \
+        } } } while (0)
+#define BIAS_FOLD() do { if (BPTT_BIAS_SUMS && ew && ((kk & 31u) == 31u || s == 0) && (lane & 15) == 0) {                                \
+        _Pragma("unroll") for (int c__ = 0; c__ < 2; ++c__)                                                                            \
+            _Pragma("unroll") for (int q = 0; q < 4; ++q) {                                                                            \
+                float* p__ = sm + B_BS + c__ * 32 + et * 16 + q * 4 + ee;                                                              \
+                p__[64] += p__[0]; p__[0] = 0.f;                                                                                       \
+            } } } while (0)
 #define PFAIL() do { sflag[0] = 1; unsigned z__ = 0u; __hip_atomic_compare_exchange_strong(d.ctrl + 1, &z__, 2u, __ATOMIC_RELAXED, __ATOMIC_RELAXED, __HIP_MEMORY_SCOPE_AGENT); } while (0)
     float rav = 0.f, rcv = 0.f, rqv = 0.f, rdv = 0.f;
     const int abc = arow ? ab : 0;
@@ -429,6 +452,14 @@
                 xpublish(xr, (unsigned)((BO_DM1 + slot * BDM1 + o) * 4), out, gen);
             }
             PSTAMP(4);
+            if (BPTT_DKEYS && d.d_keys) {
+                float* kp = d.d_keys + (long)ab * T * PA + 16 * gi + ak;
+#pragma unroll
+                for (int m = 0; m < 4 * NH; ++m) {
+                    const int t = 128 * (m >> 2) + 4 * atg + (m & 3);
+                    if (t < T) unsafeAtomicAdd(kp + (long)t * PA, sm[B_G + (15 + t) * 16 + ak]);
+                }
+            }
 #pragma unroll 1
             for (int hh = 0; hh < NH; ++hh) {
                 const int p0 = 128 * hh + 4 * atg;
@@ -522,6 +553,7 @@
                 xpublish_near(xr, (unsigned)((BO_DG1 + slot * BDG + o) * 4), val, gen, near);
             }
             if (elive) { float* o = d.dg1 + sB * 4 * PH; o[o4H] = dgv[0]; o[o4H + PH] = dgv[1]; o[o4H + 2 * PH] = dgv[2]; o[o4H + 3 * PH] = dgv[3]; }
+            BIAS_ACC(1, dgv);
         }
         PSTAMP(7);
 #define PROD_GATHER(OFF_DG)                                                                                                           \
@@ -662,6 +694,8 @@
                 xpublish_near(xr, (unsigned)((BO_DG0 + slot * BDG + o) * 4), val, gen, near);
             }
             if (elive) { float* o = d.dg0 + sB * 4 * PH; o[o4H] = dgv[0]; o[o4H + PH] = dgv[1]; o[o4H + 2 * PH] = dgv[2]; o[o4H + 3 * PH] = dgv[3]; }
+            BIAS_ACC(0, dgv);
+            BIAS_FOLD();
         }
         PSTAMP(11);
         {
@@ -681,6 +715,11 @@
         __syncthreads();
         PSTAMP(14);
     }
+    if (BPTT_BIAS_SUMS && d.db0 && tid < 32) {
+        const int cell = tid >> 4, qe = tid & 15;
+        float* out = (cell ? d.db1 : d.db0) + (qe >> 2) * PH + 4 * g0 + (qe & 3);
+        *out += sm[B_BS + 64 + cell * 32 + qe] + sm[B_BS + 64 + cell * 32 + 16 + qe];
+    }
     if (tid == 0) {
         __hip_atomic_fetch_add(d.ctrl + 2, 1u, __ATOMIC_RELAXED, __HIP_MEMORY_SCOPE_AGENT);
         if (PROF && d.stamps) {
@@ -691,6 +730,8 @@
 #undef PSTAMP
 #undef PABORT_CHECK
 #undef PFAIL
+#undef BIAS_ACC
+#undef BIAS_FOLD
 #undef PROD_GATHER
 #undef ISSUE_UPDATE1
 #undef ISSUE_UPDATE0
@@ -826,6 +867,10 @@
     a.loc_k = d->lsa.loc_k; a.loc_b = d->lsa.loc_b; a.score_w = d->lsa.score_w; a.score_b = d->lsa.score_b;
     a.d_pj = bd->d_pj; a.opk = p->opk; a.B = (int)B; a.S = (int)S; a.T = (int)T;
     a.dg0 = bd->dg0; a.dg1 = bd->dg1; a.dq_hist = bd->dq_hist; a.de_hist = bd->de_hist; a.d_in0 = bd->d_in0;
+    MSTTS_REQUIRE((bd->db0 == nullptr) == (bd->db1 == nullptr) && (BPTT_BIAS_SUMS || !bd->db0), MSTTS_ERR_SHAPE, "decoder_train_bwd_persistent: db0 / db1 go together");
+    a.db0 = bd->db0; a.db1 = bd->db1;
+    MSTTS_REQUIRE(BPTT_DKEYS || !bd->d_keys, MSTTS_ERR_SHAPE, "decoder_train_bwd_persistent: built without d_keys (BPTT_DKEYS=0)");
+    a.d_keys = bd->d_keys;
     a.xch = p->xch; a.ctrl = p->ctrl; a.stamps = (unsigned long long*)p->stamps; a.fail_step = p->selftest_fail_step > 0 ? p->selftest_fail_step - 1 : -1; a.near_xcd = p->near_xcd;
 #define PBW_LAUNCH(T_)                                                                                                                  \
     {                                                                                                                                   \
diff --git a/multi_speaker_tts_amd/engine.py b/multi_speaker_tts_amd/engine.py
--- a/multi_speaker_tts_amd/engine.py
+++ b/multi_speaker_tts_amd/engine.py
@@ -28,6 +28,9 @@
 VOC_OVERLAP = os.environ.get("MSTTS_VOC_OVERLAP", "1") != "0"
 POSTNET_WGRAD_OVERLAP = os.environ.get("MSTTS_POSTNET_WGRAD_OVERLAP", "1") != "0"
 ENC_TAIL_OVERLAP = os.environ.get("MSTTS_ENC_TAIL_OVERLAP", "1") != "0"
+BPTT_BIAS_SUMS = os.environ.get("MSTTS_BPTT_BIAS_SUMS", "1") != "0"
+BPTT_DKEYS = os.environ.get("MSTTS_BPTT_DKEYS", "0") != "0"
+LSA_PARAM_PLACE = os.environ.get("MSTTS_LSA_PARAM_PLACE", "mid")
 ENC_OVERLAP = os.environ.get("MSTTS_ENC_OVERLAP", "1") != "0"
 
 
@@ -739,6 +742,9 @@
         parts = w.d_in0_parts
         use_pbwd = bool(getattr(w, "persist_bwd_now", False)) and bool(getattr(w, "persist_bwd", False)) and bool(getattr(w, "opk_valid", False)) and not _redo
         bwd_done = None
+        db.db0 = db.db1 = db.d_keys = None
+        bias_in_launch = use_pbwd and BPTT_BIAS_SUMS
+        keys_in_launch = use_pbwd and BPTT_DKEYS
         if getattr(w, "opk_valid", False) and not use_pbwd:
             self.unpack_history(w)
         if use_pbwd:
@@ -749,7 +755,13 @@
             pb.selftest_fail_step = int(self.persist_bwd_selftest)
             pb.near_xcd = int(os.environ.get("MSTTS_PERSIST_NEAR", "1") != "0")
             pb.recurrent_bf16 = int(self.persist_bf16)
+            if bias_in_launch:
+                gb0, ogb0 = self.G(CELL % 0 + "bias"); gb1, ogb1 = self.G(CELL % 1 + "bias")
+                db.db0, db.db1 = ptr(gb0, ogb0), ptr(gb1, ogb1)
+            if keys_in_launch:
+                db.d_keys = ptr(w.d_keys)
             call("mstts_decoder_train_bwd_persistent", C.byref(db), C.byref(pb))
+            db.db0 = db.db1 = db.d_keys = None
             ev = torch.cuda.Event(enable_timing=self.trace_events)
             ev.record()
             self.bptt_end_event = ev
@@ -762,8 +774,11 @@
             call("mstts_decoder_train_bwd", C.byref(db))
         if postnet_ready_deferred:
             on_ready(*self._grad_range("decoder/conv_"))
-        def decoder_products():
-            self._recurrent_wgrads(w, 0, S, part="products")
+        def attention_params():
+            self._recurrent_wgrads(w, 0, S, part="attention", keys=not keys_in_launch)
+
+        def decoder_products(before_unfold=None):
+            self._recurrent_wgrads(w, 0, S, part="products", bias=not bias_in_launch)
             g0, og0 = self.G(CELL % 0 + "kernel")
             call("mstts_copy2d", ptr(self.dw0f), 4 * H, ptr(g0, og0 + Pn * 4 * H), 4 * H, M, 4 * H, 1)
             call("mstts_copy2d", ptr(self.dw0f), 4 * H, ptr(g0, og0 + (Pn + M) * 4 * H), 4 * H, M, 4 * H, 1)
@@ -786,6 +801,8 @@
                 t, o = self.G(LSA + name)
                 gs[field] = ptr(t, o)
             ls = w.dec.lsa
+            if before_unfold is not None:
+                before_unfold()
             call("mstts_lsa_unfold_location_grad", ls.conv_k, ls.conv_b, ls.dense_k, ptr(self.d_loc_k), gs["score_b"],
                  gs["conv_k"], gs["conv_b"], gs["dense_k"], d.att_k, d.att_ch, d.att)
 
@@ -828,7 +845,9 @@
         enc_ticket = None
         enc_persistent = bool(getattr(w, "enc_hist_valid", False)) and not _redo
         if enc_persistent and ENC_OVERLAP:
-            self._recurrent_wgrads(w, 0, S, part="attention")
+            place = LSA_PARAM_PLACE if keys_in_launch else "front"
+            if place == "front":
+                attention_params()
             memory_gradient()
             ready = torch.cuda.Event()
             ready.record()
@@ -839,14 +858,16 @@
                     encoder_tail()
                 enc_done = torch.cuda.Event()
                 enc_done.record()
-            decoder_products()
+            if place == "mid":
+                attention_params()
+            decoder_products(before_unfold=attention_params if place == "behind" else None)
             if on_ready is not None:
                 on_ready(*self._grad_range("attention/", "decoder/decoder"))
             torch.cuda.current_stream().wait_event(enc_done)
             if not ENC_TAIL_OVERLAP:
                 encoder_tail()
         else:
-            self._recurrent_wgrads(w, 0, S, part="attention")
+            attention_params()
             decoder_products()
             memory_gradient()
             if on_ready is not None:
@@ -907,7 +928,7 @@
                 self.collective_redos += 1
         return passed
 
-    def _recurrent_wgrads(self, w, lo, hi, part="all"):
+    def _recurrent_wgrads(self, w, lo, hi, part="all", bias=True, keys=True):
         d = self.d
         B, Te = w.B, w.Te
         H, M, A, Pn = d.dec_lstm, d.mem, d.att, d.prenet
@@ -915,14 +936,15 @@
         r = lo * B
         if part in ("all", "attention"):
             gsw, ogsw = self.G(LSA + "score_layer/weight_w"); gsb, ogsb = self.G(LSA + "score_layer/bias_b")
-            call("mstts_lsa_param_bwd", C.byref(w.dec.lsa), hi - lo, ptr(w.q_hist, r * A), ptr(w.cum_hist, r * Te), ptr(w.de_hist, r * Te), ptr(w.d_keys),
+            call("mstts_lsa_param_bwd", C.byref(w.dec.lsa), hi - lo, ptr(w.q_hist, r * A), ptr(w.cum_hist, r * Te), ptr(w.de_hist, r * Te), ptr(w.d_keys) if keys else None,
                  ptr(self.d_loc_k), ptr(gsw, ogsw), ptr(gsb, ogsb), ptr(w.lsa_param_ws))
         if part == "attention":
             return
         g1, og1 = self.G(CELL % 1 + "kernel"); gb1, ogb1 = self.G(CELL % 1 + "bias")
         g0, og0 = self.G(CELL % 0 + "kernel"); gb0, ogb0 = self.G(CELL % 0 + "bias")
-        call("mstts_colsum", ptr(w.dg1, r * 4 * H), n, 4 * H, 4 * H, ptr(gb1, ogb1), 1)
-        call("mstts_colsum", ptr(w.dg0, r * 4 * H), n, 4 * H, 4 * H, ptr(gb0, ogb0), 1)
+        if bias:
+            call("mstts_colsum", ptr(w.dg1, r * 4 * H), n, 4 * H, 4 * H, ptr(gb1, ogb1), 1)
+            call("mstts_colsum", ptr(w.dg0, r * 4 * H), n, 4 * H, 4 * H, ptr(gb0, ogb0), 1)
         self._gemm(w.in0, w.dg0, self.dw0f, M + H, 4 * H, n, M + H, 4 * H, 4 * H, trans_a=True, split_k=_split_k(M + H, 4 * H, n), accumulate=True,
              a_off=r * (M + H), b_off=r * 4 * H)
         self._gemm(w.in1, w.dg1, g1, 2 * H, 4 * H, n, 2 * H, 4 * H, 4 * H, trans_a=True, split_k=_split_k(2 * H, 4 * H, n), accumulate=True,
diff --git a/multi_speaker_tts_amd/lib.py b/multi_speaker_tts_amd/lib.py
--- a/multi_speaker_tts_amd/lib.py
+++ b/multi_speaker_tts_amd/lib.py
@@ -101,7 +101,7 @@
 
 class DecoderTrainBwd(C.Structure):
     _fields_ = [("fwd", C.POINTER(DecoderTrain)), ("d_pj", vp), ("dg0", vp), ("dg1", vp), ("dq_hist", vp),
-                ("de_hist", vp), ("d_in0", vp), ("ws", vp)]
+                ("de_hist", vp), ("d_in0", vp), ("ws", vp), ("db0", vp), ("db1", vp), ("d_keys", vp)]
 
 
 class DecoderInfer(C.Structure):
```

Result: no change. 634,300 (-0.5%).
